# CSB5/lofreq

Measured on AMD Instinct MI355X. Metric: pileup columns/sec at depth 10000, higher is better.
Workload: dtype f64

## Files before the change

lofreq_amd/csrc/lfq_api.hip:

```cpp
#include "lfq_bound.h"
#include "lfq_ctx.h"

namespace {

struct LfqDeviceStreams {
    hipStream_t stream = nullptr, dps = nullptr, side[2] = {nullptr, nullptr};
    hipEvent_t ev_tail[3] = {nullptr, nullptr, nullptr};
    bool tail_recorded = false;
    hipEvent_t ev_end = nullptr;
    bool end_recorded = false;
    int refs = 0;
};
std::mutex g_streams_m;
LfqDeviceStreams g_streams[64];

bool acquire_streams(int device, lfq_ctx *c);
void release_streams(int device);

void *pin_acquire_impl(lfq_ctx *c, size_t bytes, int *slot)
{
    int best = -1, empty = -1, smallest = -1;
    for (int i = 0; i < LFQ_PIN_SLOTS; i++) {
        auto &b = c->pin_pool[i];
        if (b.used) {
            continue;
        }
        if (!b.p) {
            empty = (empty < 0) ? i : empty;
        } else if (b.cap >= bytes) {
            best = (best < 0 || b.cap < c->pin_pool[best].cap) ? i : best;
        } else {
            smallest = (smallest < 0 || b.cap < c->pin_pool[smallest].cap) ? i : smallest;
        }
    }
    if (best < 0) {
        best = (empty >= 0) ? empty : smallest;
        if (best < 0) {
            return nullptr;
        }
        auto &b = c->pin_pool[best];
        if (b.p) {
            (void)hipHostFree(b.p);
            b.p = nullptr;
            b.cap = 0;
        }
        const size_t cap = std::max<size_t>(bytes + bytes / 4, (size_t)1 << 16);
        if (hipHostMalloc(&b.p, cap, hipHostMallocDefault) != hipSuccess) {
            b.p = nullptr;
            return nullptr;
        }
        b.cap = cap;
    }
    c->pin_pool[best].used = 1;
    *slot = best;
    return c->pin_pool[best].p;
}

int phred_safe(double p) { return (p <= 0.0) ? INT32_MAX : (int)(-10.0 * log10l(p)); }

double jq_threshold(int m)
{
    if (m <= 0) {
        return INFINITY;
    }
    uint64_t lo = 1, hi;
    double one = 2.0;
    memcpy(&hi, &one, 8);
    if (phred_safe(4.9406564584124654e-324) < m) {
        return 0.0;
    }
    while (hi - lo > 1) {
        const uint64_t mid = lo + (hi - lo) / 2;
        double x;
        memcpy(&x, &mid, 8);
        if (phred_safe(x) >= m) {
            lo = mid;
        } else {
            hi = mid;
        }
    }
    double x;
    memcpy(&x, &lo, 8);
    return x;
}

}

int lfq_make_params(const lfq_conf *conf, const lfq_tracks *tr, LfqParams *P, bool indel_mode)
{
    if (conf->def_alt_jq == -1) {
        return LFQ_ERR_UNSUPPORTED;
    }
    memset(P, 0, sizeof(*P));
    P->min_bq4 = std::min(std::max(conf->min_bq, 0), 128);
    P->min_alt_bq4 = std::min(std::max(std::max(conf->min_bq, conf->min_alt_bq), 0), 128);
    P->def_alt_bq = conf->def_alt_bq;
    P->jq_reject_above = jq_threshold(conf->min_jq);
    P->alt_jq_reject_above = jq_threshold(conf->min_alt_jq);
    P->def_alt_jp = (conf->def_alt_jq != 0) ? pow(10.0, -1.0 * conf->def_alt_jq / 10.0) : -1.0;
    P->general = (conf->min_jq > 0) || (conf->min_alt_jq > 0) || (conf->def_alt_bq == -1);
    P->min_cov = conf->min_cov;
    P->use_baq = (conf->flag & LFQ_USE_BAQ) && tr->baq;
    P->use_mq = (conf->flag & LFQ_USE_MQ) != 0;
    P->use_sq = (conf->flag & LFQ_USE_SQ) && tr->sq;
    P->bonf_dynamic = conf->bonf_dynamic;
    P->bonf_base = conf->bonf_subst;
    P->sig = (double)conf->sig;
    P->prune_slack = 1e-6;
    P->bonf_step = 3;
    P->bonf_reset_first = 1;
    P->phase1_chunks = LFQ_PHASE1_CHUNKS;
    P->seg_budget_mid = P->seg_budget_big = LFQ_SEG_BUDGET;
    P->seg_max = lfq_knobs().seg_max >= 0 ? lfq_knobs().seg_max : LFQ_SEG_MAX;
    P->seg_max_mid = lfq_knobs().seg_max_mid >= 0 ? lfq_knobs().seg_max_mid : LFQ_SEG_MAX;
    if (indel_mode) {
        P->min_bq4 = P->min_alt_bq4 = 0;
        P->def_alt_bq = 0;
        P->jq_reject_above = P->alt_jq_reject_above = INFINITY;
        P->def_alt_jp = -1.0;
        P->general = 0;
        P->min_cov = 0;
        P->use_baq = tr->baq != nullptr;
        P->bonf_base = conf->bonf_indel;
        P->bonf_step = 1;
        P->bonf_reset_first = 0;
    }
    return LFQ_OK;
}


namespace {

bool acquire_streams(int device, lfq_ctx *c)
{
    std::lock_guard<std::mutex> lk(g_streams_m);
    if (device < 0 || device >= 64) {
        return false;
    }
    LfqDeviceStreams &d = g_streams[device];
    if (d.refs == 0) {
        int prio_lo = 0, prio_hi = 0;
        (void)hipDeviceGetStreamPriorityRange(&prio_lo, &prio_hi);
        bool ok = true;
        ok = hipStreamCreateWithFlags(&d.stream, hipStreamNonBlocking) == hipSuccess;
        ok = ok && hipStreamCreateWithPriority(&d.dps, hipStreamNonBlocking, prio_hi) == hipSuccess;
        for (int i = 0; ok && i < 2; i++) {
            ok = hipStreamCreateWithPriority(&d.side[i], hipStreamNonBlocking, prio_hi) == hipSuccess;
        }
        for (int i = 0; ok && i < 3; i++) {
            ok = hipEventCreateWithFlags(&d.ev_tail[i], hipEventDisableTiming) == hipSuccess;
        }
        ok = ok && hipEventCreateWithFlags(&d.ev_end, hipEventDisableTiming) == hipSuccess;
        d.tail_recorded = false;
        d.end_recorded = false;
        if (!ok) {
            return false;
        }
    }
    d.refs++;
    c->stream = d.stream;
    c->dps = d.dps;
    c->side[0] = d.side[0];
    c->side[1] = d.side[1];
    return true;
}

void release_streams(int device)
{
    std::lock_guard<std::mutex> lk(g_streams_m);
    LfqDeviceStreams &d = g_streams[device];
    if (d.refs > 0 && --d.refs == 0) {
        if (d.stream) (void)hipStreamDestroy(d.stream);
        if (d.dps) (void)hipStreamDestroy(d.dps);
        for (int i = 0; i < 2; i++) {
            if (d.side[i]) (void)hipStreamDestroy(d.side[i]);
        }
        for (int i = 0; i < 3; i++) {
            if (d.ev_tail[i]) (void)hipEventDestroy(d.ev_tail[i]);
        }
        if (d.ev_end) (void)hipEventDestroy(d.ev_end);
        d = LfqDeviceStreams();
    }
}

int tail_wait(lfq_ctx *c, hipStream_t st)
{
    std::lock_guard<std::mutex> lk(g_streams_m);
    LfqDeviceStreams &d = g_streams[c->device];
    if (c->stream != d.stream || c->batch_gate == LFQ_GATE_NONE) {
        return LFQ_OK;
    }
    if (c->batch_gate == LFQ_GATE_END) {
        if (d.end_recorded && hipStreamWaitEvent(st, d.ev_end, 0) != hipSuccess) {
            return LFQ_ERR_HIP;
        }
        return LFQ_OK;
    }
    if (!d.tail_recorded) {
        return LFQ_OK;
    }
    for (int i = 0; i < 3; i++) {
        if (hipStreamWaitEvent(st, d.ev_tail[i], 0) != hipSuccess) {
            return LFQ_ERR_HIP;
        }
    }
    return LFQ_OK;
}

int tail_record(lfq_ctx *c, int i, hipStream_t on)
{
    std::lock_guard<std::mutex> lk(g_streams_m);
    LfqDeviceStreams &d = g_streams[c->device];
    if (c->stream != d.stream) {
        return LFQ_OK;
    }
    if (hipEventRecord(d.ev_tail[i], on) != hipSuccess) {
        return LFQ_ERR_HIP;
    }
    d.tail_recorded = true;
    return LFQ_OK;
}

int end_record(lfq_ctx *c, hipStream_t on)
{
    std::lock_guard<std::mutex> lk(g_streams_m);
    LfqDeviceStreams &d = g_streams[c->device];
    if (c->stream != d.stream) {
        return LFQ_OK;
    }
    if (hipEventRecord(d.ev_end, on) != hipSuccess) {
        return LFQ_ERR_HIP;
    }
    d.end_recorded = true;
    return LFQ_OK;
}

void fill_luts(LfqLuts *L)
{
    for (int q = 0; q < 256; q++) {
        const double p = pow(10.0, -1.0 * q / 10.0);
        L->bq[q] = p;
        L->baq[q] = p;
        L->mq[q] = p;
        L->sq[q] = p;
    }
    L->baq[255] = 0.0;
    L->sq[255] = 0.0;
    L->sq[254] = 0.0;
    L->mq[255] = 0.0;
    L->mq[0] = 0.5;
}

void leader_main(lfq_ctx *c)
{
    (void)hipSetDevice(c->device);
    for (;;) {
        {
            std::unique_lock<std::mutex> lk(*c->lm);
            c->lcv->wait(lk, [&] { return c->leader_go > 0 || c->leader_stop; });
            if (c->leader_stop) {
                return;
            }
            c->leader_go--;
        }
        int64_t n = 0;
        if (hipEventSynchronize(c->ev_heavy) == hipSuccess) {
            n = std::min<int64_t>(std::max<int64_t>(*(volatile int32_t *)c->h_nheavy, 0), c->heavy_cap);
        }
        lfq_sb_precompute(c->h_tuples, 3 * n);
        {
            std::lock_guard<std::mutex> lk(*c->lm);
            c->sb_pending--;
        }
        c->lcv->notify_all();
    }
}

int ensure_workspace(lfq_ctx *c, int64_t ncols)
{
    if (ncols > c->ws_cols) {
        int64_t cap = 0;
        int64_t want = ncols + ncols / 8 + 1024;
        if (c->d_flags) (void)hipFree(c->d_flags);
        if (c->d_prefix) (void)hipFree(c->d_prefix);
        if (c->d_entries) (void)hipFree(c->d_entries);
        if (c->d_tiles) (void)hipFree(c->d_tiles);
        if (c->d_unsplit) (void)hipFree(c->d_unsplit);
        if (c->d_retry) (void)hipFree(c->d_retry);
        c->d_unsplit = nullptr;
        c->d_retry = nullptr;
        c->d_flags = nullptr;
        c->d_prefix = nullptr;
        c->d_entries = nullptr;
        c->d_tiles = nullptr;
        c->ws_cols = 0;
        LFQ_TRY(grow(&c->d_flags, &cap, want));
        cap = 0;
        LFQ_TRY(grow(&c->d_prefix, &cap, want));
        cap = 0;
        LFQ_TRY(grow(&c->d_entries, &cap, want));
        cap = 0;
        LFQ_TRY(grow(&c->d_tiles, &cap, 2 * (want / 1024 + 8 * (LFQ_MAX_SEGMENTS + 1))));
        cap = 0;
        LFQ_TRY(grow(&c->d_unsplit, &cap, want));
        cap = 0;
        LFQ_TRY(grow(&c->d_retry, &cap, want));
        c->ws_cols = want;
    }
    return LFQ_OK;
}


}

void *lfq_pin_acquire(lfq_ctx *c, size_t bytes, int *slot) { return pin_acquire_impl(c, bytes, slot); }

extern "C" {

void *lfq_host_alloc(size_t bytes)
{
    void *p = nullptr;
    if (hipHostMalloc(&p, bytes ? bytes : 1, hipHostMallocDefault) != hipSuccess) {
        (void)hipGetLastError();
        return nullptr;
    }
    return p;
}

void lfq_host_free(void *p)
{
    if (p) {
        (void)hipHostFree(p);
    }
}
int lfq_create(lfq_ctx **out, int device_ordinal)
{
    if (!out) {
        return LFQ_ERR_INVALID;
    }
    *out = nullptr;
    int ndev = 0;
    if (hipGetDeviceCount(&ndev) != hipSuccess || ndev <= 0 || device_ordinal < 0 || device_ordinal >= ndev) {
        return LFQ_ERR_NO_DEVICE;
    }
    if (hipSetDevice(device_ordinal) != hipSuccess) {
        return LFQ_ERR_NO_DEVICE;
    }
    lfq_ctx *c = (lfq_ctx *)calloc(1, sizeof(lfq_ctx));
    if (!c) {
        return LFQ_ERR_NOMEM;
    }
    c->device = device_ordinal;
    c->sub_ncols = -1;
    c->dense_strand = 1;
    c->dense_counts = 1;
    c->indel_host_arrays = 1;
    c->plp_max_depth = LFQ_NO_MAX_DEPTH;
    c->baq_par_d = 0.00001f;
    c->baq_par_e = 0.4f;
    hipDeviceProp_t prop;
    c->n_cu = 256;
    if (hipGetDeviceProperties(&prop, device_ordinal) == hipSuccess && prop.multiProcessorCount > 0) {
        c->n_cu = prop.multiProcessorCount;
    }
    bool ok = acquire_streams(device_ordinal, c);
    c->own_streams = ok ? 1 : 0;
    ok = ok && hipMalloc((void **)&c->d_luts, sizeof(LfqLuts)) == hipSuccess;
    ok = ok && hipMalloc((void **)&c->d_counters, (LFQ_MAX_SEGMENTS + 1) * LFQ_NCOUNTERS * sizeof(int32_t)) == hipSuccess;
    ok = ok && hipHostMalloc((void **)&c->h_counters, (LFQ_MAX_SEGMENTS + 1) * LFQ_NCOUNTERS * sizeof(int32_t) + 16,
                             hipHostMallocDefault) == hipSuccess;
    for (int i = 0; ok && i < 4; i++) {
        ok = hipEventCreate(&c->ev[i]) == hipSuccess;
    }
    for (int i = 0; ok && i < 3; i++) {
        ok = hipEventCreate(&c->ev_join[i]) == hipSuccess;
    }
    for (int s = 0; ok && s < LFQ_MAX_SEGMENTS; s++) {
        ok = hipEventCreate(&c->ev_cnt[s][0]) == hipSuccess && hipEventCreate(&c->ev_cnt[s][1]) == hipSuccess;
        ok = ok && hipEventCreate(&c->ev_scan[s]) == hipSuccess;
        ok = ok && hipEventCreate(&c->ev_light[s][0]) == hipSuccess && hipEventCreate(&c->ev_light[s][1]) == hipSuccess;
        for (int i = 0; ok && i < 2; i++) {
            ok = hipEventCreate(&c->ev_side[i][s][0]) == hipSuccess && hipEventCreate(&c->ev_side[i][s][1]) == hipSuccess;
        }
    }
    if (ok && !lfq_knobs().no_sb_precompute) {
        c->heavy_cap = 1 << 16;
        ok = hipHostMalloc((void **)&c->h_tuples, (size_t)c->heavy_cap * 3 * 4 * sizeof(int32_t), hipHostMallocMapped) == hipSuccess
             && hipHostMalloc((void **)&c->h_nheavy, 64, hipHostMallocMapped) == hipSuccess
             && hipHostGetDevicePointer((void **)&c->d_tuples_mapped, c->h_tuples, 0) == hipSuccess
             && hipHostGetDevicePointer((void **)&c->d_nheavy_mapped, c->h_nheavy, 0) == hipSuccess
             && hipEventCreateWithFlags(&c->ev_heavy, hipEventDisableTiming) == hipSuccess;
        if (ok) {
            *c->h_nheavy = 0;
            c->lm = new std::mutex();
            c->lcv = new std::condition_variable();
            c->leader = new std::thread(leader_main, c);
        }
    }
    if (ok) {
        LfqLuts h;
        fill_luts(&h);
        ok = hipMemcpy(c->d_luts, &h, sizeof(h), hipMemcpyHostToDevice) == hipSuccess;
    }
    if (ok && lfq_knobs().private_stream) {
        ok = lfq_set_private_stream(c, 1) == LFQ_OK;
    }
    if (!ok) {
        lfq_destroy(c);
        return LFQ_ERR_HIP;
    }
    *out = c;
    return LFQ_OK;
}

void lfq_destroy(lfq_ctx *c)
{
    if (c && c->leader) {
        {
            std::lock_guard<std::mutex> lk(*c->lm);
            c->leader_stop = 1;
        }
        c->lcv->notify_all();
        c->leader->join();
        delete c->leader;
        delete c->lm;
        delete c->lcv;
        c->leader = nullptr;
    }
    if (c) {
        if (c->d_plp_in) (void)hipFree(c->d_plp_in);
        if (c->d_plp_out) (void)hipFree(c->d_plp_out);
        delete c->plp_indel;
        if (c->d_plp_ne) (void)hipFree(c->d_plp_ne);
        for (int i = 0; i < 5; i++) {
            if (c->d_tmp[i]) (void)hipFree(c->d_tmp[i]);
        }
        for (int k = 0; k < 9; k++) {
            if (c->rs_cache[k].p) (void)(k == 4 || k == 7 ? hipHostFree(c->rs_cache[k].p) : hipFree(c->rs_cache[k].p));
        }
        if (c->up_stream) (void)hipStreamDestroy(c->up_stream);
        if (c->priv_stream) (void)hipStreamDestroy(c->priv_stream);
        if (c->ev_up) (void)hipEventDestroy(c->ev_up);
        if (c->ev_apply) (void)hipEventDestroy(c->ev_apply);
        free_pinned(&c->h_pin, &c->pin_bytes);
        free_pinned(&c->h_pin2, &c->pin2_bytes);
        free_pinned(&c->h_sum, &c->h_sum_bytes);
        free_pinned(&c->h_pq, &c->h_pq_bytes);
        for (int i = 0; i < LFQ_PIN_SLOTS; i++) {
            if (c->pin_pool[i].p) (void)hipHostFree(c->pin_pool[i].p);
        }
        for (LfqEvPair *t : {&c->baq_t, &c->fill_t, &c->idq_t, &c->sites_t[0], &c->sites_t[1], &c->sum_t, &c->pq_t}) {
            t->destroy();
        }
        if (c->d_detlim) (void)hipFree(c->d_detlim);
        if (c->d_sites_in) (void)hipFree(c->d_sites_in);
        if (c->d_sites_out) (void)hipFree(c->d_sites_out);
        if (c->d_sum) (void)hipFree(c->d_sum);
        delete c->plp_sum;
        if (c->d_pq) (void)hipFree(c->d_pq);
        if (c->d_baq_scr) (void)hipFree(c->d_baq_scr);
        if (c->d_baq_expect) (void)hipFree(c->d_baq_expect);
        if (c->d_baq_tmp8) (void)hipFree(c->d_baq_tmp8);
        if (c->d_baq_nflag) (void)hipFree(c->d_baq_nflag);
        if (c->d_baq_itab) (void)hipFree(c->d_baq_itab);
        if (c->d_baq_terms) (void)hipFree(c->d_baq_terms);
        lfq_viterbi_release(c);
        lfq_bam_release(c);
        lfq_bgzf_release(c);
        lfq_bgzf_deflate_release(c);
        lfq_bam_index_release(c);
        lfq_fasta_release(c);
        lfq_bed_dev_release(c->bed);
        if (c->h_tuples) (void)hipHostFree(c->h_tuples);
        if (c->h_nheavy) (void)hipHostFree(c->h_nheavy);
        if (c->ev_heavy) (void)hipEventDestroy(c->ev_heavy);
    }
    if (!c) {
        return;
    }
    (void)hipSetDevice(c->device);
    if (c->stream) (void)hipStreamSynchronize(c->stream);
    void *bufs[] = {c->d_luts, c->d_flags, c->d_prefix, c->d_entries, c->d_counters, c->d_tiles, c->d_longs, c->d_pool, c->d_unsplit, c->d_retry,
                    c->d_scratch, c->d_counts, c->d_pvals, c->d_stage, c->d_approx_mu};
    for (void *b : bufs) {
        if (b) (void)hipFree(b);
    }
    if (c->h_counters) (void)hipHostFree(c->h_counters);
    for (int i = 0; i < 4; i++) {
        if (c->ev[i]) (void)hipEventDestroy(c->ev[i]);
    }
    for (int i = 0; i < 3; i++) {
        if (c->ev_join[i]) (void)hipEventDestroy(c->ev_join[i]);
        if (i == 0 && c->ev_segw) (void)hipEventDestroy(c->ev_segw);
        if (i == 0 && c->ev_prep) (void)hipEventDestroy(c->ev_prep);
        if (i == 0 && c->ev_mid) (void)hipEventDestroy(c->ev_mid);
    }
    for (int s = 0; s < LFQ_MAX_SEGMENTS; s++) {
        hipEvent_t evs[] = {c->ev_cnt[s][0], c->ev_cnt[s][1], c->ev_scan[s], c->ev_light[s][0], c->ev_light[s][1],
                            c->ev_side[0][s][0], c->ev_side[0][s][1], c->ev_side[1][s][0], c->ev_side[1][s][1]};
        for (hipEvent_t e : evs) {
            if (e) (void)hipEventDestroy(e);
        }
    }
    if (c->own_streams) {
        release_streams(c->device);
    }
    free(c);
}

int lfq_synchronize(lfq_ctx *c)
{
    if (!c) {
        return LFQ_ERR_INVALID;
    }
    LFQ_TRY_HIP(hipStreamSynchronize(c->stream));
    LFQ_TRY_HIP(hipEventSynchronize(c->ev[3]));
    return LFQ_OK;
}

int lfq_order_after_batch(lfq_ctx *c, hipStream_t st)
{
    if (c->batch_recorded) {
        LFQ_TRY_HIP(hipStreamWaitEvent(st, c->ev[3], 0));
    }
    return LFQ_OK;
}

int lfq_batch_device_impl(lfq_ctx *c, const lfq_conf *conf, const lfq_tracks *tr, lfq_col_counts *d_counts,
                             lfq_col_pvals *d_pvals, int64_t pvals_capacity, void *stream_or_null,
                             bool indel_mode)
{
    if (!c || !conf || !tr || tr->ncols < 0 || tr->ncols > 0x7ffffff0LL) {
        return LFQ_ERR_INVALID;
    }
    if (tr->ncols > 0 && (!tr->nt || !tr->bq || !tr->mq || !tr->col_off || !tr->ref_base || !d_counts
                          || (!d_pvals && pvals_capacity > 0))) {
        return LFQ_ERR_INVALID;
    }
    if ((((uintptr_t)tr->nt) | ((uintptr_t)tr->bq)) & 15u) {
        return LFQ_ERR_INVALID;
    }
    LFQ_TRY_HIP(hipSetDevice(c->device));
    hipStream_t st = stream_or_null ? (hipStream_t)stream_or_null : c->stream;
    const LfqKnobs &kn = lfq_knobs();
    const bool single_stream = kn.single_stream != 0;
    hipStream_t dps = single_stream ? st : c->dps;
    hipStream_t side0 = single_stream ? st : c->side[0], side1 = single_stream ? st : c->side[1];
    hipStream_t side_i[2] = {side0, side1};
    LfqParams P;
    LFQ_TRY(lfq_make_params(conf, tr, &P, indel_mode));
    if (c->batch_gate == LFQ_GATE_NONE && !indel_mode) {
        if (kn.seg_max < 0) {
            P.seg_max = 2;
        }
        if (kn.seg_max_mid < 0) {
            P.seg_max_mid = 2;
        }
    }
    P.detlim_af = indel_mode ? nullptr : c->detlim_af;
    P.lazy_strand = (c->lazy_now && !indel_mode && !P.general && !P.detlim_af) ? 1 : 0;
    P.sparse_counts = (P.lazy_strand && ((d_counts == c->d_counts && c->lazy_forced) || !c->dense_counts)) ? 1 : 0;
    P.scan_gate_maxk = 0;
    P.approx_n = (!P.detlim_af && conf->approx_threshold_n > 0) ? conf->approx_threshold_n : 0;
    LFQ_TRY(ensure_workspace(c, tr->ncols));

    LfqTracksDev T;
    T.nt = tr->nt;
    T.nt_packed = (tr->flags & LFQ_TRACKS_NT_PACKED) ? 1 : 0;
    T.pad_ = 0;
    T.bq = tr->bq;
    T.baq = tr->baq;
    T.mq = tr->mq;
    T.sq = tr->sq;
    T.col_off = tr->col_off;
    T.ref_base = tr->ref_base;
    T.coverage_plp = tr->coverage_plp;
    T.num_bases = tr->num_bases;
    T.ncols = tr->ncols;

    const int64_t ncols = tr->ncols;
    int32_t *gcounters = c->d_counters + LFQ_MAX_SEGMENTS * LFQ_NCOUNTERS;
    c->cur_stream = st;
    c->cur_pvals_cap = pvals_capacity;
    c->cur_ncols = ncols;
    c->cur_segments = 0;
    c->cur_col_off = tr->col_off;
    c->cur_indel_mode = indel_mode ? 1 : 0;
    c->cur_obs_bytes_x2 = (T.nt_packed ? 1 : 2) + 2;
    if (P.general) {
        c->cur_obs_bytes_x2 += 2 * ((T.baq ? 1 : 0) + 1 + (T.sq ? 1 : 0));
        if (P.def_alt_bq == -1) {
            c->cur_obs_bytes_x2 += (T.nt_packed ? 1 : 2) + 2;
        }
    }
    c->cur_col_bytes = 8 + 1 + (T.coverage_plp ? 4 : 0) + (T.num_bases ? 4 : 0) + (P.detlim_af ? 4 : 0);
    LFQ_TRY(lfq_order_after_batch(c, st));
    LFQ_TRY(tail_wait(c, st));
    LFQ_TRY_HIP(hipMemsetAsync(c->d_counters, 0, (LFQ_MAX_SEGMENTS + 1) * LFQ_NCOUNTERS * sizeof(int32_t), st));
    if (ncols > 0) {
        LFQ_TRY_HIP(hipMemsetAsync(c->d_retry, 0, (size_t)ncols, st));
    }
    LFQ_TRY_HIP(hipEventRecord(c->ev[0], st));
    if (ncols == 0) {
        LFQ_TRY_HIP(hipMemcpyAsync(c->h_counters, c->d_counters,
                                   (LFQ_MAX_SEGMENTS + 1) * LFQ_NCOUNTERS * sizeof(int32_t), hipMemcpyDeviceToHost, st));
        LFQ_TRY_HIP(hipEventRecord(c->ev[3], st));
        c->batch_recorded = 1;
        return LFQ_OK;
    }

    int64_t max_depth = tr->max_col_obs;
    if (max_depth <= 0) {
        LFQ_TRY(lfq_launch_maxdepth(T, gcounters, st));
        LFQ_TRY_HIP(hipMemcpyAsync(c->h_counters, gcounters, LFQ_NCOUNTERS * sizeof(int32_t), hipMemcpyDeviceToHost, st));
        LFQ_TRY_HIP(hipStreamSynchronize(st));
        max_depth = c->h_counters[LFQ_GC_MAXDEPTH];
    }
    {
        static const LfqLuts h_luts = [] {
            LfqLuts h;
            fill_luts(&h);
            return h;
        }();
        const bool lb = !P.general && P.def_alt_bq == 0 && P.def_alt_jp < 0.0;
        P.bound_p_lo = (lb && !indel_mode && kn.bound_gate && lfq_count_is_lean(T, P, max_depth))
                           ? lfq_bound_p_lo(h_luts.bq, P.min_alt_bq4, LFQ_BOUND_QLO) : 0.0;
        const int kreg = lfq_screen_kreg(c->kreg_hint);
        const bool screen_runs = !kn.skip_light && kn.light_kernel != 2 && kreg > 0;
        P.scan_gate_maxk = (P.bound_p_lo > 0.0 && P.approx_n == 0 && kn.scan_gate && screen_runs) ? kreg - 1 : 0;
    }
    const int64_t per_block = 3 * max_depth + 72;
    int n_big_blocks = c->n_cu;
    const int64_t budget = (int64_t)1 << 29;
    if (per_block * n_big_blocks > budget) {
        n_big_blocks = (int)std::max<int64_t>(8, budget / per_block);
    }
    LFQ_TRY(grow(&c->d_scratch, &c->scratch_doubles, per_block * n_big_blocks));
    if (!c->d_longs) {
        c->long_cap = 1 << 16;
        c->pool_cells = kn.split_pool_cells;
        LFQ_TRY_HIP(hipMalloc((void **)&c->d_longs, (size_t)c->long_cap * (sizeof(LfqLong) + LFQ_SEG_MAX * sizeof(int32_t))));
        LFQ_TRY_HIP(hipMalloc((void **)&c->d_pool, (size_t)std::max(c->pool_cells, 1) * sizeof(LfqSegCell)));
        LFQ_TRY_HIP(hipEventCreateWithFlags(&c->ev_segw, hipEventDisableTiming));
        LFQ_TRY_HIP(hipEventCreateWithFlags(&c->ev_prep, hipEventDisableTiming));
        LFQ_TRY_HIP(hipEventCreateWithFlags(&c->ev_mid, hipEventDisableTiming));
    }

    const int n_seg = 1;
    c->cur_segments = n_seg;
    LFQ_TRY_HIP(hipEventRecord(c->ev_join[2], st));
    LFQ_TRY_HIP(hipStreamWaitEvent(dps, c->ev_join[2], 0));

    bool big_joined = false;
    for (int s = 0; s < n_seg; s++) {
        const int64_t c0 = ncols * s / n_seg, c1 = ncols * (s + 1) / n_seg;
        LfqWork W;
        W.tested_prefix = c->d_prefix;
        W.entries = c->d_entries + c0;
        W.counters = c->d_counters + s * LFQ_NCOUNTERS;
        W.gcounters = gcounters;
        W.block_sums = (int32_t *)(c->d_tiles + 2 * (c0 / 1024 + 8 * s));
        W.long_cap = c->long_cap / n_seg;
        W.pool_cells = c->pool_cells / n_seg;
        W.longs = c->d_longs + (int64_t)s * W.long_cap;
        W.pool = c->d_pool + (int64_t)s * W.pool_cells;
        W.unsplit = c->d_unsplit + c0;

        LFQ_TRY_HIP(hipEventRecord(c->ev_cnt[s][0], st));
        const bool ungated = c->batch_gate == LFQ_GATE_NONE && st == c->stream && !c->priv_stream_on && !single_stream;
        LFQ_TRY(lfq_launch_count(T, c0, c1, P, c->d_luts, d_counts, c->d_flags, max_depth, st, ungated));
        c->cur_sparse_counts = P.sparse_counts && lfq_count_is_shallow(T, P, max_depth);
        LFQ_TRY_HIP(hipEventRecord(c->ev_cnt[s][1], st));

        LFQ_TRY_HIP(hipStreamWaitEvent(dps, c->ev_cnt[s][1], 0));
        LFQ_TRY(lfq_launch_scan(T, c0, c1, P, c->d_flags, d_counts, W, dps));
        if (P.approx_n > 0) {
            LFQ_TRY(grow(&c->d_approx_mu, &c->approx_mu_bytes, (c1 - c0) * 8));
            LFQ_TRY(lfq_launch_approx_gate(T, P, c->d_luts, d_counts, W, c1 - c0, (double *)c->d_approx_mu, c->d_flags, dps));
            LFQ_TRY(lfq_launch_scan(T, c0, c1, P, c->d_flags, d_counts, W, dps, true));
        }
        LFQ_TRY_HIP(hipEventRecord(c->ev_scan[s], dps));
        const bool sb_heavy = n_seg == 1 && !indel_mode && c->leader && !kn.no_sb_precompute;
        auto launch_heavy = [&]() -> int {
            if (P.lazy_strand) {
                LFQ_TRY(lfq_launch_strand_heavy(T, W, d_counts, c->d_tuples_mapped, c->d_nheavy_mapped, c->heavy_cap, 16, dps));
            } else {
                LFQ_TRY(lfq_launch_gather_heavy(W, d_counts, c->d_tuples_mapped, c->d_nheavy_mapped, c->heavy_cap, 16, dps));
            }
            LFQ_TRY_HIP(hipEventRecord(c->ev_heavy, dps));
            {
                std::lock_guard<std::mutex> lk(*c->lm);
                c->leader_go++;
                c->sb_pending++;
            }
            c->lcv->notify_all();
            return LFQ_OK;
        };
        const bool screen = !kn.skip_light && kn.light_kernel != 2;
        if (sb_heavy && !screen) {
            LFQ_TRY(launch_heavy());
        }
        const int64_t seg_cols = c1 - c0;
        const int screen_auto = (c->batch_gate == LFQ_GATE_NONE && !indel_mode) ? (tr->max_col_obs >= 4096 ? 1 : 2) : 4;
        const int light_waves_per_cu = kn.light_kernel == 0 ? screen_auto : 10;
        const int n_light_waves = (int)std::min<int64_t>((int64_t)c->n_cu * light_waves_per_cu, std::max<int64_t>(seg_cols / 8, 4));
        const int n_mid_waves = (int)std::min<int64_t>((int64_t)c->n_cu * 4, std::max<int64_t>(seg_cols, 4));
        const int dp_wg = (c->batch_gate == LFQ_GATE_NONE && !indel_mode && kn.dp_wg_waves > 0) ? kn.dp_wg_waves : 4;
        const bool run_big = !kn.skip_big, run_mid = !kn.skip_mid;
        const bool dbg_sync = kn.debug_sync != 0;
#define LFQ_DBG_STAGE(name)                                                        \
    do {                                                                           \
        if (dbg_sync) {                                                            \
            fprintf(stderr, "[lfq] %s launched\n", name);                          \
            hipError_t e_ = hipDeviceSynchronize();                                \
            fprintf(stderr, "[lfq] %s done (%d)\n", name, (int)e_);                \
        }                                                                          \
    } while (0)
        LFQ_TRY_HIP(hipStreamWaitEvent(side1, c->ev_scan[s], 0));
        LFQ_TRY_HIP(hipEventRecord(c->ev_side[1][s][0], side1));
        LFQ_TRY_HIP(hipStreamWaitEvent(side0, c->ev_scan[s], 0));
        LFQ_TRY_HIP(hipEventRecord(c->ev_side[0][s][0], side0));
        if (run_big) {
            LFQ_TRY(lfq_launch_dp_big_prep(T, P, c->d_luts, d_counts, W, d_pvals, pvals_capacity, c->n_cu * 2, side0));
            LFQ_DBG_STAGE("prep");
        }
        LFQ_TRY_HIP(hipEventRecord(c->ev_prep, side0));
        if (run_mid) {
            LFQ_TRY(lfq_launch_dp_mid(T, P, c->d_luts, d_counts, W, d_pvals, pvals_capacity, n_mid_waves, dp_wg, side1));
            LFQ_DBG_STAGE("mid");
        }
        const bool big_on_st = run_big && !single_stream && !kn.big_on_side && c->batch_gate != LFQ_GATE_NONE;
        if (big_on_st) {
            LFQ_TRY_HIP(hipStreamWaitEvent(st, c->ev_prep, 0));
            LFQ_TRY(lfq_launch_dp_big(T, P, c->d_luts, d_counts, W, d_pvals, pvals_capacity, c->d_scratch, per_block,
                                      n_big_blocks, st));
            LFQ_DBG_STAGE("big");
            LFQ_TRY_HIP(hipEventRecord(c->ev_segw, st));
            big_joined = true;
        }
        if (run_big) {
            LFQ_TRY(lfq_launch_dp_seg(1, T, P, c->d_luts, W, c->n_cu * 8, dp_wg, side0));
            LFQ_DBG_STAGE("seg big");
            LFQ_TRY(tail_record(c, 0, side0));
            LFQ_TRY(lfq_launch_dp_combine(1, P, d_counts, W, d_pvals, pvals_capacity, c->n_cu, side0));
            LFQ_DBG_STAGE("combine big");
            if (!big_on_st) {
                LFQ_TRY(lfq_launch_dp_big(T, P, c->d_luts, d_counts, W, d_pvals, pvals_capacity, c->d_scratch, per_block,
                                          n_big_blocks, side0));
                LFQ_DBG_STAGE("big");
            }
        }
        if (!run_big) {
            LFQ_TRY(tail_record(c, 0, side0));
        }
        LFQ_TRY_HIP(hipStreamWaitEvent(side1, c->ev_prep, 0));
        if (run_mid || run_big) {
            LFQ_TRY(lfq_launch_dp_seg(0, T, P, c->d_luts, W, c->n_cu * 8, dp_wg, side1));
            LFQ_DBG_STAGE("seg mid");
            LFQ_TRY(tail_record(c, 1, side1));
            LFQ_TRY(lfq_launch_dp_combine(0, P, d_counts, W, d_pvals, pvals_capacity, c->n_cu, side1));
            LFQ_DBG_STAGE("combine mid");
        }
        if (!(run_mid || run_big)) {
            LFQ_TRY(tail_record(c, 1, side1));
        }
        LFQ_TRY_HIP(hipEventRecord(c->ev_light[s][0], dps));
        if (!kn.skip_light) {
            if (kn.light_kernel == 2) {
                LFQ_TRY(lfq_launch_dp_light(T, P, c->d_luts, d_counts, W, d_pvals, pvals_capacity, n_light_waves, dps));
            } else {
                const int kh = indel_mode ? c->kreg_hint_indel : c->kreg_hint;
                LFQ_TRY(lfq_launch_dp_quad(T, P, c->d_luts, d_counts, W, c->d_retry + c0, d_pvals, pvals_capacity,
                                           n_light_waves, kh, dps, 1));
                LFQ_TRY(tail_record(c, 2, dps));
                if (sb_heavy) {
                    LFQ_TRY(launch_heavy());
                }
                LFQ_TRY(lfq_launch_dp_quad(T, P, c->d_luts, d_counts, W, c->d_retry + c0, d_pvals, pvals_capacity,
                                           n_light_waves, kh, dps, 2));
            }
        }
        LFQ_TRY_HIP(hipEventRecord(c->ev_light[s][1], dps));
        if (!screen) {
            LFQ_TRY(tail_record(c, 2, dps));
        }
        for (int i = 0; i < 2; i++) {
            LFQ_TRY_HIP(hipEventRecord(c->ev_side[i][s][1], side_i[i]));
        }
    }
    hipStream_t jn = (st != c->stream || single_stream) ? st : side0;
    LFQ_TRY_HIP(hipEventRecord(c->ev[1], st));
    LFQ_TRY_HIP(hipEventRecord(c->ev_join[0], side0));
    LFQ_TRY_HIP(hipEventRecord(c->ev_join[1], side1));
    LFQ_TRY_HIP(hipEventRecord(c->ev_join[2], dps));
    for (int i = 0; i < 3; i++) {
        LFQ_TRY_HIP(hipStreamWaitEvent(jn, c->ev_join[i], 0));
    }
    if (big_joined && jn != st) {
        LFQ_TRY_HIP(hipStreamWaitEvent(jn, c->ev_segw, 0));
    }
    if (P.lazy_strand && d_pvals && pvals_capacity > 0) {
        LFQ_TRY(lfq_launch_strand_pvals(T, d_pvals, gcounters + LFQ_GC_PVALS, pvals_capacity, c->n_cu, jn));
    }
    LFQ_TRY(end_record(c, jn));
    LFQ_TRY_HIP(hipMemcpyAsync(c->h_counters, c->d_counters, (LFQ_MAX_SEGMENTS + 1) * LFQ_NCOUNTERS * sizeof(int32_t),
                               hipMemcpyDeviceToHost, jn));
    {
        uint64_t *h_ends = reinterpret_cast<uint64_t *>(c->h_counters + (LFQ_MAX_SEGMENTS + 1) * LFQ_NCOUNTERS);
        if (c->cur_col_off) {
            LFQ_TRY_HIP(hipMemcpyAsync(h_ends, c->cur_col_off, 8, hipMemcpyDeviceToHost, jn));
            LFQ_TRY_HIP(hipMemcpyAsync(h_ends + 1, c->cur_col_off + c->cur_ncols, 8, hipMemcpyDeviceToHost, jn));
        }
    }
    LFQ_TRY_HIP(hipEventRecord(c->ev[3], jn));
    c->batch_recorded = 1;
    return LFQ_OK;
}

int lfq_snv_batch_device(lfq_ctx *c, const lfq_conf *conf, const lfq_tracks *tr, lfq_col_counts *d_counts,
                         lfq_col_pvals *d_pvals, int64_t pvals_capacity, void *stream_or_null)
{
    if (!c) {
        return LFQ_ERR_INVALID;
    }
    if (!c->lazy_forced) {
        c->lazy_now = !c->dense_strand;
    }
    return lfq_batch_device_impl(c, conf, tr, d_counts, d_pvals, pvals_capacity, stream_or_null, false);
}

int lfq_set_indel_arrays_on_host(lfq_ctx *c, int on)
{
    if (!c) {
        return LFQ_ERR_INVALID;
    }
    c->indel_host_arrays = on ? 1 : 0;
    return LFQ_OK;
}

int lfq_set_indel_arrays_all_columns(lfq_ctx *c, int on)
{
    if (!c) {
        return LFQ_ERR_INVALID;
    }
    c->indel_all_columns = on ? 1 : 0;
    return LFQ_OK;
}

int lfq_set_pileup_nt_packed(lfq_ctx *c, int on)
{
    if (!c) {
        return LFQ_ERR_INVALID;
    }
    c->plp_nt_bytes = on ? 0 : 1;
    return LFQ_OK;
}

int lfq_set_pileup_unsorted(lfq_ctx *c, int on)
{
    if (!c) {
        return LFQ_ERR_INVALID;
    }
    c->plp_unsorted_ok = on ? 1 : 0;
    return LFQ_OK;
}

int lfq_set_max_depth(lfq_ctx *c, int64_t max_depth)
{
    if (!c || max_depth < LFQ_NO_MAX_DEPTH) {
        return LFQ_ERR_INVALID;
    }
    c->plp_max_depth = max_depth;
    return LFQ_OK;
}

int lfq_set_baq_hmm_params(lfq_ctx *c, float gap_open, float gap_ext)
{
    if (!c || !(gap_open > 0.f) || !(gap_open < 0.5f) || !(gap_ext > 0.f) || !(gap_ext < 1.f)) {
        return LFQ_ERR_INVALID;
    }
    c->baq_par_d = gap_open;
    c->baq_par_e = gap_ext;
    return LFQ_OK;
}

int lfq_pack_nt_track(const uint8_t *nt_bytes, int64_t n_obs, uint8_t *packed_out)
{
    if (n_obs < 0 || (n_obs > 0 && (!nt_bytes || !packed_out))) {
        return LFQ_ERR_INVALID;
    }
    const int64_t full = n_obs / 8;
    for (int64_t g = 0; g < full; g++) {
        for (int k = 0; k < 4; k++) {
            packed_out[4 * g + k] = (uint8_t)((nt_bytes[8 * g + k] & 15) | ((nt_bytes[8 * g + 4 + k] & 15) << 4));
        }
    }
    if (n_obs & 7) {
        uint8_t last[8] = {0, 0, 0, 0, 0, 0, 0, 0};
        memcpy(last, nt_bytes + 8 * full, (size_t)(n_obs & 7));
        for (int k = 0; k < 4; k++) {
            packed_out[4 * full + k] = (uint8_t)((last[k] & 15) | ((last[4 + k] & 15) << 4));
        }
    }
    return LFQ_OK;
}

int lfq_set_batch_gate(lfq_ctx *c, int gate)
{
    if (!c || (gate != LFQ_GATE_TAIL && gate != LFQ_GATE_END && gate != LFQ_GATE_NONE)) {
        return LFQ_ERR_INVALID;
    }
    c->batch_gate = gate;
    return LFQ_OK;
}

int lfq_set_private_stream(lfq_ctx *c, int on)
{
    if (!c || !c->own_streams) {
        return LFQ_ERR_INVALID;
    }
    LFQ_TRY_HIP(hipSetDevice(c->device));
    LFQ_TRY(lfq_synchronize(c));
    LFQ_TRY_HIP(hipStreamSynchronize(c->stream));
    if (on) {
        if (!c->priv_stream) {
            LFQ_TRY_HIP(hipStreamCreateWithFlags(&c->priv_stream, hipStreamNonBlocking));
        }
        c->stream = c->priv_stream;
        c->priv_stream_on = 1;
    } else {
        std::lock_guard<std::mutex> lk(g_streams_m);
        c->stream = g_streams[c->device].stream;
        c->priv_stream_on = 0;
    }
    return LFQ_OK;
}

int lfq_set_dense_counts(lfq_ctx *c, int on)
{
    if (!c) {
        return LFQ_ERR_INVALID;
    }
    c->dense_counts = on ? 1 : 0;
    return LFQ_OK;
}

int lfq_set_dense_strand_counts(lfq_ctx *c, int on)
{
    if (!c) {
        return LFQ_ERR_INVALID;
    }
    c->dense_strand = on ? 1 : 0;
    return LFQ_OK;
}

int lfq_indel_batch_device(lfq_ctx *c, const lfq_conf *conf, const lfq_tracks *tr, lfq_col_counts *d_counts,
                           lfq_col_pvals *d_pvals, int64_t pvals_capacity, void *stream_or_null)
{
    return lfq_batch_device_impl(c, conf, tr, d_counts, d_pvals, pvals_capacity, stream_or_null, true);
}

int lfq_batch_finish(lfq_ctx *c, lfq_batch_stats *stats)
{
    if (!c) {
        return LFQ_ERR_INVALID;
    }
    LFQ_TRY_HIP(hipEventSynchronize(c->ev[3]));
    const uint64_t *h_ends = reinterpret_cast<const uint64_t *>(c->h_counters + (LFQ_MAX_SEGMENTS + 1) * LFQ_NCOUNTERS);
    const int64_t batch_obs = (c->cur_col_off && c->cur_ncols > 0) ? (int64_t)(h_ends[1] - h_ends[0]) : 0;
    c->cur_count_read = batch_obs * c->cur_obs_bytes_x2 / 2 + c->cur_ncols * c->cur_col_bytes;
    c->cur_count_written = c->cur_ncols * (int64_t)(sizeof(lfq_col_counts) + 1);
    if (c->cur_sparse_counts) {
        c->cur_count_written = c->cur_ncols + (int64_t)c->h_counters[LFQ_MAX_SEGMENTS * LFQ_NCOUNTERS + LFQ_GC_TESTED] * (int64_t)sizeof(lfq_col_counts);
    }
    const int32_t *g = c->h_counters + LFQ_MAX_SEGMENTS * LFQ_NCOUNTERS;
    memset(&c->times, 0, sizeof(c->times));
    float ms = 0.f;
    if (hipEventElapsedTime(&ms, c->ev[0], c->ev[3]) == hipSuccess) c->times.ms_total = ms;
    float dp_end = 0.f;
    for (int s = 0; s < c->cur_segments; s++) {
        if (hipEventElapsedTime(&ms, c->ev_cnt[s][0], c->ev_cnt[s][1]) == hipSuccess) c->times.ms_count += ms;
        if (hipEventElapsedTime(&ms, c->ev_cnt[s][1], c->ev_scan[s]) == hipSuccess) c->times.ms_scan += ms;
        if (hipEventElapsedTime(&ms, c->ev_light[s][0], c->ev_light[s][1]) == hipSuccess) c->times.ms_dp_light += ms;
        if (hipEventElapsedTime(&ms, c->ev_side[0][s][0], c->ev_side[0][s][1]) == hipSuccess) c->times.ms_dp_big += ms;
        if (hipEventElapsedTime(&ms, c->ev_side[1][s][0], c->ev_side[1][s][1]) == hipSuccess) c->times.ms_dp_mid += ms;
    }
    if (c->cur_segments > 0 && hipEventElapsedTime(&dp_end, c->ev_cnt[c->cur_segments - 1][1], c->ev[3]) == hipSuccess) {
        c->times.ms_dp = dp_end;
    }
    c->times.n_segments = c->cur_segments;
    memset(&c->work, 0, sizeof(c->work));
    memcpy(&c->work.cells, g + LFQ_GC_CELLS, 8);
    memcpy(&c->work.rows, g + LFQ_GC_ROWS, 8);
    c->work.n_light_retry = g[LFQ_GC_SCREEN_RETRY];
    c->work.n_approx_pruned = g[LFQ_GC_APPROX_PRUNED];
    for (int s = 0; s < c->cur_segments; s++) {
        const int32_t *sc = c->h_counters + s * LFQ_NCOUNTERS;
        c->work.n_light += sc[LFQ_CNT_LIGHT];
        c->work.n_mid += sc[LFQ_CNT_MID];
        c->work.n_big += sc[LFQ_CNT_BIG];
    }
    {
        const int32_t *sc = c->h_counters;
        const int64_t n_light = sc[LFQ_CNT_LIGHT];
        int hint = 64;
        for (int f = LFQ_NKHIST - 1; f >= 0; f--) {
            if ((int64_t)sc[LFQ_CNT_KHIST + f] >= n_light - n_light / 2000) {
                hint = lfq_khist_thr(f) + 1;
            }
        }
        if (n_light > 0) {
            (c->cur_indel_mode ? c->kreg_hint_indel : c->kreg_hint) = hint;
        }
    }
    c->work.bytes_read_count = c->cur_count_read;
    c->work.bytes_written_count = c->cur_count_written;
    if (stats) {
        stats->n_tested = g[LFQ_GC_TESTED];
        stats->n_pvals = std::min<int64_t>(g[LFQ_GC_PVALS], c->cur_pvals_cap);
        stats->n_obs = batch_obs;
    }
    if (g[LFQ_GC_OVERFLOW]) {
        return LFQ_ERR_CAPACITY;
    }
    return LFQ_OK;
}

int lfq_debug_counters(lfq_ctx *c, int32_t *out16)
{
    if (!c || !out16) {
        return LFQ_ERR_INVALID;
    }
    memcpy(out16, c->h_counters, 64 * sizeof(int32_t));
    return LFQ_OK;
}

int lfq_last_dp_work(lfq_ctx *c, lfq_dp_work *w)
{
    if (!c || !w) {
        return LFQ_ERR_INVALID;
    }
    *w = c->work;
    return LFQ_OK;
}

int lfq_last_kernel_times(lfq_ctx *c, lfq_kernel_times *t)
{
    if (!c || !t) {
        return LFQ_ERR_INVALID;
    }
    *t = c->times;
    return LFQ_OK;
}

int lfq_stage_tracks(lfq_ctx *c, const lfq_tracks *tr, int tracks_on_device, lfq_tracks *dev_out)
{
    const int64_t ncols = tr->ncols;
    lfq_tracks dev = *tr;
    if (ncols > 0 && (!tr->nt || !tr->bq || !tr->mq || !tr->col_off || !tr->ref_base)) {
        return LFQ_ERR_INVALID;
    }
    if (!tracks_on_device) {
        const uint64_t n_obs = tr->col_off[ncols];
        const int64_t trk = (int64_t)((n_obs + 15) / 16 * 16) + 16;
        int64_t need = 5 * trk + (ncols + 1) * 8 + (ncols + 16) + 2 * (ncols * 4 + 16) + 64;
        if (!c->up_stream && hipStreamCreateWithFlags(&c->up_stream, hipStreamNonBlocking) != hipSuccess) {
            c->up_stream = nullptr;
            return LFQ_ERR_HIP;
        }
        if (!c->ev_up && hipEventCreateWithFlags(&c->ev_up, hipEventDisableTiming) != hipSuccess) {
            return LFQ_ERR_HIP;
        }
        hipStream_t ups = c->up_stream;
        LFQ_TRY(lfq_order_after_batch(c, ups));
        LFQ_TRY(grow(&c->d_stage, &c->stage_bytes, need));
        uint8_t *p = c->d_stage;
        auto put = [&](const void *src, int64_t bytes, int64_t reserve) -> uint8_t * {
            uint8_t *dst = p;
            p += (reserve + 15) / 16 * 16;
            if (!src) {
                return nullptr;
            }
            if (bytes > 0 && hipMemcpyAsync(dst, src, (size_t)bytes, hipMemcpyHostToDevice, ups) != hipSuccess) {
                return nullptr;
            }
            return dst;
        };
        dev.nt = put(tr->nt, (tr->flags & LFQ_TRACKS_NT_PACKED) ? (int64_t)((n_obs + 7) / 8 * 4) : (int64_t)n_obs, trk);
        dev.bq = put(tr->bq, (int64_t)n_obs, trk);
        dev.baq = put(tr->baq, (int64_t)n_obs, trk);
        dev.mq = put(tr->mq, (int64_t)n_obs, trk);
        dev.sq = put(tr->sq, (int64_t)n_obs, trk);
        dev.col_off = (const uint64_t *)put(tr->col_off, (ncols + 1) * 8, (ncols + 1) * 8);
        dev.ref_base = put(tr->ref_base, ncols, ncols + 16);
        dev.coverage_plp = (const int32_t *)put(tr->coverage_plp, ncols * 4, ncols * 4 + 16);
        dev.num_bases = (const int32_t *)put(tr->num_bases, ncols * 4, ncols * 4 + 16);
        if (!dev.nt || !dev.bq || !dev.mq || !dev.col_off || !dev.ref_base) {
            return LFQ_ERR_HIP;
        }
        if (dev.max_col_obs <= 0) {
            uint64_t md = 0;
            for (int64_t i = 0; i < ncols; i++) {
                md = std::max(md, tr->col_off[i + 1] - tr->col_off[i]);
            }
            dev.max_col_obs = (int64_t)md;
        }
        LFQ_TRY_HIP(hipEventRecord(c->ev_up, ups));
        LFQ_TRY_HIP(hipStreamWaitEvent(c->stream, c->ev_up, 0));
    }

    *dev_out = dev;
    return LFQ_OK;
}

int lfq_call_snvs_submit(lfq_ctx *c, const lfq_conf *conf, const lfq_tracks *tr, int tracks_on_device)
{
    if (!c || !conf || !tr || tr->ncols < 0) {
        return LFQ_ERR_INVALID;
    }
    if (c->sub_ncols >= 0) {
        return LFQ_ERR_INVALID;
    }
    c->sub_t0 = lfq_now_ms();
    if (tr->ncols == 0) {
        c->sub_ncols = 0;
        return LFQ_OK;
    }
    LFQ_TRY_HIP(hipSetDevice(c->device));
    const int64_t ncols = tr->ncols;
    lfq_tracks dev;
    LFQ_TRY(lfq_stage_tracks(c, tr, tracks_on_device, &dev));
    LFQ_TRY(grow(&c->d_counts, &c->counts_cap, ncols));
    LFQ_TRY(grow(&c->d_pvals, &c->pvals_cap, ncols));
    LFQ_TRY(lfq_snv_batch_device(c, conf, &dev, c->d_counts, c->d_pvals, c->pvals_cap, c->stream));
    c->sub_ncols = ncols;
    c->sub_ref_host = tracks_on_device ? nullptr : tr->ref_base;
    c->sub_t1 = lfq_now_ms();
    return LFQ_OK;
}

int lfq_call_snvs_wait(lfq_ctx *c)
{
    if (!c || c->sub_ncols < 0) {
        return LFQ_ERR_INVALID;
    }
    if (c->sub_ncols == 0) {
        return LFQ_OK;
    }
    LFQ_TRY_HIP(hipSetDevice(c->device));
    LFQ_TRY_HIP(hipEventSynchronize(c->ev[3]));
    return LFQ_OK;
}

int lfq_call_snvs_collect(lfq_ctx *c, lfq_conf *conf, lfq_snv_record *records, int64_t records_capacity,
                          int64_t *n_records, lfq_col_counts *h_counts_or_null, lfq_batch_stats *stats_out)
{
    if (!c || !conf || !n_records || c->sub_ncols < 0) {
        return LFQ_ERR_INVALID;
    }
    *n_records = 0;
    const int64_t ncols = c->sub_ncols;
    if (ncols > 0 && h_counts_or_null && c->cur_sparse_counts) {
        return LFQ_ERR_INVALID;
    }
    c->sub_ncols = -1;
    if (ncols == 0) {
        if (stats_out) memset(stats_out, 0, sizeof(*stats_out));
        return LFQ_OK;
    }
    LFQ_TRY_HIP(hipSetDevice(c->device));
    double tp[4];
    tp[0] = lfq_now_ms();
    lfq_batch_stats st;
    LFQ_TRY(lfq_batch_finish(c, &st));
    tp[1] = lfq_now_ms();
    LfqPin<lfq_col_pvals> h_pv(c, (size_t)st.n_pvals);
    LFQ_PIN_OK(h_pv);
    if (st.n_pvals > 0) {
        LFQ_TRY_HIP(hipMemcpy(h_pv.data(), c->d_pvals, (size_t)st.n_pvals * sizeof(lfq_col_pvals),
                              hipMemcpyDeviceToHost));
    }
    if (h_counts_or_null) {
        LFQ_TRY_HIP(hipMemcpy(h_counts_or_null, c->d_counts, (size_t)ncols * sizeof(lfq_col_counts),
                              hipMemcpyDeviceToHost));
    }
    tp[2] = lfq_now_ms();
    if (c->leader) {
        std::unique_lock<std::mutex> lk(*c->lm);
        c->lcv->wait(lk, [&] { return c->sb_pending == 0 || c->leader_stop; });
    }
    int rc = lfq_finalize_pvals(conf, h_pv.data(), st.n_pvals, nullptr, c->sub_ref_host, records, records_capacity,
                                n_records);
    tp[3] = lfq_now_ms();
    if (lfq_timing_on) {
        fprintf(stderr, "[lfq timing] launch %.3f  wait %.3f  d2h %.3f  finalize %.3f ms (kernels %.3f ms, %ld records)\n",
                c->sub_t1 - c->sub_t0, tp[1] - tp[0], tp[2] - tp[1], tp[3] - tp[2], (double)c->times.ms_total, (long)st.n_pvals);
    }
    if (st.n_tested > 0) {
        if (conf->bonf_dynamic) {
            conf->bonf_subst = ((conf->bonf_subst == 1) ? 0 : conf->bonf_subst) + 3 * st.n_tested;
        }
        conf->num_snv_tests += 3 * st.n_tested;
    }
    if (stats_out) {
        *stats_out = st;
    }
    return rc;
}

int lfq_call_snvs_collect_pvals(lfq_ctx *c, lfq_col_pvals *pvals, int64_t pvals_capacity, int64_t *n_pvals,
                                lfq_batch_stats *stats_out)
{
    if (!c || !n_pvals || c->sub_ncols < 0 || pvals_capacity < 0 || (pvals_capacity > 0 && !pvals)) {
        return LFQ_ERR_INVALID;
    }
    *n_pvals = 0;
    const int64_t ncols = c->sub_ncols;
    c->sub_ncols = -1;
    if (ncols == 0) {
        if (stats_out) memset(stats_out, 0, sizeof(*stats_out));
        return LFQ_OK;
    }
    LFQ_TRY_HIP(hipSetDevice(c->device));
    lfq_batch_stats st;
    LFQ_TRY(lfq_batch_finish(c, &st));
    if (c->leader) {
        std::unique_lock<std::mutex> lk(*c->lm);
        c->lcv->wait(lk, [&] { return c->sb_pending == 0 || c->leader_stop; });
    }
    if (stats_out) {
        *stats_out = st;
    }
    *n_pvals = st.n_pvals;
    if (st.n_pvals > pvals_capacity) {
        return LFQ_ERR_CAPACITY;
    }
    if (st.n_pvals > 0) {
        LfqPin<lfq_col_pvals> h_pv(c, (size_t)st.n_pvals);
        LFQ_PIN_OK(h_pv);
        LFQ_TRY_HIP(hipMemcpy(h_pv.data(), c->d_pvals, (size_t)st.n_pvals * sizeof(lfq_col_pvals), hipMemcpyDeviceToHost));
        memcpy(pvals, h_pv.data(), (size_t)st.n_pvals * sizeof(lfq_col_pvals));
    }
    return LFQ_OK;
}

int lfq_call_snvs_batch(lfq_ctx *c, lfq_conf *conf, const lfq_tracks *tr, int tracks_on_device,
                        lfq_snv_record *records, int64_t records_capacity, int64_t *n_records,
                        lfq_col_counts *h_counts_or_null, lfq_batch_stats *stats_out)
{
    if (!c || !conf || !tr || !n_records || tr->ncols < 0) {
        return LFQ_ERR_INVALID;
    }
    *n_records = 0;
    c->lazy_forced = 1;
    c->lazy_now = h_counts_or_null == nullptr;
    const int rc = lfq_call_snvs_submit(c, conf, tr, tracks_on_device);
    c->lazy_forced = 0;
    LFQ_TRY(rc);
    return lfq_call_snvs_collect(c, conf, records, records_capacity, n_records, h_counts_or_null, stats_out);
}
static inline float lfq_uniq_reset_af(float af)
{
    if (af < 0.0 || af > 1.0) {
        return af < 0.0 ? 0.01f : 1.0f;
    }
    return af;
}

int lfq_uniq_detlim_batch(lfq_ctx *c, const lfq_tracks *tr, int tracks_on_device, const float *af,
                          uint8_t *detectable, long double *pvalue_or_null)
{
    if (!c || !tr || !af || !detectable || tr->ncols < 0) {
        return LFQ_ERR_INVALID;
    }
    const int64_t ncols = tr->ncols;
    if (ncols == 0) {
        return LFQ_OK;
    }
    LFQ_TRY_HIP(hipSetDevice(c->device));
    LfqPin<float> h_af(c, (size_t)ncols);
    LFQ_PIN_OK(h_af);
    for (int64_t i = 0; i < ncols; i++) {
        if (af[i] != af[i]) {
            return LFQ_ERR_INVALID;
        }
        h_af[(size_t)i] = lfq_uniq_reset_af(af[i]);
    }
    lfq_conf conf;
    lfq_conf_init(&conf);
    conf.bonf_dynamic = 0;
    conf.bonf_subst = 1;
    conf.sig = 0.01f;
    lfq_tracks dev;
    LFQ_TRY(lfq_stage_tracks(c, tr, tracks_on_device, &dev));
    LFQ_TRY(grow(&c->d_counts, &c->counts_cap, ncols));
    LFQ_TRY(grow(&c->d_pvals, &c->pvals_cap, ncols));
    LFQ_TRY(grow(&c->d_detlim, &c->detlim_cap, ncols));
    LFQ_TRY_HIP(hipMemcpyAsync(c->d_detlim, h_af.data(), (size_t)ncols * 4, hipMemcpyHostToDevice, c->stream));
    c->detlim_af = c->d_detlim;
    int rc = lfq_snv_batch_device(c, &conf, &dev, c->d_counts, c->d_pvals, c->pvals_cap, c->stream);
    c->detlim_af = nullptr;
    LFQ_TRY(rc);
    lfq_batch_stats st;
    LFQ_TRY(lfq_batch_finish(c, &st));
    LfqPin<lfq_col_pvals> h_pv(c, (size_t)st.n_pvals);
    LFQ_PIN_OK(h_pv);
    if (st.n_pvals > 0) {
        LFQ_TRY_HIP(hipMemcpy(h_pv.data(), c->d_pvals, (size_t)st.n_pvals * sizeof(lfq_col_pvals), hipMemcpyDeviceToHost));
    }
    memset(detectable, 0, (size_t)ncols);
    if (pvalue_or_null) {
        for (int64_t i = 0; i < ncols; i++) {
            pvalue_or_null[i] = LDBL_MAX;
        }
    }
    const int bonf = 1;
    const float alpha = 0.01f;
    for (size_t pi = 0; pi < h_pv.size(); pi++) {
        const lfq_col_pvals &p = h_pv[pi];
        if (p.col < 0 || p.col >= ncols || p.status[0] == LFQ_PV_NONE) {
            continue;
        }
        const long double pv = lfq_pvalue_from_log(p.logp[0], p.status[0]);
        if (pvalue_or_null) {
            pvalue_or_null[p.col] = pv;
        }
        detectable[p.col] = (pv * (float)bonf < alpha) ? 1 : 0;
    }
    return LFQ_OK;
}

int lfq_uniq_binom_batch(lfq_ctx *c, const lfq_tracks *tr, int tracks_on_device, const float *af, const char *alt_base,
                         int32_t *uq_out, double *pvalue_or_null)
{
    if (!c || !tr || !af || !alt_base || !uq_out || tr->ncols < 0) {
        return LFQ_ERR_INVALID;
    }
    const int64_t ncols = tr->ncols;
    if (ncols == 0) {
        return LFQ_OK;
    }
    LFQ_TRY_HIP(hipSetDevice(c->device));
    lfq_tracks dev;
    LFQ_TRY(lfq_stage_tracks(c, tr, tracks_on_device, &dev));
    LfqTracksDev T;
    memset(&T, 0, sizeof(T));
    T.nt = dev.nt;
    T.bq = dev.bq;
    T.col_off = dev.col_off;
    T.ncols = ncols;
    T.nt_packed = (dev.flags & LFQ_TRACKS_NT_PACKED) ? 1 : 0;
    LFQ_TRY(grow(&c->d_counts, &c->counts_cap, ncols));
    int32_t *d_nt = reinterpret_cast<int32_t *>(c->d_counts);
    LFQ_TRY(lfq_launch_ntcount(T, d_nt, c->stream));
    LfqPin<int32_t> h_nt(c, (size_t)ncols * 4), h_cov(c, dev.coverage_plp ? (size_t)ncols : 0);
    LfqPin<uint64_t> h_off(c, (size_t)ncols + 1);
    LFQ_PIN_OK(h_nt);
    LFQ_PIN_OK(h_cov);
    LFQ_PIN_OK(h_off);
    LFQ_TRY_HIP(hipMemcpyAsync(h_nt.data(), d_nt, (size_t)ncols * 16, hipMemcpyDeviceToHost, c->stream));
    LFQ_TRY_HIP(hipMemcpyAsync(h_off.data(), dev.col_off, ((size_t)ncols + 1) * 8, hipMemcpyDeviceToHost, c->stream));
    if (dev.coverage_plp) {
        LFQ_TRY_HIP(hipMemcpyAsync(h_cov.data(), dev.coverage_plp, (size_t)ncols * 4, hipMemcpyDeviceToHost, c->stream));
    }
    LFQ_TRY_HIP(hipStreamSynchronize(c->stream));
    for (int64_t i = 0; i < ncols; i++) {
        uq_out[i] = -1;
        if (pvalue_or_null) {
            pvalue_or_null[i] = -1.0;
        }
        const int coverage = dev.coverage_plp ? h_cov[(size_t)i] : (int)(h_off[(size_t)i + 1] - h_off[(size_t)i]);
        if (coverage < 1) {
            continue;
        }
        const char ab = alt_base[i];
        const int code = (ab == 'A' || ab == 'a') ? 0 : (ab == 'C' || ab == 'c') ? 1 : (ab == 'G' || ab == 'g') ? 2
                         : (ab == 'T' || ab == 't') ? 3 : 4;
        const int n_col = (int)(h_off[(size_t)i + 1] - h_off[(size_t)i]);
        const int32_t *cn = &h_nt[(size_t)i * 4];
        const int alt_count = code < 4 ? cn[code] : n_col - cn[0] - cn[1] - cn[2] - cn[3];
        int st = 0;
        const double pv = lfq_binom_cdf(coverage, alt_count, (double)lfq_uniq_reset_af(af[i]), &st);
        if (st != 0) {
            continue;
        }
        uq_out[i] = phred_safe(pv);
        if (pvalue_or_null) {
            pvalue_or_null[i] = pv;
        }
    }
    return LFQ_OK;
}

int lfq_readset_uniq(lfq_ctx *c, lfq_readset *rs, const lfq_uniq_variants *v, int use_det_lim, int min_plp_bq,
                     lfq_uniq_result *out)
{
    if (!c || !rs || !v || !out || v->n < 0
        || (v->n > 0 && (!v->pos || !v->ref_off || !v->alt_off || !v->ref || !v->alt || !v->af))) {
        return LFQ_ERR_INVALID;
    }
    const int64_t n = v->n;
    if (n == 0) {
        lfq_tracks none;
        return lfq_readset_sites_impl(c, rs, nullptr, 0, min_plp_bq, nullptr, nullptr, nullptr, &none, nullptr, nullptr, nullptr, nullptr);
    }
    for (int64_t i = 0; i < n; i++) {
        if (v->ref_off[i + 1] < v->ref_off[i] || v->alt_off[i + 1] < v->alt_off[i] || v->af[i] != v->af[i]) {
            return LFQ_ERR_INVALID;
        }
    }
    std::vector<uint8_t> is_indel((size_t)n), key_del((size_t)n);
    std::vector<int64_t> key_off((size_t)n + 1, 0);
    std::vector<char> key_chars;
    bool any_indel = false, any_snv = false;
    for (int64_t i = 0; i < n; i++) {
        const int64_t rl = v->ref_off[i + 1] - v->ref_off[i], al = v->alt_off[i + 1] - v->alt_off[i];
        is_indel[(size_t)i] = (rl > 1 || al > 1 || (v->indel_key_or_null && v->indel_key_or_null[i])) ? 1 : 0;
        key_del[(size_t)i] = 0;
        if (is_indel[(size_t)i]) {
            any_indel = true;
            const bool del = rl > al;
            key_del[(size_t)i] = del ? 1 : 0;
            const char *s = del ? v->ref + v->ref_off[i] : v->alt + v->alt_off[i];
            const int64_t l = del ? rl : al;
            if (l > 1) {
                key_chars.insert(key_chars.end(), s + 1, s + l);
            }
        } else {
            any_snv = true;
        }
        key_off[(size_t)i + 1] = (int64_t)key_chars.size();
    }
    const bool keys = any_indel && !use_det_lim;
    key_chars.push_back('\0');
    lfq_tracks T;
    std::vector<int32_t> cov((size_t)n), nb((size_t)n), tails((size_t)n), ev((size_t)n, 0);
    LFQ_TRY(lfq_readset_sites_impl(c, rs, v->pos, n, min_plp_bq, keys ? key_off.data() : nullptr, key_chars.data(),
                                   key_del.data(), &T, cov.data(), nb.data(), tails.data(), keys ? ev.data() : nullptr));
    for (int64_t i = 0; i < n; i++) {
        cov[(size_t)i] -= is_indel[(size_t)i] ? tails[(size_t)i] : 0;
        if (out->coverage) out->coverage[i] = cov[(size_t)i];
        if (out->alt_count) out->alt_count[i] = 0;
        if (out->uq) out->uq[i] = -1;
        if (out->pvalue) out->pvalue[i] = -1.0;
        if (out->detectable) out->detectable[i] = 0;
    }
    if (use_det_lim) {
        std::vector<uint8_t> det((size_t)n);
        LFQ_TRY(lfq_uniq_detlim_batch(c, &T, 1, v->af, det.data(), nullptr));
        for (int64_t i = 0; i < n && out->detectable; i++) {
            out->detectable[i] = (cov[(size_t)i] >= 1 && det[(size_t)i]) ? 1 : 0;
        }
        return LFQ_OK;
    }
    LfqPin<int32_t> h_nt(c, any_snv ? (size_t)n * 4 : 0);
    LFQ_PIN_OK(h_nt);
    if (any_snv) {
        LfqTracksDev D;
        memset(&D, 0, sizeof(D));
        D.nt = T.nt;
        D.bq = T.bq;
        D.col_off = T.col_off;
        D.ncols = n;
        D.nt_packed = 0;
        LFQ_TRY(grow(&c->d_counts, &c->counts_cap, n));
        int32_t *d_nt = reinterpret_cast<int32_t *>(c->d_counts);
        LFQ_TRY(lfq_launch_ntcount(D, d_nt, c->stream));
        LFQ_TRY_HIP(hipMemcpyAsync(h_nt.data(), d_nt, (size_t)n * 16, hipMemcpyDeviceToHost, c->stream));
        LFQ_TRY_HIP(hipStreamSynchronize(c->stream));
    }
    for (int64_t i = 0; i < n; i++) {
        if (cov[(size_t)i] < 1) {
            continue;
        }
        int alt_count;
        if (is_indel[(size_t)i]) {
            alt_count = ev[(size_t)i];
        } else {
            const char ab = v->alt_off[i + 1] > v->alt_off[i] ? v->alt[v->alt_off[i]] : '\0';
            const int code = (ab == 'A' || ab == 'a') ? 0 : (ab == 'C' || ab == 'c') ? 1 : (ab == 'G' || ab == 'g') ? 2
                             : (ab == 'T' || ab == 't') ? 3 : 4;
            const int32_t *cn = &h_nt[(size_t)i * 4];
            const int64_t n_col = nb[(size_t)i];
            alt_count = code < 4 ? cn[code] : (int)(n_col - cn[0] - cn[1] - cn[2] - cn[3]);
        }
        if (out->alt_count) out->alt_count[i] = alt_count;
        int st = 0;
        const double pv = lfq_binom_cdf(cov[(size_t)i], alt_count, (double)lfq_uniq_reset_af(v->af[i]), &st);
        if (st != 0) {
            continue;
        }
        if (out->uq) out->uq[i] = phred_safe(pv);
        if (out->pvalue) out->pvalue[i] = pv;
    }
    return LFQ_OK;
}

int lfq_pileup_skip_snv_columns(lfq_ctx *c, const uint8_t *skip, int64_t ncols)
{
    if (!c || !skip || ncols < 0 || !c->d_plp_out || ncols != c->plp_ncols) {
        return LFQ_ERR_INVALID;
    }
    if (ncols == 0) {
        return LFQ_OK;
    }
    LFQ_TRY_HIP(hipSetDevice(c->device));
    LfqPin<uint8_t> h(c, (size_t)ncols);
    LFQ_PIN_OK(h);
    memcpy(h.data(), skip, (size_t)ncols);
    LFQ_TRY(lfq_order_after_batch(c, c->stream));
    LFQ_TRY(grow(&c->d_tmp[2], &c->tmp_bytes[2], ncols));
    LFQ_TRY_HIP(hipMemcpyAsync(c->d_tmp[2], h.data(), (size_t)ncols, hipMemcpyHostToDevice, c->stream));
    LFQ_TRY(lfq_launch_skip_columns(c->d_plp_nb, c->d_tmp[2], ncols, c->stream));
    LFQ_TRY_HIP(hipStreamSynchronize(c->stream));
    return LFQ_OK;
}

int lfq_synth_fill_device(lfq_ctx *c, uint64_t seed, uint32_t depth, uint32_t plant_period, int64_t col_begin,
                          int64_t ncols, uint8_t *d_nt, uint8_t *d_bq, uint8_t *d_baq, uint8_t *d_mq,
                          uint64_t *d_col_off, uint8_t *d_ref_base, void *stream_or_null)
{
    return lfq_synth_fill_device_layout(c, seed, depth, plant_period, col_begin, ncols, d_nt, d_bq, d_baq, d_mq, d_col_off,
                                        d_ref_base, 0, stream_or_null);
}

int lfq_synth_fill_device_layout(lfq_ctx *c, uint64_t seed, uint32_t depth, uint32_t plant_period, int64_t col_begin,
                                 int64_t ncols, uint8_t *d_nt, uint8_t *d_bq, uint8_t *d_baq, uint8_t *d_mq,
                                 uint64_t *d_col_off, uint8_t *d_ref_base, int nt_packed, void *stream_or_null)
{
    if (!c || !d_nt || !d_bq || !d_baq || !d_mq || !d_col_off || !d_ref_base || ncols < 0 || depth == 0) {
        return LFQ_ERR_INVALID;
    }
    LFQ_TRY_HIP(hipSetDevice(c->device));
    lfq_synth_spec s;
    memset(&s, 0, sizeof(s));
    s.seed = seed;
    s.depth = depth;
    s.plant_period = plant_period;
    for (int q = 0; q < 64; q++) {
        const long double p = powl(10.0L, -(long double)q / 10.0L);
        const long double t = floorl(p * 18446744073709551616.0L);
        s.err_thresh[q] = (t >= 18446744073709551615.0L) ? UINT64_MAX : (uint64_t)t;
    }
    hipStream_t st = stream_or_null ? (hipStream_t)stream_or_null : c->stream;
    LFQ_TRY(lfq_order_after_batch(c, st));
    return lfq_launch_synth(&s, col_begin, ncols, d_nt, d_bq, d_baq, d_mq, d_col_off, d_ref_base, nt_packed ? 1 : 0, st);
}

}
```

lofreq_amd/csrc/lfq_ctx.h:

```cpp
#ifndef LFQ_CTX_H
#define LFQ_CTX_H

#include <hip/hip_runtime.h>

#include <ctype.h>
#include <float.h>
#include <math.h>
#include <stdio.h>
#include <stdlib.h>
#include <string.h>

#include <algorithm>
#include <chrono>
#include <condition_variable>
#include <mutex>
#include <string>
#include <atomic>
#include <functional>
#include <unistd.h>
#include <fcntl.h>
#include <sys/file.h>
#include <thread>
#include <vector>

#include "lfq_internal.h"
#include "lfq_plp_indel_host.h"
#include "lfq_bed.h"
#include "lofreq_synth.h"

#define LFQ_TRY_HIP(expr)           \
    do {                            \
        hipError_t e_ = (expr);     \
        if (e_ != hipSuccess) {     \
            return LFQ_ERR_HIP;     \
        }                           \
    } while (0)

#define LFQ_TRY(expr)               \
    do {                            \
        int rc_ = (expr);           \
        if (rc_ != LFQ_OK) {        \
            return rc_;             \
        }                           \
    } while (0)

static inline double lfq_now_ms()
{
    return std::chrono::duration<double, std::milli>(std::chrono::steady_clock::now().time_since_epoch()).count();
}
#define lfq_timing_on (lfq_knobs().timing != 0)

#if defined(__x86_64__) || defined(__i386__)
#define LFQ_CPU_PAUSE() __builtin_ia32_pause()
#elif defined(__aarch64__)
#define LFQ_CPU_PAUSE() __asm__ __volatile__("yield")
#else
#define LFQ_CPU_PAUSE() std::this_thread::yield()
#endif

#define LFQ_HOST_PARTS 16

class LfqLoopPool {
public:
    static LfqLoopPool &instance()
    {
        static LfqLoopPool p;
        return p;
    }
    bool try_run(int parts, const std::function<void(int)> &task)
    {
        if (parts - 1 > (int)th_.size() || getpid() != pid_ || !call_m_.try_lock()) {
            return false;
        }
        job_ = &task;
        want_ = parts - 1;
        pending_.store((int)th_.size(), std::memory_order_relaxed);
        gen_.fetch_add(1, std::memory_order_seq_cst);
        if (sleepers_.load(std::memory_order_seq_cst) > 0) {
            { std::lock_guard<std::mutex> lk(m_); }
            cv_.notify_all();
        }
        return true;
    }
    void finish()
    {
        while (pending_.load(std::memory_order_acquire) > 0) {
            LFQ_CPU_PAUSE();
        }
        job_ = nullptr;
        call_m_.unlock();
    }

private:
    LfqLoopPool() : pid_(getpid())
    {
        spin_us_ = lfq_knobs().host_spin_us;
        const unsigned hw = std::max(1u, lfq_cpu_budget() / (unsigned)std::max(lfq_knobs().local_world_size, 1));
        const unsigned want = (unsigned)std::min<long>(std::max<long>(lfq_knobs().host_loop_threads, 1), LFQ_HOST_PARTS);
        const int n = spin_us_ < 0 ? 0 : (int)std::min(want - 1u, hw - 1u);
        for (int i = 0; i < n; i++) {
            th_.emplace_back([this, i] { loop(i); });
        }
    }
    ~LfqLoopPool()
    {
        if (getpid() != pid_) {
            for (auto &t : th_) {
                t.detach();
            }
            return;
        }
        stop_.store(true);
        gen_.fetch_add(1, std::memory_order_seq_cst);
        { std::lock_guard<std::mutex> lk(m_); }
        cv_.notify_all();
        for (auto &t : th_) {
            t.join();
        }
    }
    void loop(int idx)
    {
        uint64_t seen = 0;
        for (;;) {
            const double t0 = lfq_now_ms();
            int polls = 0;
            while (gen_.load(std::memory_order_acquire) == seen) {
                LFQ_CPU_PAUSE();
                if ((++polls & 255) == 0 && (lfq_now_ms() - t0) * 1e3 > (double)spin_us_) {
                    std::unique_lock<std::mutex> lk(m_);
                    sleepers_.fetch_add(1, std::memory_order_seq_cst);
                    cv_.wait(lk, [&] { return gen_.load(std::memory_order_seq_cst) != seen; });
                    sleepers_.fetch_sub(1, std::memory_order_seq_cst);
                }
            }
            if (stop_.load()) {
                return;
            }
            seen = gen_.load(std::memory_order_acquire);
            if (idx < want_ && job_) {
                (*job_)(idx + 1);
            }
            pending_.fetch_sub(1, std::memory_order_release);
        }
    }
    std::vector<std::thread> th_;
    std::mutex call_m_, m_;
    std::condition_variable cv_;
    std::atomic<uint64_t> gen_{0};
    std::atomic<int> pending_{0}, sleepers_{0};
    std::atomic<bool> stop_{false};
    const std::function<void(int)> *job_ = nullptr;
    int want_ = 0;
    long spin_us_ = 2000;
    pid_t pid_;
};

template <typename F>
static void lfq_run_parts(int n_parts, F f)
{
    const std::function<void(int)> task = [&](int p) { f(p); };
    if (n_parts > 1 && LfqLoopPool::instance().try_run(n_parts, task)) {
        f(0);
        LfqLoopPool::instance().finish();
        return;
    }
    std::vector<std::thread> th;
    for (int p = 1; p < n_parts; p++) {
        th.emplace_back([&f, p] { f(p); });
    }
    f(0);
    for (auto &t : th) {
        t.join();
    }
}

template <typename F>
static void lfq_for_reads(int64_t n, F f, int *parts_out = nullptr)
{
    int parts = 1;
    const int64_t par_min = lfq_knobs().host_par_min;
    if (n >= par_min) {
        unsigned hw = lfq_cpu_budget();
        hw = std::max(1u, hw / (unsigned)lfq_knobs().local_world_size);
        const unsigned want = (unsigned)std::min<long>(std::max<long>(lfq_knobs().host_loop_threads, 1), LFQ_HOST_PARTS);
        parts = (int)std::min<int64_t>(std::min<unsigned>(hw ? hw : 1u, want), n / std::max<int64_t>(par_min / 2, 1));
        parts = std::max(parts, 1);
    }
    if (parts_out) {
        *parts_out = parts;
    }
    lfq_run_parts(parts, [&](int p) { f(n * p / parts, n * (p + 1) / parts, p); });
}

struct LfqSummaryOwned {
    lfq_plp_summary sum;
    std::vector<int64_t> col_pos, key_off;
    std::vector<uint8_t> ref_base, cons_kind;
    std::vector<int32_t> n_ins, n_dels, hrun, cov;
    std::vector<char> key_chars;
};

#define LFQ_PIN_SLOTS 40

struct LfqEvPair {
    hipEvent_t ev[2];
    int begin(hipStream_t st)
    {
        for (hipEvent_t &e : ev) {
            if (!e && hipEventCreate(&e) != hipSuccess) {
                return LFQ_ERR_HIP;
            }
        }
        return hipEventRecord(ev[0], st) == hipSuccess ? (int)LFQ_OK : (int)LFQ_ERR_HIP;
    }
    int end(hipStream_t st) { return !ev[1] || hipEventRecord(ev[1], st) == hipSuccess ? (int)LFQ_OK : (int)LFQ_ERR_HIP; }
    template <typename T> int ms(T *out) const
    {
        float t = 0.f;
        if (ev[1] && hipEventSynchronize(ev[1]) != hipSuccess) {
            return LFQ_ERR_HIP;
        }
        if (ev[1] && hipEventElapsedTime(&t, ev[0], ev[1]) == hipSuccess) {
            *out = (T)t;
        }
        return LFQ_OK;
    }
    void destroy()
    {
        for (hipEvent_t &e : ev) {
            if (e) (void)hipEventDestroy(e);
            e = nullptr;
        }
    }
};

struct LfqBedDev {
    std::atomic<int> refs;
    LfqBedName host;
    int32_t *d;
    LfqBedTab tab;
};
static inline LfqBedDev *lfq_bed_dev_retain(LfqBedDev *b)
{
    if (b) b->refs.fetch_add(1);
    return b;
}
void lfq_bed_dev_release(LfqBedDev *b);

struct lfq_ctx {
    int device;
    hipStream_t stream;
    LfqLuts *d_luts;
    int64_t ws_cols;
    uint8_t *d_flags;
    uint8_t *d_approx_mu;
    int64_t approx_mu_bytes;
    int32_t *d_prefix, *d_counters;
    LfqEntry *d_entries;
    hipStream_t dps;
    hipStream_t side[2];
    hipEvent_t ev_mid;
    hipEvent_t ev_cnt[LFQ_MAX_SEGMENTS][2];
    hipEvent_t ev_scan[LFQ_MAX_SEGMENTS];
    hipEvent_t ev_light[LFQ_MAX_SEGMENTS][2];
    hipEvent_t ev_side[2][LFQ_MAX_SEGMENTS][2];
    hipEvent_t ev_join[3];
    int cur_segments;
    uint64_t *d_tiles;
    double *d_scratch;
    int64_t scratch_doubles;
    LfqLong *d_longs;
    LfqSegCell *d_pool;
    int32_t long_cap, pool_cells;
    hipEvent_t ev_segw, ev_prep;
    int32_t *d_unsplit;
    uint8_t *d_retry;
    int32_t *h_counters;
    lfq_col_counts *d_counts;
    int64_t counts_cap;
    lfq_col_pvals *d_pvals;
    int64_t pvals_cap;
    uint8_t *d_stage;
    int64_t stage_bytes;
    hipStream_t cur_stream;
    int64_t cur_pvals_cap;
    int64_t cur_ncols;
    hipEvent_t ev[4];
    lfq_kernel_times times;
    lfq_dp_work work;
    int64_t cur_count_read, cur_count_written;
    const uint64_t *cur_col_off;
    int cur_obs_bytes_x2, cur_col_bytes;
    int cur_sparse_counts;
    int n_cu;
    int32_t *h_tuples, *d_tuples_mapped;
    int32_t *h_nheavy, *d_nheavy_mapped;
    int heavy_cap;
    hipEvent_t ev_heavy;
    uint8_t *d_plp_in, *d_plp_out;
    int64_t plp_in_bytes, plp_out_bytes;
    uint8_t *d_tmp[5];
    struct { void *p; size_t cap; } rs_cache[9];
    int priv_stream_on;
    hipStream_t priv_stream;
    hipStream_t up_stream;
    hipEvent_t ev_up;
    hipEvent_t ev_apply;
    uint8_t *h_pin;
    int64_t pin_bytes;
    uint8_t *h_pin2;
    int64_t pin2_bytes;
    int64_t tmp_bytes[5];
    int64_t plp_ne_cap;
    LfqIndelColsOwned *plp_indel;
    int indel_host_arrays;
    int16_t *d_plp_ne;
    int64_t plp_ne_total[2];
    int dense_counts;
    int dense_strand;
    int lazy_forced;
    LfqEvPair baq_t;
    int32_t baq_launches;
    int64_t baq_reads, baq_bases;
    LfqEvPair fill_t;
    lfq_baq_fill_stats fill_stats;
    int fill_hmm, fill_merge;
    LfqEvPair idq_t;
    lfq_indelqual_times idq_times;
    int batch_gate;
    int lazy_now;
    int64_t sub_ncols;
    int batch_recorded;
    float baq_par_d, baq_par_e;
    int plp_nt_bytes;
    int plp_unsorted_ok;
    int64_t plp_max_depth;
    const uint8_t *sub_ref_host;
    double sub_t0, sub_t1;
    const float *detlim_af;
    float *d_detlim;
    int64_t detlim_cap;
    int32_t *d_plp_nb;
    uint8_t *d_sites_in, *d_sites_out;
    int64_t sites_in_bytes, sites_out_bytes;
    LfqEvPair sites_t[2];
    lfq_sites_times sites_times;
    int64_t plp_ncols;
    uint8_t *d_sum;
    int64_t sum_bytes;
    uint8_t *h_sum;
    int64_t h_sum_bytes;
    struct LfqSummaryOwned *plp_sum;
    LfqEvPair sum_t;
    lfq_summary_times sum_times;
    uint8_t *d_pq;
    int64_t pq_bytes;
    uint8_t *h_pq;
    int64_t h_pq_bytes;
    lfq_plp_quals plp_quals;
    LfqEvPair pq_t;
    lfq_plp_quals_times pq_times;
    int indel_all_columns;
    double *d_baq_scr;
    int32_t *d_baq_expect;
    uint8_t *d_baq_tmp8;
    uint8_t *d_baq_nflag;
    int64_t baq_nflag_bytes;
    int32_t *d_baq_itab;
    double *d_baq_terms;
    int64_t baq_scr_bytes, baq_expect_bytes, baq_tmp8_bytes, baq_itab_bytes, baq_terms_bytes;
    std::thread *leader;
    std::mutex *lm;
    std::condition_variable *lcv;
    int leader_go, leader_stop;
    int own_streams;
    int kreg_hint, kreg_hint_indel;
    int cur_indel_mode;
    int sb_pending;
    struct { void *p; size_t cap; int used; } pin_pool[LFQ_PIN_SLOTS];
    struct LfqViterbiState *vit;
    struct LfqBamState *bam;
    struct LfqBgzfState *bgzf;
    struct LfqBgzfDefState *bgzf_def;
    struct LfqBamIdxState *bamidx;
    LfqBedDev *bed;
    struct LfqFastaState *fasta;
};

template <typename T>
int grow(T **ptr, int64_t *cap, int64_t need)
{
    if (need <= *cap && *ptr) {
        return LFQ_OK;
    }
    if (*ptr) {
        (void)hipFree(*ptr);
        *ptr = nullptr;
    }
    int64_t n = std::max<int64_t>(need, 16);
    if (hipMalloc((void **)ptr, (size_t)n * sizeof(T)) != hipSuccess) {
        *cap = 0;
        return LFQ_ERR_NOMEM;
    }
    *cap = n;
    return LFQ_OK;
}

static inline int grow_pinned(uint8_t **ptr, int64_t *cap, int64_t need)
{
    if (need <= *cap && *ptr) {
        return LFQ_OK;
    }
    if (*ptr) {
        (void)hipHostFree(*ptr);
        *ptr = nullptr;
    }
    if (hipHostMalloc((void **)ptr, (size_t)std::max<int64_t>(need, 16), hipHostMallocDefault) != hipSuccess) {
        *cap = 0;
        return LFQ_ERR_NOMEM;
    }
    *cap = std::max<int64_t>(need, 16);
    return LFQ_OK;
}
static inline void free_pinned(uint8_t **ptr, int64_t *cap)
{
    if (*ptr) (void)hipHostFree(*ptr);
    *ptr = nullptr;
    *cap = 0;
}

static inline bool lfq_is_pinned(const void *p)
{
    if (!p) {
        return true;
    }
    hipPointerAttribute_t at;
    memset(&at, 0, sizeof(at));
    if (hipPointerGetAttributes(&at, p) != hipSuccess) {
        (void)hipGetLastError();
        return false;
    }
    return at.type == hipMemoryTypeHost;
}

void *lfq_pin_acquire(lfq_ctx *c, size_t bytes, int *slot);

template <typename T>
struct LfqPin {
    lfq_ctx *c;
    T *p = nullptr;
    size_t n = 0;
    int slot = -1;
    LfqPin(lfq_ctx *ctx, size_t count) : c(ctx), n(count)
    {
        p = (T *)lfq_pin_acquire(c, std::max<size_t>(count, 1) * sizeof(T), &slot);
    }
    LfqPin(lfq_ctx *ctx, size_t count, T v) : LfqPin(ctx, count)
    {
        if (p) {
            std::fill(p, p + n, v);
        }
    }
    LfqPin(const LfqPin &) = delete;
    LfqPin &operator=(const LfqPin &) = delete;
    ~LfqPin()
    {
        if (slot >= 0) {
            c->pin_pool[slot].used = 0;
        }
    }
    bool ok() const { return p != nullptr; }
    T *data() { return p; }
    const T *data() const { return p; }
    size_t size() const { return n; }
    T &operator[](size_t i) { return p[i]; }
    const T &operator[](size_t i) const { return p[i]; }
    T &back() { return p[n - 1]; }
};
#define LFQ_PIN_OK(v)                                                                                                  \
    do {                                                                                                               \
        if (!(v).ok()) {                                                                                               \
            return LFQ_ERR_NOMEM;                                                                                      \
        }                                                                                                              \
    } while (0)

int lfq_make_params(const lfq_conf *conf, const lfq_tracks *tr, LfqParams *P, bool indel_mode);
void lfq_viterbi_release(lfq_ctx *c);
int lfq_viterbi_run(lfq_ctx *c, const lfq_baq_reads *reads, int def_qual, const LfqReadsDev *res,
                    const lfq_viterbi_result **out);
int lfq_viterbi_permute(lfq_ctx *c, int64_t n_reads, int64_t n_bases, const int64_t *d_new_off, const int64_t *old_start,
                        int n_arrays, const uint8_t *const *src, uint8_t *const *dst);
struct LfqBamIn {
    const uint8_t *data;
    int64_t data_bytes;
    int first_shift;
    bool pinned;
};
void lfq_bam_release(lfq_ctx *c);
void lfq_bam_times_reset(lfq_ctx *c, int64_t n_reads, int64_t n_bases, int64_t n_data_bytes);
int lfq_bam_aux(lfq_ctx *c, const LfqBamIn &in, const int64_t *desc, int64_t n, int64_t nb, uint8_t *flags_out, int *any_bi,
                int *any_bd, unsigned read_tags, uint8_t *stored_out);
int lfq_bam_bases(lfq_ctx *c, uint8_t *d_seq, uint8_t *d_qual, uint8_t *d_bi, uint8_t *d_bd, uint8_t *h_seq, uint8_t *h_qual,
                  uint8_t *h_bi, uint8_t *h_bd);
int lfq_bam_stored(lfq_ctx *c, uint8_t *const d_dst[3]);
int lfq_bam_merge(const int64_t *d_seq_off, const uint8_t *d_take, const uint8_t *const d_src[3], uint8_t *const d_dst[3],
                  uint8_t *d_tagfl, int64_t n, int64_t nb, hipStream_t st);
struct LfqBamRead {
    int64_t rec, end;
    int32_t l_qseq;
    uint32_t n_cigar;
    uint16_t l_qname, flag;
    uint32_t pad_;
};
struct LfqBamEncIn {
    LfqBamIn recs;
    const LfqBamRead *reads;
    int64_t n;
    unsigned what;
    bool uniform;
    LfqReadsDev rd;
    const uint8_t *d_fl, *d_lb, *d_ai, *d_ad, *d_bi, *d_bd;
    const int64_t *src;
    const int32_t *pos;
    const uint32_t *n_cigar;
};
int lfq_bam_encode(lfq_ctx *c, const LfqBamEncIn *in, const lfq_bam_encoded **out);
int lfq_bam_encode_empty(lfq_ctx *c, const lfq_bam_encoded **out);
void lfq_bgzf_release(lfq_ctx *c);
const uint8_t *lfq_bgzf_resident(lfq_ctx *c, const uint8_t *p, int64_t bytes);
const uint8_t *lfq_bgzf_resident_bytes(lfq_ctx *c, const uint8_t *p, int64_t bytes);
const uint8_t *lfq_bam_framed_resident(lfq_ctx *c, const uint8_t *p, int64_t bytes);
void lfq_bgzf_deflate_release(lfq_ctx *c);
void lfq_bam_index_release(lfq_ctx *c);
void lfq_fasta_release(lfq_ctx *c);
const uint8_t *lfq_fasta_resident(lfq_ctx *c, const uint8_t *p, int64_t bytes);
int lfq_launch_bed_keep(const LfqBedTab &tab, const int32_t *pos, const int64_t *cigar_off, const uint32_t *cigar, int64_t n,
                        uint8_t *keep_out, void *stream);
int lfq_launch_bed_mask_columns(const LfqBedTab &tab, int64_t begin, int64_t width, int32_t *cov, int32_t *nb_or_null, void *stream);
extern "C" {
int lfq_order_after_batch(lfq_ctx *c, hipStream_t st);
int lfq_batch_device_impl(lfq_ctx *c, const lfq_conf *conf, const lfq_tracks *tr, lfq_col_counts *d_counts,
                          lfq_col_pvals *d_pvals, int64_t pvals_capacity, void *stream_or_null, bool indel_mode);
int lfq_stage_tracks(lfq_ctx *c, const lfq_tracks *tr, int tracks_on_device, lfq_tracks *dev_out);
int lfq_readset_sites_impl(lfq_ctx *c, lfq_readset *rs, const int64_t *site_pos, int64_t n_sites, int min_plp_bq,
                           const int64_t *key_off, const char *key_chars, const uint8_t *key_del, lfq_tracks *out,
                           int32_t *cov_out, int32_t *nb_out, int32_t *tails_out, int32_t *ev_out);
int lfq_readset_from_bam_ends(lfq_ctx *c, const lfq_bam_records *recs, const int64_t *data_end, unsigned read_tags, lfq_readset **out);
}

#endif
```

lofreq_amd/csrc/lfq_host.cpp:

```cpp
#include <errno.h>
#include <fenv.h>
#include <float.h>
#include <limits.h>
#include <math.h>
#include <stdio.h>
#include <stdlib.h>
#include <string.h>

#include <algorithm>
#include <atomic>
#include <chrono>
#include <condition_variable>
#include <functional>
#include <mutex>
#include <sched.h>
#include <string>
#include <thread>
#include <unordered_map>
#include <vector>

#include "lofreq_amd.h"
#include "lfq_internal.h"

#ifdef LFQ_TUNE
#define LFQ_TUNE_I(name, dflt) geti(name, dflt)
#define LFQ_TUNE_HAS(name) has(name)
#else
#define LFQ_TUNE_I(name, dflt) ((long)(dflt))
#define LFQ_TUNE_HAS(name) false
#endif
const LfqKnobs &lfq_knobs(void)
{
    static const LfqKnobs k = [] {
        LfqKnobs x;
        memset(&x, 0, sizeof(x));
        auto geti = [](const char *name, long dflt) -> long {
            const char *e = getenv(name);
            return (e && *e) ? atol(e) : dflt;
        };
        auto has = [](const char *name) { return getenv(name) != nullptr; };
        x.timing = has("LFQ_TIMING");
        x.single_stream = has("LFQ_SINGLE_STREAM");
        x.debug_sync = has("LFQ_DEBUG_SYNC");
        x.private_stream = (int)geti("LFQ_PRIVATE_STREAM", 0);
        x.sync_upload = (int)geti("LFQ_SYNC_UPLOAD", 0);
        x.baq_scratch_mb = geti("LFQ_BAQ_SCRATCH_MB", -1);
        x.host_threads = (int)geti("LFQ_HOST_THREADS", -1);
        x.host_loop_threads = geti("LFQ_HOST_LOOP_THREADS", 8);
        x.host_spin_us = geti("LFQ_HOST_SPIN_US", 2000);
        x.local_world_size = (int)std::max(1L, geti("LOCAL_WORLD_SIZE", 1));
        x.no_sb_precompute = LFQ_TUNE_HAS("LFQ_NO_SB_PRECOMPUTE");
#ifdef LFQ_TUNE
        if (const char *sk = getenv("LFQ_DEBUG_SKIP")) {
            x.skip_light = strstr(sk, "light") != nullptr;
            x.skip_mid = strstr(sk, "mid") != nullptr;
            x.skip_big = strstr(sk, "big") != nullptr;
        }
        if (const char *lk = getenv("LFQ_LIGHT_KERNEL")) {
            x.light_kernel = !strcmp(lk, "wave") ? 2 : 0;
        }
#endif
        x.screen_rounds = (int)std::max(1L, LFQ_TUNE_I("LFQ_SCREEN_ROUNDS", 24));
        {
            const long both = LFQ_TUNE_I("LFQ_SEG_MAX", -1);
            const long big = LFQ_TUNE_I("LFQ_SEG_MAX_BIG", both), mid = LFQ_TUNE_I("LFQ_SEG_MAX_MID", both);
            x.seg_max = big < 0 ? -1 : (int)std::min((long)LFQ_SEG_MAX, std::max(2L, big));
            x.seg_max_mid = mid < 0 ? -1 : (int)std::min((long)LFQ_SEG_MAX, std::max(2L, mid));
        }
        x.split_pool_cells = (int)std::max(0L, LFQ_TUNE_I("LFQ_SPLIT_POOL_CELLS", 8L << 20));
        x.count_multi_below = LFQ_TUNE_I("LFQ_COUNT_MULTI_BELOW", 4096);
        x.big_on_side = LFQ_TUNE_HAS("LFQ_BIG_ON_SIDE");
        x.pileup_tiles = (int)LFQ_TUNE_I("LFQ_PILEUP_TILES", 1);
        x.baq_one_variant = LFQ_TUNE_HAS("LFQ_BAQ_ONE_VARIANT") ? 1 : 0;
        x.count_lpg4_below = LFQ_TUNE_I("LFQ_COUNT_LPG4_BELOW", 320);
        x.count_lpg8_below = LFQ_TUNE_I("LFQ_COUNT_LPG8_BELOW", 900);
        x.host_par_min = std::max(1L, LFQ_TUNE_I("LFQ_HOST_PAR_MIN", 200000));
        x.indel_host_pack = LFQ_TUNE_HAS("LFQ_INDEL_HOST_PACK");
        x.pileup_atomic = LFQ_TUNE_HAS("LFQ_PILEUP_ATOMIC");
        x.baq_lds = LFQ_TUNE_I("LFQ_BAQ_LDS", 1) != 0;
        x.bound_gate = LFQ_TUNE_I("LFQ_BOUND_GATE", 1) != 0;
        x.scan_gate = LFQ_TUNE_I("LFQ_SCAN_GATE", 1) != 0;
        {
            const long w = LFQ_TUNE_I("LFQ_DP_WG_WAVES", 0);
            x.dp_wg_waves = w <= 0 ? 0 : (w >= 16 ? 16 : (w >= 8 ? 8 : 4));
        }
        (void)geti;
        (void)has;
        return x;
    }();
    return k;
}

namespace {

inline double phred_to_prob(int q)
{
    return (q == INT_MAX) ? DBL_MIN : pow(10.0, -1.0 * q / 10.0);
}

inline int prob_to_phred(long double p) { return (int)(-10.0 * log10l(p)); }

inline int prob_to_phred_safe(double p) { return (p <= 0.0) ? INT_MAX : (int)(-10.0 * log10l(p)); }

inline int eps_cmp(double a, double b)
{
    if (fabs(a - b) < DBL_EPSILON) {
        return 0;
    }
    return a < b ? -1 : (a > b ? 1 : 0);
}

struct IndexedP {
    double p;
    int64_t i;
};

void sort_indexed(std::vector<IndexedP> &v)
{
    std::stable_sort(v.begin(), v.end(), [](const IndexedP &a, const IndexedP &b) { return eps_cmp(a.p, b.p) < 0; });
}


double log_choose(int n, int k)
{
    if (k == 0 || n == k) {
        return 0;
    }
    int sg;
    return lgamma_r(n + 1, &sg) - lgamma_r(k + 1, &sg) - lgamma_r(n - k + 1, &sg);
}

double hypergeom(int n11, int n1_, int n_1, int n)
{
    return exp(log_choose(n1_, n11) + log_choose(n - n1_, n_1 - n11) - log_choose(n, n_1));
}

struct HyperAcc {
    int n11, n1_, n_1, n;
    double p;
};

double hypergeom_next(int n11, int n1_, int n_1, int n, HyperAcc &s)
{
    if (n1_ || n_1 || n) {
        s.n11 = n11;
        s.n1_ = n1_;
        s.n_1 = n_1;
        s.n = n;
    } else {
        if (n11 % 11 && n11 + s.n - s.n1_ - s.n_1) {
            if (n11 == s.n11 + 1) {
                s.p *= (double)(s.n1_ - s.n11) / n11 * (s.n_1 - s.n11) / (n11 + s.n - s.n1_ - s.n_1);
                s.n11 = n11;
                return s.p;
            }
            if (n11 == s.n11 - 1) {
                s.p *= (double)s.n11 / (s.n1_ - n11) * (s.n11 + s.n - s.n1_ - s.n_1) / (s.n_1 - n11);
                s.n11 = n11;
                return s.p;
            }
        }
        s.n11 = n11;
    }
    s.p = hypergeom(s.n11, s.n1_, s.n_1, s.n);
    return s.p;
}

}

unsigned lfq_cpu_budget(void)
{
    static const unsigned budget = [] {
        unsigned n = std::thread::hardware_concurrency();
        n = n ? n : 1u;
        cpu_set_t set;
        CPU_ZERO(&set);
        if (sched_getaffinity(0, sizeof(set), &set) == 0) {
            const int a = CPU_COUNT(&set);
            if (a > 0) {
                n = std::min<unsigned>(n, (unsigned)a);
            }
        }
        long long quota = -1, period = -1;
        if (FILE *f = fopen("/sys/fs/cgroup/cpu.max", "r")) {
            char q[32];
            if (fscanf(f, "%31s %lld", q, &period) == 2 && strcmp(q, "max") != 0) {
                quota = atoll(q);
            }
            fclose(f);
        } else {
            if (FILE *g = fopen("/sys/fs/cgroup/cpu/cpu.cfs_quota_us", "r")) {
                if (fscanf(g, "%lld", &quota) != 1) quota = -1;
                fclose(g);
            }
            if (FILE *g = fopen("/sys/fs/cgroup/cpu/cpu.cfs_period_us", "r")) {
                if (fscanf(g, "%lld", &period) != 1) period = -1;
                fclose(g);
            }
        }
        if (quota > 0 && period > 0) {
            n = std::min<unsigned>(n, (unsigned)std::max<long long>(1, (quota + period - 1) / period));
        }
        return std::max(1u, n);
    }();
    return budget;
}

namespace {

class LfqPool {
public:
    static LfqPool &instance()
    {
        static LfqPool p;
        return p;
    }
    int size() const { return (int)threads_.size(); }
    void run(const std::function<void()> &f, int helpers)
    {
        helpers = std::max(0, std::min(helpers, size()));
        if (helpers == 0) {
            f();
            return;
        }
        std::unique_lock<std::mutex> call_lock(call_m_, std::try_to_lock);
        if (!call_lock.owns_lock()) {
            f();
            return;
        }
        {
            std::lock_guard<std::mutex> lk(m_);
            job_ = &f;
            want_ = helpers;
            pending_ = helpers;
            generation_++;
        }
        cv_start_.notify_all();
        f();
        std::unique_lock<std::mutex> lk(m_);
        cv_done_.wait(lk, [&] { return pending_ == 0; });
        job_ = nullptr;
    }

private:
    LfqPool()
    {
        unsigned hw = lfq_cpu_budget();
        const LfqKnobs &kn = lfq_knobs();
        hw = std::max(1u, hw / (unsigned)kn.local_world_size);
        int n = (int)std::min<unsigned>(hw > 1 ? hw - 1 : 0, 63u);
        if (kn.host_threads >= 0) {
            n = std::max(0, std::min(kn.host_threads - 1, 255));
        }
        for (int i = 0; i < n; i++) {
            threads_.emplace_back([this, i] { loop(i); });
        }
    }
    ~LfqPool()
    {
        {
            std::lock_guard<std::mutex> lk(m_);
            stop_ = true;
            generation_++;
        }
        cv_start_.notify_all();
        for (auto &t : threads_) {
            t.join();
        }
    }
    void loop(int idx)
    {
        int seen = 0;
        for (;;) {
            const std::function<void()> *job = nullptr;
            {
                std::unique_lock<std::mutex> lk(m_);
                cv_start_.wait(lk, [&] { return generation_ != seen; });
                seen = generation_;
                if (stop_) {
                    return;
                }
                if (idx >= want_) {
                    continue;
                }
                job = job_;
            }
            (*job)();
            {
                std::lock_guard<std::mutex> lk(m_);
                pending_--;
            }
            cv_done_.notify_one();
        }
    }
    std::vector<std::thread> threads_;
    std::mutex m_, call_m_;
    std::condition_variable cv_start_, cv_done_;
    const std::function<void()> *job_ = nullptr;
    int generation_ = 0, want_ = 0, pending_ = 0;
    bool stop_ = false;
};

}

namespace {

struct SbKey {
    int32_t a, b, c, d;
    bool operator==(const SbKey &o) const { return a == o.a && b == o.b && c == o.c && d == o.d; }
};
struct SbKeyHash {
    size_t operator()(const SbKey &k) const
    {
        uint64_t h = (uint64_t)(uint32_t)k.a * 0x9E3779B97F4A7C15ull;
        h ^= ((uint64_t)(uint32_t)k.b + 0x7F4A7C15ull) * 0xC2B2AE3D27D4EB4Full;
        h ^= ((uint64_t)(uint32_t)k.c + 0x165667B1ull) * 0x9E3779B97F4A7C15ull + (h << 6);
        h ^= ((uint64_t)(uint32_t)k.d + 0x27D4EB2Full) * 0xC2B2AE3D27D4EB4Full + (h >> 3);
        return (size_t)h;
    }
};

class LfqSbCache {
public:
    static LfqSbCache &instance()
    {
        static LfqSbCache c;
        return c;
    }
    void publish(std::vector<std::pair<SbKey, int>> &items)
    {
        std::lock_guard<std::mutex> lk(m_);
        if (map_.size() + items.size() > ((size_t)1 << 18)) {
            map_.clear();
        }
        map_.reserve(map_.size() + items.size());
        for (auto &it : items) {
            map_.emplace(it.first, it.second);
        }
    }
    bool lookup(const SbKey &k, int *sb)
    {
        std::lock_guard<std::mutex> lk(m_);
        return lookup_locked(k, sb);
    }
    template <typename F>
    void with_lock(F f)
    {
        std::lock_guard<std::mutex> lk(m_);
        f();
    }
    bool lookup_locked(const SbKey &k, int *sb)
    {
        auto it = map_.find(k);
        if (it == map_.end()) {
            return false;
        }
        *sb = it->second;
        return true;
    }

private:
    std::mutex m_;
    std::unordered_map<SbKey, int, SbKeyHash> map_;
};

}

void lfq_sb_precompute(const int32_t *tuples, int64_t n)
{
    std::vector<std::pair<SbKey, int>> items;
    items.reserve((size_t)std::max<int64_t>(n, 0));
    for (int64_t i = 0; i < n; i++) {
        const int32_t *t = tuples + 4 * i;
        if (t[0] | t[1] | t[2] | t[3]) {
            items.push_back({SbKey{t[0], t[1], t[2], t[3]}, 0});
        }
    }
    std::sort(items.begin(), items.end(), [](const std::pair<SbKey, int> &x, const std::pair<SbKey, int> &y) {
        return (int64_t)x.first.c + x.first.d > (int64_t)y.first.c + y.first.d;
    });
    std::atomic<int64_t> next(0);
    const int64_t m = (int64_t)items.size();
    auto work = [&]() {
        for (;;) {
            const int64_t i = next.fetch_add(1);
            if (i >= m) {
                break;
            }
            const SbKey &k = items[(size_t)i].first;
            items[(size_t)i].second = lfq_sb_phred(k.a, k.b, k.c, k.d);
        }
    };
    LfqPool::instance().run(work, (int)std::min<int64_t>(LfqPool::instance().size(), m / 2));
    LfqSbCache::instance().publish(items);
}

extern "C" {

int lfq_abi_version(void) { return LFQ_ABI_VERSION; }

const char *lfq_strerror(int status)
{
    switch (status) {
    case LFQ_OK: return "ok";
    case LFQ_ERR_INVALID: return "invalid argument";
    case LFQ_ERR_NO_DEVICE: return "no usable HIP device";
    case LFQ_ERR_NOMEM: return "out of memory";
    case LFQ_ERR_CAPACITY: return "output capacity too small";
    case LFQ_ERR_UNSUPPORTED: return "unsupported option (the reference rejects it too)";
    case LFQ_ERR_HIP: return "HIP runtime error";
    default: return "unknown error";
    }
}

void lfq_conf_init(lfq_conf *c)
{
    memset(c, 0, sizeof(*c));
    c->min_bq = 6;
    c->min_alt_bq = 6;
    c->def_alt_bq = 0;
    c->min_jq = 0;
    c->min_alt_jq = 0;
    c->def_alt_jq = 0;
    c->bonf_dynamic = 1;
    c->min_cov = 1;
    c->bonf_subst = 1;
    c->sig = 0.01;
    c->flag = LFQ_USE_MQ | LFQ_USE_BAQ;
    c->num_snv_tests = 0;
    c->bonf_indel = 1;
    c->num_indel_tests = 0;
    c->flag |= LFQ_USE_IDAQ;
    c->approx_threshold_n = -1;
}

long double lfq_pvalue_from_log(double logp, int status)
{
    if (status == LFQ_PV_NONE) {
        return LDBL_MAX;
    }
    if (status == LFQ_PV_UNDERFLOW) {
        return LDBL_MIN;
    }
    errno = 0;
    feclearexcept(FE_ALL_EXCEPT);
    long double pv = expl(logp);
    const int errsv = errno;
    const bool bad = errsv || fetestexcept(FE_INVALID | FE_DIVBYZERO | FE_OVERFLOW | FE_UNDERFLOW)
                     || status == LFQ_PV_LOG_FECLAMP;
    if (bad) {
        pv = (pv < DBL_EPSILON) ? LDBL_MIN : LDBL_MAX;
    }
    return pv;
}

double lfq_fisher_exact(int n11, int n12, int n21, int n22, double *left_out, double *right_out,
                        double *two_out)
{
    HyperAcc acc;
    const int row1 = n11 + n12, col1 = n11 + n21, tot = n11 + n12 + n21 + n22;
    const int hi = (col1 < row1) ? col1 : row1;
    int lo = row1 + col1 - tot;
    if (lo < 0) {
        lo = 0;
    }
    *two_out = *left_out = *right_out = 1.;
    if (lo == hi) {
        return 1.;
    }
    const double q = hypergeom_next(n11, row1, col1, tot, acc);
    int i, j;
    double left, right;
    double p = hypergeom_next(lo, 0, 0, 0, acc);
    for (left = 0., i = lo + 1; p < 0.99999999 * q; ++i) {
        left += p;
        p = hypergeom_next(i, 0, 0, 0, acc);
    }
    --i;
    if (p < 1.00000001 * q) {
        left += p;
    } else {
        --i;
    }
    p = hypergeom_next(hi, 0, 0, 0, acc);
    for (right = 0., j = hi - 1; p < 0.99999999 * q; --j) {
        right += p;
        p = hypergeom_next(j, 0, 0, 0, acc);
    }
    ++j;
    if (p < 1.00000001 * q) {
        right += p;
    } else {
        ++j;
    }
    *two_out = left + right;
    if (*two_out > 1.) {
        *two_out = 1.;
    }
    if (abs(i - n11) < abs(j - n11)) {
        right = 1. - left + q;
    } else {
        left = 1.0 - right + q;
    }
    *left_out = left;
    *right_out = right;
    return q;
}

int lfq_sb_phred(int ref_fw, int ref_rv, int alt_fw, int alt_rv)
{
    if ((ref_fw + ref_rv) == 0 && (alt_fw == 0 || alt_rv == 0)) {
        return INT_MAX;
    }
    double l, r, two;
    (void)lfq_fisher_exact(ref_fw, ref_rv, alt_fw, alt_rv, &l, &r, &two);
    return prob_to_phred_safe(two);
}

int lfq_snvqual_thresh(float sig, int64_t bonf_subst)
{
    int t = INT_MAX;
    if (bonf_subst) {
        t = prob_to_phred(sig / (long long)bonf_subst);
        if (t < 0) {
            t = 0;
        }
    }
    return t;
}

int lfq_finalize_pvals(const lfq_conf *conf, const lfq_col_pvals *pvals, int64_t n_pvals,
                       const int32_t *coverage_plp_or_null, const uint8_t *ref_base,
                       lfq_snv_record *records, int64_t records_capacity, int64_t *n_records)
{
    if (!conf || (!pvals && n_pvals > 0) || !n_records || n_pvals < 0) {
        return LFQ_ERR_INVALID;
    }
    const bool timing = lfq_knobs().timing != 0;
    auto now = [] { return std::chrono::duration<double, std::milli>(std::chrono::steady_clock::now().time_since_epoch()).count(); };
    double tf[6] = {now(), 0, 0, 0, 0, 0};
    std::vector<int64_t> order((size_t)n_pvals);
    for (int64_t i = 0; i < n_pvals; i++) {
        order[(size_t)i] = i;
    }
    std::sort(order.begin(), order.end(), [&](int64_t a, int64_t b) { return pvals[a].col < pvals[b].col; });

    struct PvQ {
        long double pv[3];
        int qual[3];
    };
    std::vector<PvQ> pvq((size_t)n_pvals);
    {
        std::atomic<int64_t> nextp(0);
        auto workp = [&]() {
            for (;;) {
                const int64_t i0 = nextp.fetch_add(64);
                if (i0 >= n_pvals) {
                    break;
                }
                for (int64_t i = i0; i < std::min(n_pvals, i0 + 64); i++) {
                    const lfq_col_pvals &r = pvals[i];
                    for (int a = 0; a < 3; a++) {
                        pvq[(size_t)i].pv[a] = lfq_pvalue_from_log(r.logp[a], r.status[a]);
                        pvq[(size_t)i].qual[a] = (r.status[a] != LFQ_PV_NONE) ? prob_to_phred(pvq[(size_t)i].pv[a]) : 0;
                    }
                }
            }
        };
        LfqPool::instance().run(workp, n_pvals >= 256 ? std::min(LfqPool::instance().size(), 8) : 0);
    }

    tf[1] = now();
    static const char acgt[4] = {'A', 'C', 'G', 'T'};
    int64_t n_out = 0;
    for (int64_t oi = 0; oi < n_pvals; oi++) {
        const lfq_col_pvals &r = pvals[order[(size_t)oi]];
        const lfq_col_counts &cn = r.counts;
        const double bonf = (double)r.bonf;
        const long double *pv = pvq[(size_t)order[(size_t)oi]].pv;
        const int *quals = pvq[(size_t)order[(size_t)oi]].qual;
        int kmax = 0;
        for (int a = 0; a < 3; a++) {
            kmax = std::max(kmax, cn.alt_counts[a]);
        }
        bool main_ok = false;
        for (int a = 0; a < 3; a++) {
            if (cn.alt_counts[a] == kmax && kmax > 0 && r.status[a] != LFQ_PV_NONE) {
                main_ok = !(pv[a] * bonf > (double)conf->sig);
                break;
            }
        }
        if (!main_ok) {
            continue;
        }
        char refc = ref_base ? (char)ref_base[r.col] : (char)r.ref_base;
        int ref_code = -1;
        for (int x = 0; x < 4; x++) {
            if (acgt[x] == refc) {
                ref_code = x;
            }
        }
        if (ref_code < 0) {
            continue;
        }
        const int cov = coverage_plp_or_null ? coverage_plp_or_null[r.col] : cn.coverage;
        int ai = 0;
        for (int x = 0; x < 4; x++) {
            if (x == ref_code) {
                continue;
            }
            const int a = ai++;
            if (pv[a] * bonf < conf->sig) {
                if (n_out >= records_capacity) {
                    *n_records = n_out;
                    return LFQ_ERR_CAPACITY;
                }
                lfq_snv_record &o = records[n_out++];
                memset(&o, 0, sizeof(o));
                o.col = r.col;
                o.pvalue = pv[a];
                o.qual = quals[a];
                o.dp = cov;
                o.alt_raw_count = cn.alt_raw_counts[a];
                o.ref_fw = cn.ref_fw;
                o.ref_rv = cn.ref_rv;
                o.alt_fw = cn.alt_fw[a];
                o.alt_rv = cn.alt_raw_counts[a] - cn.alt_fw[a];
                o.hqa = cn.alt_counts[a];
                o.sb = 0;
                o.ref = refc;
                o.alt = acgt[x];
            }
        }
    }
    {
        const int64_t n = n_out;
        std::atomic<int64_t> next(0);
        tf[2] = now();
        LfqSbCache &cache = LfqSbCache::instance();
        tf[3] = now();
        std::vector<int64_t> miss;
        cache.with_lock([&] {
            for (int64_t i = 0; i < n; i++) {
                lfq_snv_record &o = records[i];
                if (!cache.lookup_locked(SbKey{o.ref_fw, o.ref_rv, o.alt_fw, o.alt_rv}, &o.sb)) {
                    miss.push_back(i);
                }
            }
        });
        const int64_t nm = (int64_t)miss.size();
        auto work = [&]() {
            for (;;) {
                const int64_t j = next.fetch_add(1);
                if (j >= nm) {
                    break;
                }
                lfq_snv_record &o = records[miss[(size_t)j]];
                o.sb = lfq_sb_phred(o.ref_fw, o.ref_rv, o.alt_fw, o.alt_rv);
            }
        };
        int64_t cost = 0;
        for (int64_t j = 0; j < nm; j++) {
            cost += records[miss[(size_t)j]].alt_fw + records[miss[(size_t)j]].alt_rv;
        }
        const int helpers = cost < 4000 ? 0 : (int)std::min<int64_t>(LfqPool::instance().size(), nm / 4);
        LfqPool::instance().run(work, helpers);
        tf[4] = now();
        if (timing) {
            fprintf(stderr, "[lfq timing] finalize: p-values+QUAL %.3f  records %.3f  wait for SB precompute %.3f  SB lookups %.3f ms (%ld misses of %ld)\n",
                    tf[1] - tf[0], tf[2] - tf[1], tf[3] - tf[2], tf[4] - tf[3], (long)nm, (long)n);
        }
    }
    *n_records = n_out;
    return LFQ_OK;
}

int lfq_format_snv_record(char *buf, int buflen, const char *chrom, int64_t pos0, const lfq_snv_record *rec,
                          const char *filter_or_null)
{
    const float af = rec->alt_raw_count / (float)rec->dp;
    return snprintf(buf, (size_t)buflen, "%s\t%ld\t.\t%c\t%c\t%d\t%s\tDP=%d;AF=%f;SB=%d;DP4=%d,%d,%d,%d;HQA=%d\n",
                    chrom, (long)(pos0 + 1), rec->ref, rec->alt, rec->qual,
                    filter_or_null ? filter_or_null : ".", rec->dp, af, rec->sb, rec->ref_fw, rec->ref_rv,
                    rec->alt_fw, rec->alt_rv, rec->hqa);
}

int lfq_filter_indel_records(const lfq_indel_record *recs, int64_t n, int indelqual_thresh, int apply_defaults,
                             int32_t *keep)
{
    if (n < 0 || (n > 0 && (!recs || !keep))) {
        return LFQ_ERR_INVALID;
    }
    for (int64_t i = 0; i < n; i++) {
        bool ok = true;
        if (indelqual_thresh > 0 && recs[i].qual > -1 && recs[i].qual < indelqual_thresh) {
            ok = false;
        }
        if (apply_defaults && recs[i].dp < 10) {
            ok = false;
        }
        keep[i] = ok ? 1 : 0;
    }
    return LFQ_OK;
}

int lfq_format_indel_record(char *buf, int buflen, const char *chrom, int64_t pos0, const char *ref,
                            const char *alt, int qual, int dp, float af, int sb, int ref_fw, int ref_rv,
                            int alt_fw, int alt_rv, int hrun, const char *filter_or_null)
{
    return snprintf(buf, (size_t)buflen, "%s\t%ld\t.\t%s\t%s\t%d\t%s\tDP=%d;AF=%f;SB=%d;DP4=%d,%d,%d,%d;INDEL;HRUN=%d\n",
                    chrom, (long)(pos0 + 1), ref, alt, qual, filter_or_null ? filter_or_null : ".", dp, af, sb,
                    ref_fw, ref_rv, alt_fw, alt_rv, hrun);
}

int lfq_format_plp_summary(char *buf, int buflen, const char *chrom, const lfq_plp_summary *s, int64_t col)
{
    if (!buf || buflen < 0 || !chrom || !s || col < 0 || col >= s->ncols) {
        return LFQ_ERR_INVALID;
    }
    char cons[1024];
    const int64_t k0 = s->cons_key_off[col], k1 = s->cons_key_off[col + 1];
    if (s->cons_kind[col] == 0) {
        cons[0] = (char)s->cons_nt[col];
        cons[1] = '\0';
    } else {
        if (k1 - k0 > (int64_t)sizeof(cons) - 2) {
            return LFQ_ERR_CAPACITY;
        }
        cons[0] = s->cons_kind[col] == 1 ? '+' : '-';
        memcpy(cons + 1, s->cons_key_chars + k0, (size_t)(k1 - k0));
        cons[1 + (k1 - k0)] = '\0';
    }
    const int32_t *fw = s->fw + col * 5, *rv = s->rv + col * 5;
    const int n = snprintf(buf, (size_t)buflen,
                           "%s\t%d\t%c\t%s\tA:%lu/%lu\tC:%lu/%lu\tG:%lu/%lu\tT:%lu/%lu\tN:%lu/%lu\theads:%d\ttails:%d\tins:%d\tdels:%d\thrun:%d\n",
                           chrom, (int)(s->col_pos[col] + 1), (char)s->ref_base[col], cons,
                           (unsigned long)fw[0], (unsigned long)rv[0], (unsigned long)fw[1], (unsigned long)rv[1],
                           (unsigned long)fw[2], (unsigned long)rv[2], (unsigned long)fw[3], (unsigned long)rv[3],
                           (unsigned long)fw[4], (unsigned long)rv[4], s->num_heads[col], s->num_tails[col], s->num_ins[col],
                           s->num_dels[col], s->hrun[col]);
    if (n < 0) {
        return LFQ_ERR_INVALID;
    }
    return n < buflen ? n : LFQ_ERR_CAPACITY;
}

namespace {
struct PlpText {
    char *buf;
    int64_t cap, len;
    void put(const char *s, size_t n)
    {
        if (buf && len + (int64_t)n <= cap) {
            memcpy(buf + len, s, n);
        }
        len += (int64_t)n;
    }
    void str(const char *s) { put(s, strlen(s)); }
    void num(int v)
    {
        char t[16];
        const int n = snprintf(t, sizeof(t), " %d", v);
        put(t, (size_t)n);
    }
    int finish()
    {
        if (len > INT_MAX) {
            return LFQ_ERR_CAPACITY;
        }
        if (!buf) {
            return (int)len;
        }
        if (len > cap) {
            return LFQ_ERR_CAPACITY;
        }
        buf[len] = '\0';
        return (int)len;
    }
};
}

int lfq_format_plp_quals(char *buf, int64_t buflen, const lfq_plp_quals *q, int64_t col, int flag)
{
    if (!q || col < q->col_begin || col >= q->col_begin + q->ncols || !q->nt_off || buflen < 0 || (!buf && buflen != 0)) {
        return LFQ_ERR_INVALID;
    }
    const bool use_baq = (flag & LFQ_USE_BAQ) != 0, use_sq = (flag & LFQ_USE_SQ) != 0;
    if (!q->bq || !q->mq || (use_baq && !q->baq) || (use_sq && !q->sq)) {
        return LFQ_ERR_INVALID;
    }
    PlpText T = {buf, buf ? buflen - 1 : 0, 0};
    if (buf && buflen == 0) {
        return LFQ_ERR_CAPACITY;
    }
    static const char *title[] = {"BQ", "BAQ", "MQ", "SQ"};
    const int64_t *off = q->nt_off + 5 * (col - q->col_begin);
    for (int i = 0; i < 5; i++) {
        if (off[i + 1] == off[i]) {
            continue;
        }
        for (int x = 0; x < (use_sq ? 4 : 3); x++) {
            char head[16];
            const int n = snprintf(head, sizeof(head), "  %c\t%s =\t", "ACGTN"[i], title[x]);
            T.put(head, (size_t)n);
            for (int64_t j = off[i]; j < off[i + 1]; j++) {
                int v = -1;
                if (x == 0) {
                    v = q->bq[j];
                } else if (x == 1 && use_baq) {
                    v = q->baq[j] == LFQ_Q_MISSING ? -1 : q->baq[j];
                } else if (x == 2) {
                    v = q->mq[j];
                } else if (x == 3) {
                    v = q->sq[j] == LFQ_Q_MISSING ? -1 : (q->sq[j] == 254 ? 49314 : q->sq[j]);
                }
                T.num(v);
            }
            T.str("\n");
        }
    }
    return T.finish();
}

int lfq_format_plp_indel_quals(char *buf, int64_t buflen, const lfq_indel_columns *b, int64_t col)
{
    if (!b || col < 0 || col >= b->ncols || buflen < 0 || (!buf && buflen != 0)) {
        return LFQ_ERR_INVALID;
    }
    for (int sd = 0; sd < 2; sd++) {
        const lfq_indel_side &S = b->side[sd];
        if (!S.ne_off || !S.ne_q || !S.ne_mq || !S.ev_off || !S.key_off || !S.key_chars || !S.rd_off || !S.rd_q || !S.rd_mq
            || !S.rd_aq || !S.rd_sq || !S.non_fw || !S.non_rv) {
            return LFQ_ERR_INVALID;
        }
        if (S.ne_off[col + 1] == S.ne_off[col] && S.non_fw[col] + S.non_rv[col] > 0) {
            return LFQ_ERR_INVALID;
        }
    }
    if (buf && buflen == 0) {
        return LFQ_ERR_CAPACITY;
    }
    PlpText T = {buf, buf ? buflen - 1 : 0, 0};
    for (int sd = 0; sd < 2; sd++) {
        const lfq_indel_side &S = b->side[sd];
        const char t = sd == 0 ? '+' : '-';
        char head[8];
        snprintf(head, sizeof(head), "  %c", t);
        T.str(head);
        T.str("0\tIDQ =\t");
        for (int64_t i = S.ne_off[col]; i < S.ne_off[col + 1]; i++) {
            T.num(S.ne_q[i]);
        }
        T.str("\n");
        T.str(head);
        T.str("0\tMQ =\t");
        for (int64_t i = S.ne_off[col]; i < S.ne_off[col + 1]; i++) {
            T.num(S.ne_mq[i]);
        }
        T.str("\n");
        static const char *title[2][4] = {{"IQ", "MQ", "AQ", "SQ"}, {"IDQ", "MQ", "AQ", "SQ"}};
        for (int64_t e = S.ev_off[col]; e < S.ev_off[col + 1]; e++) {
            const int16_t *arr[4] = {S.rd_q, S.rd_mq, S.rd_aq, S.rd_sq};
            for (int x = 0; x < 4; x++) {
                T.str(head);
                T.put(S.key_chars + S.key_off[e], (size_t)(S.key_off[e + 1] - S.key_off[e]));
                T.str("\t");
                T.str(title[sd][x]);
                T.str(" =\t");
                for (int64_t i = S.rd_off[e]; i < S.rd_off[e + 1]; i++) {
                    const int v = arr[x][i];
                    T.num(x == 3 && v == 32767 ? 49314 : v);
                }
                T.str("\n");
            }
        }
    }
    T.str("\n");
    return T.finish();
}

int64_t lfq_format_vcf(char *buf, int64_t buflen, const char *chrom, const int64_t *pos0_or_null,
                       const lfq_snv_record *recs, int64_t n, const uint8_t *keep_or_null,
                       const char *filter_or_null)
{
    if (n >= 256) {
        constexpr int SLOT = 320;
        std::vector<char> slots((size_t)n * SLOT);
        std::vector<int32_t> lens((size_t)n, 0);
        std::atomic<int64_t> next(0);
        std::atomic<int> bad(0);
        auto work = [&]() {
            for (;;) {
                const int64_t i0 = next.fetch_add(32);
                if (i0 >= n) {
                    break;
                }
                for (int64_t i = i0; i < std::min(n, i0 + 32); i++) {
                    if (keep_or_null && !keep_or_null[i]) {
                        continue;
                    }
                    const int64_t pos0 = pos0_or_null ? pos0_or_null[i] : recs[i].col;
                    const int len = lfq_format_snv_record(&slots[(size_t)i * SLOT], SLOT, chrom, pos0, &recs[i], filter_or_null);
                    if (len < 0 || len >= SLOT) {
                        bad.store(1);
                    }
                    lens[(size_t)i] = len;
                }
            }
        };
        LfqPool::instance().run(work, std::min(LfqPool::instance().size(), 8));
        if (!bad.load()) {
            int64_t used = 0;
            for (int64_t i = 0; i < n; i++) {
                const int len = lens[(size_t)i];
                if (buf && len > 0 && used + len <= buflen) {
                    memcpy(buf + used, &slots[(size_t)i * SLOT], (size_t)len);
                }
                used += len;
            }
            return used;
        }
    }
    int64_t used = 0;
    char line[512];
    for (int64_t i = 0; i < n; i++) {
        if (keep_or_null && !keep_or_null[i]) {
            continue;
        }
        const int64_t pos0 = pos0_or_null ? pos0_or_null[i] : recs[i].col;
        const int len = lfq_format_snv_record(line, (int)sizeof(line), chrom, pos0, &recs[i], filter_or_null);
        if (len < 0) {
            return LFQ_ERR_INVALID;
        }
        if (buf && used + len <= buflen) {
            memcpy(buf + used, line, (size_t)len);
        }
        used += len;
    }
    return used;
}

void lfq_bonf_corr(double *pvals, int64_t n, int64_t num_tests)
{
    const int64_t fac = (num_tests < 1) ? n : num_tests;
    for (int64_t i = 0; i < n; i++) {
        pvals[i] *= fac;
    }
}

void lfq_holm_bonf_corr(double *pvals, int64_t n, double alpha, int64_t num_tests)
{
    std::vector<IndexedP> ix((size_t)n);
    for (int64_t i = 0; i < n; i++) {
        ix[(size_t)i] = {pvals[i], i};
    }
    sort_indexed(ix);
    int64_t lp = (num_tests < 1) ? n : num_tests;
    double seen = n ? ix[0].p : 0.0;
    for (int64_t i = 0; i < n; i++) {
        if (eps_cmp(ix[(size_t)i].p, seen) != 0) {
            lp = (num_tests < 1) ? n - i : num_tests - i;
            seen = ix[(size_t)i].p;
        }
        const double tp = ix[(size_t)i].p * 1. / lp;
        if (eps_cmp(tp, alpha) < 0) {
            pvals[ix[(size_t)i].i] = ix[(size_t)i].p * lp;
        }
    }
}

int64_t lfq_fdr(const double *pvals, int64_t n, double alpha, int64_t num_tests, int64_t *rejected_idx)
{
    std::vector<IndexedP> ix((size_t)n);
    for (int64_t i = 0; i < n; i++) {
        ix[(size_t)i] = {pvals[i], i};
    }
    sort_indexed(ix);
    const int64_t m = (num_tests < 1) ? n : num_tests;
    int64_t nrej = 0;
    for (int64_t i = n; i > 0; i--) {
        if (ix[(size_t)(i - 1)].p < (alpha * i / (float)m)) {
            nrej = i;
            break;
        }
    }
    if (rejected_idx) {
        for (int64_t i = 0; i < nrej; i++) {
            rejected_idx[i] = ix[(size_t)i].i;
        }
    }
    return nrej;
}

double lfq_binom_cdf(int n, int k, double pr, int *status_or_null)
{
    int st = 0;
    double out = 0.0;
    if (n <= 0) {
        st = -5;
    } else if (k < 0 || k > n) {
        st = -4;
    } else if (!(pr >= 0.0 && pr <= 1.0)) {
        st = -6;
    } else if (k >= n || pr <= 0.0) {
        out = 1.0;
    } else if (pr >= 1.0) {
        out = 0.0;
    } else {
        const long double N = n, P = pr, Q = 1.0L - P, odds = P / Q;
        auto log_term = [&](int i) {
            const long double I = i;
            return lgammal(N + 1.0L) - lgammal(I + 1.0L) - lgammal(N - I + 1.0L) + I * logl(P) + (N - I) * log1pl(-P);
        };
        const int mode = (int)floorl((N + 1.0L) * P);
        if (k < mode) {
            long double t = expl(log_term(k)), sum = t;
            for (int i = k; i > 0 && t > sum * 1e-25L; i--) {
                t *= (long double)i / (N - (long double)i + 1.0L) / odds;
                sum += t;
            }
            out = (double)sum;
        } else {
            long double t = expl(log_term(k + 1)), sum = t;
            for (int i = k + 1; i < n && t > sum * 1e-25L; i++) {
                t *= (N - (long double)i) / ((long double)i + 1.0L) * odds;
                sum += t;
            }
            const long double r = 1.0L - sum;
            out = (double)(r < 0.0L ? 0.0L : r);
        }
    }
    if (status_or_null) {
        *status_or_null = st;
    }
    return st ? 0.0 : out;
}

int lfq_uniq_mtc(const int32_t *uq, int64_t n, int mtc_type, double alpha, int64_t ntests, uint8_t *pass)
{
    if ((!uq || !pass) && n > 0) {
        return LFQ_ERR_INVALID;
    }
    if (mtc_type < 1 || mtc_type > 3 || n < 0) {
        return LFQ_ERR_INVALID;
    }
    if (!ntests) {
        ntests = n;
    }
    std::vector<double> pr((size_t)n);
    for (int64_t i = 0; i < n; i++) {
        pr[(size_t)i] = phred_to_prob(uq[i] < 0 ? 0 : uq[i]);
    }
    if (mtc_type == 1) {
        lfq_bonf_corr(pr.data(), n, ntests);
    } else if (mtc_type == 2) {
        lfq_holm_bonf_corr(pr.data(), n, alpha, ntests);
    } else {
        std::vector<int64_t> idx((size_t)std::max<int64_t>(n, 1));
        const int64_t nrej = lfq_fdr(pr.data(), n, alpha, ntests, idx.data());
        for (int64_t i = 0; i < nrej; i++) {
            pr[(size_t)idx[(size_t)i]] = -1;
        }
    }
    for (int64_t i = 0; i < n; i++) {
        pass[i] = pr[(size_t)i] > alpha ? 0 : 1;
    }
    return LFQ_OK;
}

int lfq_filter_records(const lfq_snv_record *records, int64_t n, int snvqual_thresh, int apply_defaults,
                       uint8_t *keep)
{
    if ((!records && n > 0) || !keep || n < 0) {
        return LFQ_ERR_INVALID;
    }
    for (int64_t i = 0; i < n; i++) {
        keep[i] = 1;
    }
    if (apply_defaults && n > 0) {
        const double alpha = 0.001;
        std::vector<double> sbp((size_t)n);
        std::vector<int64_t> rej((size_t)n);
        for (int64_t i = 0; i < n; i++) {
            sbp[(size_t)i] = phred_to_prob(records[i].sb);
        }
        const int64_t nrej = lfq_fdr(sbp.data(), n, alpha, n, rej.data());
        for (int64_t i = 0; i < nrej; i++) {
            const lfq_snv_record &r = records[rej[(size_t)i]];
            const float ratio = std::max(r.alt_fw, r.alt_rv) / (float)(r.alt_fw + r.alt_rv);
            if (ratio > 0.85) {
                keep[rej[(size_t)i]] = 0;
            }
        }
        for (int64_t i = 0; i < n; i++) {
            if (records[i].dp < 10) {
                keep[i] = 0;
            }
        }
    }
    if (snvqual_thresh) {
        for (int64_t i = 0; i < n; i++) {
            if (records[i].qual > -1 && records[i].qual < snvqual_thresh) {
                keep[i] = 0;
            }
        }
    }
    return LFQ_OK;
}

#define LFQ_HOST_TRY(expr) do { const int rc_ = (expr); if (rc_ != LFQ_OK) return rc_; } while (0)
void lfq_filter_conf_init(lfq_filter_conf *c)
{
    if (!c) {
        return;
    }
    memset(c, 0, sizeof(*c));
    c->dp_min = c->dp_max = -1;
    c->af_min = c->af_max = -1;
    c->sb_alpha = c->snvqual_alpha = c->indelqual_alpha = 0.01;
}

void lfq_filter_conf_defaults(lfq_filter_conf *c)
{
    if (!c) {
        return;
    }
    if (c->sb_mtc_type == LFQ_MTC_NONE && !c->sb_thresh) {
        c->sb_mtc_type = LFQ_MTC_FDR;
        c->sb_alpha = 0.001;
    }
    if (c->dp_min < 0) {
        c->dp_min = 10;
    }
}

namespace {

int filter_mtc(std::vector<double> &p, int mtc_type, double alpha, int64_t *ntests, std::vector<uint8_t> &signif)
{
    const int64_t n = (int64_t)p.size();
    signif.assign((size_t)n, 0);
    if (n <= 0) {
        return LFQ_OK;
    }
    if (!*ntests) {
        *ntests = n;
    }
    if (mtc_type == LFQ_MTC_BONF) {
        lfq_bonf_corr(p.data(), n, *ntests);
    } else if (mtc_type == LFQ_MTC_HOLMBONF) {
        lfq_holm_bonf_corr(p.data(), n, alpha, *ntests);
    } else if (mtc_type == LFQ_MTC_FDR) {
        std::vector<int64_t> rej((size_t)n);
        const int64_t nrej = lfq_fdr(p.data(), n, alpha, *ntests, rej.data());
        std::fill(p.begin(), p.end(), DBL_MAX);
        for (int64_t i = 0; i < nrej; i++) {
            p[(size_t)rej[(size_t)i]] = -1;
        }
    } else {
        return LFQ_ERR_INVALID;
    }
    for (int64_t i = 0; i < n; i++) {
        signif[(size_t)i] = p[(size_t)i] < alpha ? 1 : 0;
    }
    return LFQ_OK;
}

bool alt_mostly_on_one_strand(const lfq_filter_var &v)
{
    const float ratio = std::max(v.alt_fw, v.alt_rv) / (float)(v.alt_fw + v.alt_rv);
    return ratio > 0.85;
}

const char *mtc_name(int t)
{
    return t == LFQ_MTC_BONF ? "bonf" : (t == LFQ_MTC_HOLMBONF ? "holmbonf" : (t == LFQ_MTC_FDR ? "fdr" : "none"));
}

}

int lfq_filter_vars(lfq_filter_conf *c, const lfq_filter_var *vars, int64_t n, uint32_t *fail)
{
    if (!c || n < 0 || (n > 0 && (!vars || !fail))) {
        return LFQ_ERR_INVALID;
    }
    if ((c->only_indels && c->only_snvs) || (c->dp_max > 0 && c->dp_max < c->dp_min)
        || (c->af_max > 0 && c->af_max < c->af_min) || c->af_max > 1.0
        || (c->sb_thresh && c->sb_mtc_type != LFQ_MTC_NONE) || (c->snvqual_thresh && c->snvqual_mtc_type != LFQ_MTC_NONE)
        || (c->indelqual_thresh && c->indelqual_mtc_type != LFQ_MTC_NONE)) {
        return LFQ_ERR_INVALID;
    }
    std::vector<uint8_t> sb_sig, iq_sig, sq_sig;
    std::vector<int64_t> sb_ix, iq_ix, sq_ix;
    errno = 0;
    auto qual_of = [](const lfq_filter_var &v) { return v.qual == -1 ? INT_MAX : v.qual; };
    if (c->sb_mtc_type != LFQ_MTC_NONE) {
        std::vector<double> p;
        for (int64_t i = 0; i < n; i++) {
            if (!c->sb_incl_indels && vars[i].is_indel) {
                continue;
            }
            p.push_back(phred_to_prob(vars[i].sb));
            sb_ix.push_back(i);
        }
        LFQ_HOST_TRY(filter_mtc(p, c->sb_mtc_type, c->sb_alpha, &c->sb_ntests, sb_sig));
    }
    if (c->indelqual_mtc_type != LFQ_MTC_NONE) {
        std::vector<double> p;
        for (int64_t i = 0; i < n; i++) {
            if (vars[i].is_indel) {
                p.push_back(phred_to_prob(qual_of(vars[i])));
                iq_ix.push_back(i);
            }
        }
        LFQ_HOST_TRY(filter_mtc(p, c->indelqual_mtc_type, c->indelqual_alpha, &c->indelqual_ntests, iq_sig));
    }
    if (c->snvqual_mtc_type != LFQ_MTC_NONE) {
        std::vector<double> p;
        for (int64_t i = 0; i < n; i++) {
            if (!vars[i].is_indel) {
                p.push_back(phred_to_prob(qual_of(vars[i])));
                sq_ix.push_back(i);
            }
        }
        LFQ_HOST_TRY(filter_mtc(p, c->snvqual_mtc_type, c->snvqual_alpha, &c->snvqual_ntests, sq_sig));
    }
    const bool af_off = errno == ERANGE;
    for (int64_t i = 0; i < n; i++) {
        const lfq_filter_var &v = vars[i];
        uint32_t f = 0;
        if ((c->only_snvs && v.is_indel) || (c->only_indels && !v.is_indel)) {
            fail[i] = LFQ_FILT_DROPPED;
            continue;
        }
        if (!af_off && c->af_min > 0.0 && v.af < c->af_min) f |= LFQ_FILT_AF_MIN;
        if (!af_off && c->af_max > 0.0 && v.af > c->af_max) f |= LFQ_FILT_AF_MAX;
        if (c->dp_min > 0 && v.dp < c->dp_min) f |= LFQ_FILT_DP_MIN;
        if (c->dp_max > 0 && v.dp > c->dp_max) f |= LFQ_FILT_DP_MAX;
        if (!v.is_indel && c->snvqual_thresh && v.qual > -1 && v.qual < c->snvqual_thresh) f |= LFQ_FILT_SNVQUAL;
        if (v.is_indel && c->indelqual_thresh && v.qual > -1 && v.qual < c->indelqual_thresh) f |= LFQ_FILT_INDELQUAL;
        if (c->sb_thresh && (!v.is_indel || c->sb_incl_indels) && v.sb > c->sb_thresh
            && (c->sb_no_compound || alt_mostly_on_one_strand(v))) {
            f |= LFQ_FILT_SB;
        }
        fail[i] = f;
    }
    for (size_t k = 0; k < sq_ix.size(); k++) {
        if (!sq_sig[k] && fail[sq_ix[k]] != LFQ_FILT_DROPPED) fail[sq_ix[k]] |= LFQ_FILT_SNVQUAL;
    }
    for (size_t k = 0; k < iq_ix.size(); k++) {
        if (!iq_sig[k] && fail[iq_ix[k]] != LFQ_FILT_DROPPED) fail[iq_ix[k]] |= LFQ_FILT_INDELQUAL;
    }
    for (size_t k = 0; k < sb_ix.size(); k++) {
        const int64_t i = sb_ix[k];
        if (sb_sig[k] && fail[i] != LFQ_FILT_DROPPED && (c->sb_no_compound || alt_mostly_on_one_strand(vars[i]))) {
            fail[i] |= LFQ_FILT_SB;
        }
    }
    return LFQ_OK;
}

int lfq_filter_id(const lfq_filter_conf *c, uint32_t bit, char *buf, int buflen)
{
    if (!c || !buf || buflen < 1) {
        return 0;
    }
    int k = 0;
    buf[0] = 0;
    switch (bit) {
    case LFQ_FILT_AF_MIN: if (c->af_min > 0) k = snprintf(buf, (size_t)buflen, "min_af_%f", c->af_min); break;
    case LFQ_FILT_AF_MAX: if (c->af_max > 0) k = snprintf(buf, (size_t)buflen, "max_af_%f", c->af_max); break;
    case LFQ_FILT_DP_MIN: if (c->dp_min > 0) k = snprintf(buf, (size_t)buflen, "min_dp_%d", c->dp_min); break;
    case LFQ_FILT_DP_MAX: if (c->dp_max > 0) k = snprintf(buf, (size_t)buflen, "max_dp_%d", c->dp_max); break;
    case LFQ_FILT_SB:
        if (c->sb_thresh > 0) k = snprintf(buf, (size_t)buflen, "max_sb_%d", c->sb_thresh);
        else if (c->sb_mtc_type != LFQ_MTC_NONE) k = snprintf(buf, (size_t)buflen, "sb_%s", mtc_name(c->sb_mtc_type));
        break;
    case LFQ_FILT_SNVQUAL:
        if (c->snvqual_thresh > 0) k = snprintf(buf, (size_t)buflen, "min_snvqual_%d", c->snvqual_thresh);
        else if (c->snvqual_mtc_type != LFQ_MTC_NONE) k = snprintf(buf, (size_t)buflen, "snvqual_%s", mtc_name(c->snvqual_mtc_type));
        break;
    case LFQ_FILT_INDELQUAL:
        if (c->indelqual_thresh > 0) k = snprintf(buf, (size_t)buflen, "min_indelqual_%d", c->indelqual_thresh);
        else if (c->indelqual_mtc_type != LFQ_MTC_NONE) k = snprintf(buf, (size_t)buflen, "indelqual_%s", mtc_name(c->indelqual_mtc_type));
        break;
    default: break;
    }
    return k < 0 ? 0 : (k >= buflen ? buflen - 1 : k);
}

int lfq_filter_string(const lfq_filter_conf *c, uint32_t f, char *buf, int buflen)
{
    if (!c || !buf || buflen < 5) {
        return 0;
    }
    static const uint32_t order[] = {LFQ_FILT_AF_MIN, LFQ_FILT_AF_MAX, LFQ_FILT_DP_MIN, LFQ_FILT_DP_MAX, LFQ_FILT_SNVQUAL,
                                     LFQ_FILT_INDELQUAL, LFQ_FILT_SB};
    int used = 0;
    buf[0] = 0;
    for (uint32_t b : order) {
        if (!(f & b)) {
            continue;
        }
        char id[96];
        const int k = lfq_filter_id(c, b, id, (int)sizeof(id));
        if (k <= 0 || used + k + 2 > buflen) {
            continue;
        }
        if (used) {
            buf[used++] = ';';
        }
        memcpy(buf + used, id, (size_t)k + 1);
        used += k;
    }
    if (!used) {
        used = snprintf(buf, (size_t)buflen, "PASS");
    }
    return used;
}

int lfq_filter_header_lines(const lfq_filter_conf *c, char *buf, int buflen)
{
    if (!c || !buf || buflen < 1) {
        return 0;
    }
    std::string s;
    char id[96], line[512];
    auto add = [&](const char *fmt, auto... a) {
        snprintf(line, sizeof(line), fmt, a...);
        s += line;
    };
    if (lfq_filter_id(c, LFQ_FILT_AF_MIN, id, sizeof(id))) add("##FILTER=<ID=%s,Description=\"Minimum allele frequency %f\">\n", id, c->af_min);
    if (lfq_filter_id(c, LFQ_FILT_AF_MAX, id, sizeof(id))) add("##FILTER=<ID=%s,Description=\"Maximum allele frequency %f\">\n", id, c->af_max);
    if (lfq_filter_id(c, LFQ_FILT_DP_MIN, id, sizeof(id))) add("##FILTER=<ID=%s,Description=\"Minimum Coverage %d\">\n", id, c->dp_min);
    if (lfq_filter_id(c, LFQ_FILT_DP_MAX, id, sizeof(id))) add("##FILTER=<ID=%s,Description=\"Maximum Coverage %d\">\n", id, c->dp_max);
    if (lfq_filter_id(c, LFQ_FILT_SB, id, sizeof(id))) {
        if (c->sb_thresh > 0) add("##FILTER=<ID=%s,Description=\"Maximum Strand-Bias Phred %d\">\n", id, c->sb_thresh);
        else add("##FILTER=<ID=%s,Description=\"Strand-Bias Multiple Testing Correction: %s corr. pvalue > %f\">\n", id, mtc_name(c->sb_mtc_type), c->sb_alpha);
    }
    if (lfq_filter_id(c, LFQ_FILT_SNVQUAL, id, sizeof(id))) {
        if (c->snvqual_thresh > 0) add("##FILTER=<ID=%s,Description=\"Minimum SNV Quality (Phred) %d\">\n", id, c->snvqual_thresh);
        else add("##FILTER=<ID=%s,Description=\"SNV Quality Multiple Testing Correction: %s corr. pvalue < %f\">\n", id, mtc_name(c->snvqual_mtc_type), c->snvqual_alpha);
    }
    if (lfq_filter_id(c, LFQ_FILT_INDELQUAL, id, sizeof(id))) {
        if (c->indelqual_thresh > 0) add("##FILTER=<ID=%s,Description=\"Minimum Indel Quality (Phred) %d\">\n", id, c->indelqual_thresh);
        else add("##FILTER=<ID=%s,Description=\"Indel Quality Multiple Testing Correction: %s corr. pvalue < %f\">\n", id, mtc_name(c->indelqual_mtc_type), c->indelqual_alpha);
    }
    const int k = (int)std::min<size_t>(s.size(), (size_t)buflen - 1);
    memcpy(buf, s.data(), (size_t)k);
    buf[k] = 0;
    return (int)s.size();
}

static float af_through_text(float af)
{
    char t[64];
    snprintf(t, sizeof(t), "%f", af);
    return strtof(t, nullptr);
}

void lfq_filter_var_from_snv(const lfq_snv_record *r, lfq_filter_var *o)
{
    memset(o, 0, sizeof(*o));
    o->is_indel = 0;
    o->qual = r->qual;
    o->dp = r->dp;
    o->sb = r->sb;
    o->alt_fw = r->alt_fw;
    o->alt_rv = r->alt_rv;
    o->af = af_through_text(r->alt_raw_count / (float)r->dp);
}

void lfq_filter_var_from_indel(const lfq_indel_record *r, lfq_filter_var *o)
{
    memset(o, 0, sizeof(*o));
    o->is_indel = 1;
    o->qual = r->qual;
    o->dp = r->dp;
    o->sb = r->sb;
    o->alt_fw = r->alt_fw;
    o->alt_rv = r->alt_rv;
    o->af = af_through_text(r->af);
}

}
```

lofreq_amd/csrc/lfq_internal.h:

```cpp
#ifndef LFQ_INTERNAL_H
#define LFQ_INTERNAL_H

#include <stdint.h>

#include "lofreq_amd.h"

struct LfqLuts {
    double bq[256];
    double baq[256];
    double mq[256];
    double sq[256];
};

struct LfqParams {
    int32_t min_bq4;
    int32_t min_alt_bq4;
    int32_t def_alt_bq;
    int32_t general;
    double jq_reject_above;
    double alt_jq_reject_above;
    double def_alt_jp;
    int32_t min_cov;
    int32_t use_baq, use_mq, use_sq;
    int32_t bonf_dynamic;
    int64_t bonf_base;
    int32_t bonf_step;
    int32_t bonf_reset_first;
    double sig;
    double prune_slack;
    int32_t seg_max;
    int32_t seg_max_mid;
    int32_t seg_budget_mid, seg_budget_big;
    int32_t phase1_chunks;
    const float *detlim_af;
    int32_t lazy_strand;
    int32_t approx_n;
    int32_t sparse_counts;
    int32_t scan_gate_maxk;
    double bound_p_lo;
};

struct LfqTracksDev {
    const uint8_t *nt, *bq, *baq, *mq, *sq;
    const uint64_t *col_off;
    const uint8_t *ref_base;
    const int32_t *coverage_plp, *num_bases;
    int64_t ncols;
    int32_t nt_packed;
    int32_t pad_;
};

struct LfqEntry {
    uint64_t off0;
    int32_t n_obs;
    int32_t col;
    int32_t prefix;
    int32_t kmax;
    int16_t median_ref_bq;
    uint8_t ref_code;
    uint8_t pad_;
    int32_t pad2_;
};

#define LFQ_FLAG_NLO_SHIFT 3
#define LFQ_FLAG_DROPPED (1u << LFQ_FLAG_NLO_SHIFT)

#if defined(__HIPCC__)
__host__ __device__
#endif
static inline int64_t lfq_bonf_of_prefix(const LfqParams &P, int prefix)
{
    int64_t bonf = P.bonf_base;
    if (P.bonf_dynamic) {
        bonf = ((P.bonf_reset_first && P.bonf_base == 1) ? 0 : P.bonf_base) + (int64_t)P.bonf_step * prefix;
    }
    return bonf;
}

struct LfqSegCell {
    double v;
    int32_t e;
    int32_t pad_;
};

struct LfqLong {
    uint64_t off0;
    int64_t bonf;
    int64_t cell0;
    int32_t n_obs, col;
    int32_t K;
    int32_t n_seg;
    int32_t ch_begin;
    int32_t phase1;
    uint32_t uf_mask;
    int32_t force_fe;
    int32_t pruned;
    int32_t rows;
    int16_t median_ref_bq;
    uint8_t ref_code;
    uint8_t pad0_;
    int32_t pad1_;
    double uf_bound[3];
    int64_t pad_[4];
};

#define LFQ_SEG_MAX 8
#include "lfq_seg_items.h"
#define LFQ_SEG_CLASSES 5
#define LFQ_SEG_MIN_CHUNKS 16
#ifndef LFQ_SEG_MIN_CHUNKS_SHORT
#define LFQ_SEG_MIN_CHUNKS_SHORT 4
#endif
#define LFQ_SEG_SHORT_BELOW 48
#define LFQ_PHASE1_CHUNKS 8
#define LFQ_SEG_BUDGET 4096
#define LFQ_SPLIT_MAX_K 2016

#if defined(__HIPCC__)
__host__ __device__
#endif
static inline int lfq_khist_thr(int f)
{
    return f == 0 ? 5 : f == 1 ? 7 : f == 2 ? 9 : f == 3 ? 11 : f == 4 ? 15 : f == 5 ? 23 : 31;
}
static inline int lfq_screen_kreg(int kreg_hint)
{
    const int want = kreg_hint > 0 ? kreg_hint : 8;
    return want <= 6 ? 6 : want <= 8 ? 8 : want <= 10 ? 10 : want <= 12 ? 12 : want <= 16 ? 16 : want <= 24 ? 24 : want <= 32 ? 32 : 0;
}

struct LfqWork {
    int32_t *tested_prefix;
    LfqEntry *entries;
    int32_t *gcounters;
    int32_t *counters;
    int32_t *block_sums;
    LfqLong *longs;
    int32_t *unsplit;
    LfqSegCell *pool;
    int32_t long_cap;
    int32_t pool_cells;
};

#define LFQ_MID_K 64
#define LFQ_BIG_K 250
#define LFQ_NCOUNTERS 320
#define LFQ_MAX_SEGMENTS 1
#define LFQ_GC_PVALS 0
#define LFQ_GC_OVERFLOW 1
#define LFQ_GC_TESTED 2
#define LFQ_GC_MAXDEPTH 3
#define LFQ_GC_CELLS 8
#define LFQ_GC_ROWS 10
#define LFQ_GC_APPROX_PRUNED 13
#define LFQ_GC_SCREEN_RETRY 12
#define LFQ_CNT_TESTED 0
#define LFQ_CNT_BIG 1
#define LFQ_CNT_MID 2
#define LFQ_CNT_LIGHT 3
#define LFQ_CNT_LIST_LIGHT 31
#define LFQ_CNT_HEAD 4
#define LFQ_CNT_CARRY_IN 15
#define LFQ_CNT_HEAD_LIGHT 12
#define LFQ_CNT_HEAD_MID 13
#define LFQ_CNT_UNSPLIT 5
#define LFQ_CNT_HEAD_PREP 6
#define LFQ_CNT_POOL 7
#define LFQ_CNT_HEAD_COMB 24
#define LFQ_CNT_HEAD_FOLD 48
#define LFQ_CNT_KLE7 26
#define LFQ_CNT_KLE15 27
#define LFQ_CNT_KLE31 28
#define LFQ_CNT_XHEAD 64
#define LFQ_CNT_KHIST 40
#define LFQ_NKHIST 7
#define LFQ_CNT_LONG0 16
#define LFQ_CNT_SEG_ITEMS 22

#define LFQ_SEQ_LETTERS "ACGTN=MRSVWYHKDB"
#if defined(__HIPCC__)
__host__ __device__
#endif
static inline char lfq_seq_letter(unsigned code)
{
    return code > 15u ? 'N' : LFQ_SEQ_LETTERS[code];
}

#if defined(__HIPCC__)
__host__ __device__ inline __attribute__((always_inline))
#else
static inline
#endif
int lfq_cigar_peek_indel(const uint32_t *cg, int nc, int k)
{
    int indel = 0;
    if (k + 1 < nc) {
        const int op2 = cg[k + 1] & 0xf, l2 = cg[k + 1] >> 4;
        if (op2 == 2) {
            indel = -l2;
        } else if (op2 == 1) {
            indel = l2;
        } else if (op2 == 6 && k + 2 < nc) {
            int l3 = 0;
            for (int kk = k + 2; kk < nc; ++kk) {
                const int o3 = cg[kk] & 0xf;
                if (o3 == 1) {
                    l3 += cg[kk] >> 4;
                } else if (o3 == 2 || o3 == 0 || o3 == 3 || o3 == 7 || o3 == 8) {
                    break;
                }
            }
            indel = l3 > 0 ? l3 : 0;
        }
    }
    return indel;
}

struct LfqKnobs {
    int timing;
    int single_stream;
    int no_sb_precompute;
    int debug_sync;
    int skip_light, skip_mid, skip_big;
    int light_kernel;
    int screen_rounds;
    int seg_max;
    int seg_max_mid;
    int split_pool_cells;
    long count_multi_below;
    int big_on_side;
    int baq_one_variant;
    int pileup_tiles;
    long host_loop_threads;
    long count_lpg4_below, count_lpg8_below;
    long host_spin_us;
    int sync_upload;
    int host_threads;
    long host_par_min;
    int local_world_size;
    int indel_host_pack;
    int pileup_atomic;
    int baq_lds;
    long baq_scratch_mb;
    int private_stream;
    int bound_gate;
    int scan_gate;
    int dp_wg_waves;
};
const LfqKnobs &lfq_knobs(void);
unsigned lfq_cpu_budget(void);

void lfq_sb_precompute(const int32_t *tuples, int64_t n);

static inline int64_t lfq_al(int64_t b)
{
    return (b + 255) / 256 * 256;
}

struct LfqReadsDev {
    int64_t n_reads;
    const int32_t *pos;
    const int64_t *cigar_off, *seq_off;
    const uint32_t *cigar;
    const uint8_t *seq, *qual;
    const uint8_t *baq;
    const uint8_t *mapq, *reverse;
    const uint8_t *ref;
    int64_t ref_len;
    const uint8_t *sq;
    const uint8_t *bi, *bd;
    const uint8_t *tag_flags;
    const int32_t *pmax_end;
    const int32_t *read_idx;
};

struct LfqBaqGeom {
    int32_t xb, l_ref;
    int32_t bw;
};
struct LfqBaqRead {
    int32_t pos;
    int32_t l_qseq;
    int32_t xb, l_ref;
    int32_t bw;
    int32_t n_cigar;
    int64_t cigar_off;
};

struct LfqBaqArgs : LfqReadsDev {
    const LfqBaqGeom *geom;
    uint8_t *lb_out;
    double *scratch;
    int32_t *expect;
    uint8_t *tmp8;
    const float *qual2prob;
    int32_t rows, W;
    int32_t baq_extended;
    float par_d, par_e;
    int32_t first_read;
    const int32_t *order;
    int32_t max_lref;
    int32_t lds_rows;
    uint8_t *ai_out, *ad_out;
    uint8_t *tagfl_out;
    int32_t *itab;
    double *terms;
    uint8_t *nflag;
};
#define LFQ_BAQ_MAX_INDELS 64
#define LFQ_BAQ_MAX_TERMS 1024
#define LFQ_BAQ_LDS_CELLS 51
#define LFQ_BAQ_BAND8_CELLS 57
#define LFQ_BAQ_LDS_BAND 15
#define LFQ_BAQ_LDS_MAX_LREF 300
int lfq_launch_baq(const LfqBaqArgs &a, int64_t n_launch, int lds, void *stream, int nmode = 0);

struct LfqPileupArgs : LfqReadsDev {
    int64_t begin, width;
    int32_t min_plp_bq;
    int32_t *cov, *nb, *cursor;
    const int32_t *col_index;
    const uint64_t *col_off;
    uint8_t *t_nt, *t_bq, *t_baq, *t_mq;
    uint8_t *t_sq;
};
int lfq_launch_pileup_count(const LfqPileupArgs &a, void *stream);
int lfq_launch_pileup_columns(const LfqPileupArgs &a, int scatter, void *stream);

struct LfqPlpIndelArgs : LfqReadsDev {
    int64_t begin, width;
    int32_t min_plp_idq;
    int32_t *cov, *tails, *non_indels, *n_ins, *n_dels, *non_ins_fw, *non_del_fw;
    int32_t *ne_qsum[2];
    const int64_t *ne_off[2];
    int32_t *cursor[2];
    int16_t *ne_q[2], *ne_mq[2];
};
int lfq_launch_plp_indel(const LfqPlpIndelArgs &a, int scatter, void *stream);
int lfq_launch_plp_indel_columns(const LfqPlpIndelArgs &a, int scatter, void *stream);
struct LfqSitesArgs : LfqReadsDev {
    int64_t n_sites;
    const int64_t *site_pos;
    int32_t min_plp_bq;
    const int64_t *key_off;
    const uint8_t *key_chars, *key_del;
    int32_t *counts;
    int64_t *win;
    const uint64_t *col_off;
    uint8_t *t_nt, *t_bq, *t_baq, *t_mq, *t_sq;
};
int lfq_launch_pileup_sites(const LfqSitesArgs &a, int scatter, void *stream);
struct LfqSummaryArgs : LfqReadsDev {
    int64_t n_cols;
    const int64_t *col_pos;
    int32_t min_plp_bq;
    const double *incr;
    int32_t *fw, *rv;
    int32_t *heads, *tails;
    uint8_t *cons_nt;
    uint8_t *ordered;
};
int lfq_launch_plp_summary(const LfqSummaryArgs &a, void *stream);
struct LfqPlpGroupArgs {
    const uint8_t *nt, *bq, *baq, *mq, *sq;
    const uint64_t *col_off;
    int64_t n_cols;
    uint64_t in_shift;
    uint8_t *o_bq, *o_baq, *o_mq, *o_sq;
    int64_t *nt_off;
};
int lfq_launch_plp_group(const LfqPlpGroupArgs &a, void *stream);
int64_t lfq_keep_compact_scratch(int64_t n);
int lfq_launch_keep_compact(const uint8_t *keep, const int32_t *pos, int64_t n, void *scratch, int32_t *kept_idx,
                            int32_t *kept_pos, int32_t *kept_pmax, void *stream);
struct LfqIdqArgs : LfqReadsDev {
    int64_t n_bases;
    const uint8_t *tab;
    int64_t tab_begin, tab_end;
    uint32_t ins_byte, del_byte;
    uint8_t *bi_out, *bd_out;
};
int lfq_launch_idq_table(const uint8_t *ref, int64_t ref_len, int64_t tab_begin, int64_t tab_end, uint8_t *tab, void *stream);
int lfq_launch_idq_fill(const LfqIdqArgs &a, void *stream);
uint8_t lfq_idq_ref_byte(const char *ref, int64_t ref_len, int64_t x);
uint8_t lfq_idq_host_byte(const char *ref, int64_t ref_len, int64_t pos, const uint32_t *cigar, int n_cigar, int64_t qpos);
int lfq_launch_flag_merge(uint8_t *fl, const uint8_t *tag, int64_t n, void *stream);
int lfq_launch_skip_columns(int32_t *nb, const uint8_t *skip, int64_t n, void *stream);
int lfq_launch_pack_nt(const uint8_t *nt_bytes, uint8_t *nt_packed, int64_t n_obs, void *stream);
#define LFQ_PLP_COMPACT_TILE 4096
int lfq_launch_plp_compact_sums(const int32_t *cov, const int32_t *nb, int64_t width, int64_t *tile_cols, uint64_t *tile_obs,
                                int32_t *tile_max, int64_t *totals, void *stream);
int lfq_launch_plp_compact_apply(const int32_t *cov, const int32_t *nb, int64_t width, int64_t begin, const uint8_t *ref,
                                 int64_t ref_len, const int64_t *tile_cols, const uint64_t *tile_obs, const int64_t *totals,
                                 int32_t *col_index, uint64_t *col_off, uint8_t *ref_base, int32_t *cov_c, int32_t *nb_c,
                                 int64_t *col_pos, void *stream);
int lfq_launch_gather2(const uint8_t *a, const uint8_t *b, const int64_t *idx, int64_t n, uint8_t *oa, uint8_t *ob, void *stream);

struct LfqIndelTestDesc {
    int64_t out_off;
    int64_t ne_off;
    int64_t rd_begin;
    int32_t ne_len, rd_len;
    int32_t me_begin, me_len;
    int32_t side, pad_;
};
struct LfqIndelPackArgs {
    const LfqIndelTestDesc *tests;
    int64_t n_tests;
    const int16_t *ne_q[2], *ne_mq[2];
    const int16_t *rd_q[2], *rd_aq[2], *rd_mq[2], *rd_sq[2];
    int32_t use_mq, use_sq, use_aq, pad_;
    uint8_t *nt, *bq, *baq, *mq, *sq;
};
int lfq_launch_indel_pack(const LfqIndelPackArgs &a, void *stream);

#define LFQ_DBL_EPSILON 2.220446049250313e-16
#define LFQ_SRCQ_LDS_CELLS 768
#define LFQ_SRCQ_NA 0
#define LFQ_SRCQ_PERFECT 1
#define LFQ_SRCQ_VALUE 2
struct LfqSrcqArgs : LfqReadsDev {
    const uint8_t *ign;
    int32_t nonmatch_qual, min_bq;
    double *scratch;
    int64_t scratch_cells;
    double *prob;
    uint8_t *status;
};
int lfq_launch_srcq(const LfqSrcqArgs &a, const LfqLuts *d_luts, int n_blocks, void *stream);
int lfq_launch_pileup_scatter(const LfqPileupArgs &a, void *stream);

int lfq_launch_strand_heavy(const LfqTracksDev &t, const LfqWork &w, lfq_col_counts *d_counts, int32_t *tuples_mapped,
                            int32_t *n_mapped, int cap_entries, int min_alt, void *stream);
int lfq_launch_strand_pvals(const LfqTracksDev &t, lfq_col_pvals *d_pvals, const int32_t *d_n_pvals, int64_t cap, int n_blocks,
                            void *stream);
int lfq_launch_gather_heavy(const LfqWork &w, const lfq_col_counts *d_counts, int32_t *tuples_mapped,
                            int32_t *n_mapped, int cap_entries, int min_alt, void *stream);
int lfq_launch_maxdepth(const LfqTracksDev &t, int32_t *d_gcounters, void *stream);
int lfq_launch_ntcount(const LfqTracksDev &t, int32_t *d_out, void *stream);
bool lfq_count_is_shallow(const LfqTracksDev &t, const LfqParams &p, int64_t max_col_obs);
int lfq_launch_count(const LfqTracksDev &t, int64_t c0, int64_t c1, const LfqParams &p, const LfqLuts *d_luts,
                     lfq_col_counts *d_counts, uint8_t *d_flags, int64_t max_col_obs, void *stream, bool shallow_half_cu = false);
bool lfq_count_is_lean(const LfqTracksDev &t, const LfqParams &p, int64_t max_col_obs);
int lfq_launch_scan(const LfqTracksDev &t, int64_t c0, int64_t c1, const LfqParams &p, uint8_t *d_flags,
                    const lfq_col_counts *d_counts, const LfqWork &w, void *stream, bool relist = false);
int lfq_launch_approx_gate(const LfqTracksDev &t, const LfqParams &p, const LfqLuts *d_luts, const lfq_col_counts *d_counts,
                           const LfqWork &w, int64_t ncols_seg, double *d_mu, uint8_t *d_flags, void *stream);
int lfq_launch_dp_light(const LfqTracksDev &t, const LfqParams &p, const LfqLuts *d_luts,
                        const lfq_col_counts *d_counts, const LfqWork &w, lfq_col_pvals *d_pvals,
                        int64_t pvals_capacity, int n_waves, void *stream);
int lfq_launch_dp_quad(const LfqTracksDev &t, const LfqParams &p, const LfqLuts *d_luts,
                       const lfq_col_counts *d_counts, const LfqWork &w, uint8_t *d_retry, lfq_col_pvals *d_pvals,
                       int64_t pvals_capacity, int n_waves, int kreg_hint, void *stream, int phase = 0);
int lfq_launch_dp_mid(const LfqTracksDev &t, const LfqParams &p, const LfqLuts *d_luts,
                      const lfq_col_counts *d_counts, const LfqWork &w, lfq_col_pvals *d_pvals,
                      int64_t pvals_capacity, int n_waves, int wg_waves, void *stream);
int lfq_launch_dp_big(const LfqTracksDev &t, const LfqParams &p, const LfqLuts *d_luts,
                      const lfq_col_counts *d_counts, const LfqWork &w, lfq_col_pvals *d_pvals,
                      int64_t pvals_capacity, double *d_scratch, int64_t scratch_doubles_per_block,
                      int n_blocks, void *stream);
int lfq_launch_dp_big_prep(const LfqTracksDev &t, const LfqParams &p, const LfqLuts *d_luts,
                           const lfq_col_counts *d_counts, const LfqWork &w, lfq_col_pvals *d_pvals,
                           int64_t pvals_capacity, int n_blocks, void *stream);
int lfq_launch_dp_seg(int mode, const LfqTracksDev &t, const LfqParams &p, const LfqLuts *d_luts,
                      const LfqWork &w, int n_waves, int wg_waves, void *stream);
int lfq_launch_dp_combine(int mode, const LfqParams &p, const lfq_col_counts *d_counts, const LfqWork &w,
                          lfq_col_pvals *d_pvals, int64_t pvals_capacity, int n_blocks, void *stream);
int lfq_launch_synth(const struct lfq_synth_spec *d_spec_host, int64_t col_begin, int64_t ncols,
                     uint8_t *d_nt, uint8_t *d_bq, uint8_t *d_baq, uint8_t *d_mq, uint64_t *d_col_off,
                     uint8_t *d_ref_base, int nt_packed, void *stream);

#endif
```

Measured before the change: 388.5 million.

## Share host pool across concurrent jobs and let collector take over SB precompute

Replaces the single-job host thread pool, where a second caller ran alone when the pool was busy, with a queue-based pool that lets concurrent jobs share the worker threads. Adds an LfqSbJob state machine so the strand-bias precompute can be started by the leader thread or taken over by the finishing thread when it collects, instead of the finisher blocking on a pending counter. The aim is to stop the SB precompute from running single-threaded while finalize work holds the pool, and to cut finisher wait time. It adds locking complexity and possible races between arm, lead and collect.

```diff
diff --git a/lofreq_amd/csrc/lfq_api.hip b/lofreq_amd/csrc/lfq_api.hip
--- a/lofreq_amd/csrc/lfq_api.hip
+++ b/lofreq_amd/csrc/lfq_api.hip
@@ -1,5 +1,6 @@
 #include "lfq_bound.h"
 #include "lfq_ctx.h"
+#include "lfq_pool.h"
 
 namespace {
 
@@ -251,10 +252,16 @@
     L->mq[0] = 0.5;
 }
 
+int64_t sb_tuples_ready(const lfq_ctx *c)
+{
+    return 3 * std::min<int64_t>(std::max<int64_t>(*(volatile int32_t *)c->h_nheavy, 0), c->heavy_cap);
+}
+
 void leader_main(lfq_ctx *c)
 {
     (void)hipSetDevice(c->device);
     for (;;) {
+        uint64_t seq;
         {
             std::unique_lock<std::mutex> lk(*c->lm);
             c->lcv->wait(lk, [&] { return c->leader_go > 0 || c->leader_stop; });
@@ -262,17 +269,27 @@
                 return;
             }
             c->leader_go--;
-        }
-        int64_t n = 0;
-        if (hipEventSynchronize(c->ev_heavy) == hipSuccess) {
-            n = std::min<int64_t>(std::max<int64_t>(*(volatile int32_t *)c->h_nheavy, 0), c->heavy_cap);
-        }
-        lfq_sb_precompute(c->h_tuples, 3 * n);
-        {
-            std::lock_guard<std::mutex> lk(*c->lm);
-            c->sb_pending--;
-        }
-        c->lcv->notify_all();
+            seq = c->sb_job->seq_locked();
+        }
+        const int64_t n = hipEventSynchronize(c->ev_heavy) == hipSuccess ? sb_tuples_ready(c) : 0;
+        const double t_ev = lfq_now_ms();
+        const bool led = c->sb_job->lead(seq, c->h_tuples, n);
+        if (lfq_timing_on) {
+            int64_t items;
+            {
+                std::lock_guard<std::mutex> lk(*c->lm);
+                items = c->sb_job->n_items_locked();
+            }
+            fprintf(stderr, "[lfq timing] leader %p: ev_heavy at %.3f  precompute %.3f ms  %ld items  %s\n", (void *)c, t_ev,
+                    lfq_now_ms() - t_ev, (long)items, led ? "started here, shared pool" : "taken by the collect");
+        }
+    }
+}
+
+void lfq_sb_collect(lfq_ctx *c)
+{
+    if (c->sb_job) {
+        c->sb_job->collect(c->h_tuples, sb_tuples_ready(c));
     }
 }
 
@@ -394,6 +411,7 @@
             *c->h_nheavy = 0;
             c->lm = new std::mutex();
             c->lcv = new std::condition_variable();
+            c->sb_job = new LfqSbJob(c->lm, c->lcv, &lfq_host_pool(), &lfq_sb_cache());
             c->leader = new std::thread(leader_main, c);
         }
     }
@@ -423,9 +441,11 @@
         c->lcv->notify_all();
         c->leader->join();
         delete c->leader;
+        delete c->sb_job;
         delete c->lm;
         delete c->lcv;
         c->leader = nullptr;
+        c->sb_job = nullptr;
     }
     if (c) {
         if (c->d_plp_in) (void)hipFree(c->d_plp_in);
@@ -691,7 +711,7 @@
             {
                 std::lock_guard<std::mutex> lk(*c->lm);
                 c->leader_go++;
-                c->sb_pending++;
+                c->sb_job->arm_locked();
             }
             c->lcv->notify_all();
             return LFQ_OK;
@@ -1185,10 +1205,7 @@
                               hipMemcpyDeviceToHost));
     }
     tp[2] = lfq_now_ms();
-    if (c->leader) {
-        std::unique_lock<std::mutex> lk(*c->lm);
-        c->lcv->wait(lk, [&] { return c->sb_pending == 0 || c->leader_stop; });
-    }
+    lfq_sb_collect(c);
     int rc = lfq_finalize_pvals(conf, h_pv.data(), st.n_pvals, nullptr, c->sub_ref_host, records, records_capacity,
                                 n_records);
     tp[3] = lfq_now_ms();
@@ -1224,10 +1241,7 @@
     LFQ_TRY_HIP(hipSetDevice(c->device));
     lfq_batch_stats st;
     LFQ_TRY(lfq_batch_finish(c, &st));
-    if (c->leader) {
-        std::unique_lock<std::mutex> lk(*c->lm);
-        c->lcv->wait(lk, [&] { return c->sb_pending == 0 || c->leader_stop; });
-    }
+    lfq_sb_collect(c);
     if (stats_out) {
         *stats_out = st;
     }
diff --git a/lofreq_amd/csrc/lfq_ctx.h b/lofreq_amd/csrc/lfq_ctx.h
--- a/lofreq_amd/csrc/lfq_ctx.h
+++ b/lofreq_amd/csrc/lfq_ctx.h
@@ -376,7 +376,7 @@
     int own_streams;
     int kreg_hint, kreg_hint_indel;
     int cur_indel_mode;
-    int sb_pending;
+    class LfqSbJob *sb_job;
     struct { void *p; size_t cap; int used; } pin_pool[LFQ_PIN_SLOTS];
     struct LfqViterbiState *vit;
     struct LfqBamState *bam;
diff --git a/lofreq_amd/csrc/lfq_host.cpp b/lofreq_amd/csrc/lfq_host.cpp
--- a/lofreq_amd/csrc/lfq_host.cpp
+++ b/lofreq_amd/csrc/lfq_host.cpp
@@ -21,6 +21,7 @@
 
 #include "lofreq_amd.h"
 #include "lfq_internal.h"
+#include "lfq_pool.h"
 
 #ifdef LFQ_TUNE
 #define LFQ_TUNE_I(name, dflt) geti(name, dflt)
@@ -206,45 +207,9 @@
     return budget;
 }
 
-namespace {
-
-class LfqPool {
-public:
-    static LfqPool &instance()
-    {
-        static LfqPool p;
-        return p;
-    }
-    int size() const { return (int)threads_.size(); }
-    void run(const std::function<void()> &f, int helpers)
-    {
-        helpers = std::max(0, std::min(helpers, size()));
-        if (helpers == 0) {
-            f();
-            return;
-        }
-        std::unique_lock<std::mutex> call_lock(call_m_, std::try_to_lock);
-        if (!call_lock.owns_lock()) {
-            f();
-            return;
-        }
-        {
-            std::lock_guard<std::mutex> lk(m_);
-            job_ = &f;
-            want_ = helpers;
-            pending_ = helpers;
-            generation_++;
-        }
-        cv_start_.notify_all();
-        f();
-        std::unique_lock<std::mutex> lk(m_);
-        cv_done_.wait(lk, [&] { return pending_ == 0; });
-        job_ = nullptr;
-    }
-
-private:
-    LfqPool()
-    {
+LfqPool &lfq_host_pool(void)
+{
+    static LfqPool p([] {
         unsigned hw = lfq_cpu_budget();
         const LfqKnobs &kn = lfq_knobs();
         hw = std::max(1u, hw / (unsigned)kn.local_world_size);
@@ -252,147 +217,15 @@
         if (kn.host_threads >= 0) {
             n = std::max(0, std::min(kn.host_threads - 1, 255));
         }
-        for (int i = 0; i < n; i++) {
-            threads_.emplace_back([this, i] { loop(i); });
-        }
-    }
-    ~LfqPool()
-    {
-        {
-            std::lock_guard<std::mutex> lk(m_);
-            stop_ = true;
-            generation_++;
-        }
-        cv_start_.notify_all();
-        for (auto &t : threads_) {
-            t.join();
-        }
-    }
-    void loop(int idx)
-    {
-        int seen = 0;
-        for (;;) {
-            const std::function<void()> *job = nullptr;
-            {
-                std::unique_lock<std::mutex> lk(m_);
-                cv_start_.wait(lk, [&] { return generation_ != seen; });
-                seen = generation_;
-                if (stop_) {
-                    return;
-                }
-                if (idx >= want_) {
-                    continue;
-                }
-                job = job_;
-            }
-            (*job)();
-            {
-                std::lock_guard<std::mutex> lk(m_);
-                pending_--;
-            }
-            cv_done_.notify_one();
-        }
-    }
-    std::vector<std::thread> threads_;
-    std::mutex m_, call_m_;
-    std::condition_variable cv_start_, cv_done_;
-    const std::function<void()> *job_ = nullptr;
-    int generation_ = 0, want_ = 0, pending_ = 0;
-    bool stop_ = false;
-};
-
-}
-
-namespace {
-
-struct SbKey {
-    int32_t a, b, c, d;
-    bool operator==(const SbKey &o) const { return a == o.a && b == o.b && c == o.c && d == o.d; }
-};
-struct SbKeyHash {
-    size_t operator()(const SbKey &k) const
-    {
-        uint64_t h = (uint64_t)(uint32_t)k.a * 0x9E3779B97F4A7C15ull;
-        h ^= ((uint64_t)(uint32_t)k.b + 0x7F4A7C15ull) * 0xC2B2AE3D27D4EB4Full;
-        h ^= ((uint64_t)(uint32_t)k.c + 0x165667B1ull) * 0x9E3779B97F4A7C15ull + (h << 6);
-        h ^= ((uint64_t)(uint32_t)k.d + 0x27D4EB2Full) * 0xC2B2AE3D27D4EB4Full + (h >> 3);
-        return (size_t)h;
-    }
-};
-
-class LfqSbCache {
-public:
-    static LfqSbCache &instance()
-    {
-        static LfqSbCache c;
-        return c;
-    }
-    void publish(std::vector<std::pair<SbKey, int>> &items)
-    {
-        std::lock_guard<std::mutex> lk(m_);
-        if (map_.size() + items.size() > ((size_t)1 << 18)) {
-            map_.clear();
-        }
-        map_.reserve(map_.size() + items.size());
-        for (auto &it : items) {
-            map_.emplace(it.first, it.second);
-        }
-    }
-    bool lookup(const SbKey &k, int *sb)
-    {
-        std::lock_guard<std::mutex> lk(m_);
-        return lookup_locked(k, sb);
-    }
-    template <typename F>
-    void with_lock(F f)
-    {
-        std::lock_guard<std::mutex> lk(m_);
-        f();
-    }
-    bool lookup_locked(const SbKey &k, int *sb)
-    {
-        auto it = map_.find(k);
-        if (it == map_.end()) {
-            return false;
-        }
-        *sb = it->second;
-        return true;
-    }
-
-private:
-    std::mutex m_;
-    std::unordered_map<SbKey, int, SbKeyHash> map_;
-};
-
-}
-
-void lfq_sb_precompute(const int32_t *tuples, int64_t n)
-{
-    std::vector<std::pair<SbKey, int>> items;
-    items.reserve((size_t)std::max<int64_t>(n, 0));
-    for (int64_t i = 0; i < n; i++) {
-        const int32_t *t = tuples + 4 * i;
-        if (t[0] | t[1] | t[2] | t[3]) {
-            items.push_back({SbKey{t[0], t[1], t[2], t[3]}, 0});
-        }
-    }
-    std::sort(items.begin(), items.end(), [](const std::pair<SbKey, int> &x, const std::pair<SbKey, int> &y) {
-        return (int64_t)x.first.c + x.first.d > (int64_t)y.first.c + y.first.d;
-    });
-    std::atomic<int64_t> next(0);
-    const int64_t m = (int64_t)items.size();
-    auto work = [&]() {
-        for (;;) {
-            const int64_t i = next.fetch_add(1);
-            if (i >= m) {
-                break;
-            }
-            const SbKey &k = items[(size_t)i].first;
-            items[(size_t)i].second = lfq_sb_phred(k.a, k.b, k.c, k.d);
-        }
-    };
-    LfqPool::instance().run(work, (int)std::min<int64_t>(LfqPool::instance().size(), m / 2));
-    LfqSbCache::instance().publish(items);
+        return n;
+    }());
+    return p;
+}
+
+LfqSbCache &lfq_sb_cache(void)
+{
+    static LfqSbCache c;
+    return c;
 }
 
 extern "C" {
@@ -567,7 +400,7 @@
                 }
             }
         };
-        LfqPool::instance().run(workp, n_pvals >= 256 ? std::min(LfqPool::instance().size(), 8) : 0);
+        lfq_host_pool().run(workp, n_pvals >= 256 ? std::min(lfq_host_pool().size(), 8) : 0);
     }
 
     tf[1] = now();
@@ -637,13 +470,13 @@
         const int64_t n = n_out;
         std::atomic<int64_t> next(0);
         tf[2] = now();
-        LfqSbCache &cache = LfqSbCache::instance();
+        LfqSbCache &cache = lfq_sb_cache();
         tf[3] = now();
         std::vector<int64_t> miss;
         cache.with_lock([&] {
             for (int64_t i = 0; i < n; i++) {
                 lfq_snv_record &o = records[i];
-                if (!cache.lookup_locked(SbKey{o.ref_fw, o.ref_rv, o.alt_fw, o.alt_rv}, &o.sb)) {
+                if (!cache.lookup_locked(LfqSbKey{o.ref_fw, o.ref_rv, o.alt_fw, o.alt_rv}, &o.sb)) {
                     miss.push_back(i);
                 }
             }
@@ -663,8 +496,8 @@
         for (int64_t j = 0; j < nm; j++) {
             cost += records[miss[(size_t)j]].alt_fw + records[miss[(size_t)j]].alt_rv;
         }
-        const int helpers = cost < 4000 ? 0 : (int)std::min<int64_t>(LfqPool::instance().size(), nm / 4);
-        LfqPool::instance().run(work, helpers);
+        const int helpers = cost < 4000 ? 0 : (int)std::min<int64_t>(lfq_host_pool().size(), nm / 4);
+        lfq_host_pool().run(work, helpers);
         tf[4] = now();
         if (timing) {
             fprintf(stderr, "[lfq timing] finalize: p-values+QUAL %.3f  records %.3f  wait for SB precompute %.3f  SB lookups %.3f ms (%ld misses of %ld)\n",
@@ -908,7 +741,7 @@
                 }
             }
         };
-        LfqPool::instance().run(work, std::min(LfqPool::instance().size(), 8));
+        lfq_host_pool().run(work, std::min(lfq_host_pool().size(), 8));
         if (!bad.load()) {
             int64_t used = 0;
             for (int64_t i = 0; i < n; i++) {
diff --git a/lofreq_amd/csrc/lfq_internal.h b/lofreq_amd/csrc/lfq_internal.h
--- a/lofreq_amd/csrc/lfq_internal.h
+++ b/lofreq_amd/csrc/lfq_internal.h
@@ -250,7 +250,10 @@
 const LfqKnobs &lfq_knobs(void);
 unsigned lfq_cpu_budget(void);
 
-void lfq_sb_precompute(const int32_t *tuples, int64_t n);
+class LfqPool;
+class LfqSbCache;
+LfqPool &lfq_host_pool(void);
+LfqSbCache &lfq_sb_cache(void);
 
 static inline int64_t lfq_al(int64_t b)
 {
diff --git a/lofreq_amd/csrc/lfq_pool.h b/lofreq_amd/csrc/lfq_pool.h
--- /dev/null
+++ b/lofreq_amd/csrc/lfq_pool.h
@@ -0,0 +1,297 @@
+#ifndef LFQ_POOL_H
+#define LFQ_POOL_H
+
+#include <stdint.h>
+
+#include <algorithm>
+#include <atomic>
+#include <condition_variable>
+#include <functional>
+#include <memory>
+#include <mutex>
+#include <thread>
+#include <unordered_map>
+#include <utility>
+#include <vector>
+
+#include "lofreq_amd.h"
+
+class LfqPool {
+public:
+    explicit LfqPool(int n_threads)
+    {
+        for (int i = 0; i < n_threads; i++) {
+            threads_.emplace_back([this] { loop(); });
+        }
+    }
+    ~LfqPool()
+    {
+        {
+            std::lock_guard<std::mutex> lk(m_);
+            stop_ = true;
+        }
+        cv_start_.notify_all();
+        for (auto &t : threads_) {
+            t.join();
+        }
+    }
+    LfqPool(const LfqPool &) = delete;
+    LfqPool &operator=(const LfqPool &) = delete;
+
+    int size() const { return (int)threads_.size(); }
+
+    void run(const std::function<void()> &f, int helpers)
+    {
+        helpers = std::max(0, std::min(helpers, size()));
+        if (helpers == 0) {
+            f();
+            return;
+        }
+        Job j;
+        j.f = &f;
+        j.want = helpers;
+        {
+            std::lock_guard<std::mutex> lk(m_);
+            *tail_ = &j;
+            tail_ = &j.next;
+        }
+        cv_start_.notify_all();
+        f();
+        std::unique_lock<std::mutex> lk(m_);
+        if (j.want > 0) {
+            unlink(&j);
+        }
+        cv_done_.wait(lk, [&] { return j.inside == 0; });
+    }
+
+private:
+    struct Job {
+        const std::function<void()> *f = nullptr;
+        int want = 0;
+        int inside = 0;
+        Job *next = nullptr;
+    };
+    void unlink(Job *j)
+    {
+        Job **pp = &head_;
+        while (*pp != j) {
+            pp = &(*pp)->next;
+        }
+        *pp = j->next;
+        if (tail_ == &j->next) {
+            tail_ = pp;
+        }
+        j->next = nullptr;
+        j->want = 0;
+    }
+    void loop()
+    {
+        std::unique_lock<std::mutex> lk(m_);
+        for (;;) {
+            cv_start_.wait(lk, [&] { return stop_ || head_ != nullptr; });
+            if (stop_) {
+                return;
+            }
+            Job *j = head_;
+            j->inside++;
+            if (--j->want == 0) {
+                unlink(j);
+            }
+            lk.unlock();
+            (*j->f)();
+            lk.lock();
+            if (--j->inside == 0) {
+                cv_done_.notify_all();
+            }
+        }
+    }
+    std::vector<std::thread> threads_;
+    std::mutex m_;
+    std::condition_variable cv_start_, cv_done_;
+    Job *head_ = nullptr, **tail_ = &head_;
+    bool stop_ = false;
+};
+
+struct LfqSbKey {
+    int32_t a, b, c, d;
+    bool operator==(const LfqSbKey &o) const { return a == o.a && b == o.b && c == o.c && d == o.d; }
+};
+struct LfqSbKeyHash {
+    size_t operator()(const LfqSbKey &k) const
+    {
+        uint64_t h = (uint64_t)(uint32_t)k.a * 0x9E3779B97F4A7C15ull;
+        h ^= ((uint64_t)(uint32_t)k.b + 0x7F4A7C15ull) * 0xC2B2AE3D27D4EB4Full;
+        h ^= ((uint64_t)(uint32_t)k.c + 0x165667B1ull) * 0x9E3779B97F4A7C15ull + (h << 6);
+        h ^= ((uint64_t)(uint32_t)k.d + 0x27D4EB2Full) * 0xC2B2AE3D27D4EB4Full + (h >> 3);
+        return (size_t)h;
+    }
+};
+
+class LfqSbCache {
+public:
+    void publish(const std::vector<std::pair<LfqSbKey, int>> &items)
+    {
+        std::lock_guard<std::mutex> lk(m_);
+        if (map_.size() + items.size() > ((size_t)1 << 18)) {
+            map_.clear();
+        }
+        map_.reserve(map_.size() + items.size());
+        for (auto &it : items) {
+            map_.emplace(it.first, it.second);
+        }
+    }
+    bool lookup(const LfqSbKey &k, int *sb)
+    {
+        std::lock_guard<std::mutex> lk(m_);
+        return lookup_locked(k, sb);
+    }
+    template <typename F>
+    void with_lock(F f)
+    {
+        std::lock_guard<std::mutex> lk(m_);
+        f();
+    }
+    bool lookup_locked(const LfqSbKey &k, int *sb)
+    {
+        auto it = map_.find(k);
+        if (it == map_.end()) {
+            return false;
+        }
+        *sb = it->second;
+        return true;
+    }
+
+private:
+    std::mutex m_;
+    std::unordered_map<LfqSbKey, int, LfqSbKeyHash> map_;
+};
+
+class LfqSbJob {
+public:
+    typedef int (*SbFn)(int, int, int, int);
+    LfqSbJob(std::mutex *lm, std::condition_variable *lcv, LfqPool *pool, LfqSbCache *cache, SbFn fn = lfq_sb_phred)
+        : lm_(lm), lcv_(lcv), pool_(pool), cache_(cache), fn_(fn)
+    {
+    }
+    uint64_t arm_locked()
+    {
+        state_ = ARMED;
+        return ++seq_;
+    }
+    uint64_t seq_locked() const { return seq_; }
+
+    bool lead(uint64_t seq, const int32_t *tuples, int64_t n)
+    {
+        {
+            std::lock_guard<std::mutex> lk(*lm_);
+            if (state_ != ARMED || seq_ != seq) {
+                return false;
+            }
+            state_ = BUILDING;
+        }
+        start(tuples, n);
+        return true;
+    }
+    int collect(const int32_t *tuples, int64_t n)
+    {
+        int how;
+        std::shared_ptr<Run> r;
+        {
+            std::unique_lock<std::mutex> lk(*lm_);
+            if (state_ == IDLE || state_ == DONE) {
+                return 0;
+            }
+            how = state_ == ARMED ? 2 : 1;
+            if (state_ == ARMED) {
+                state_ = BUILDING;
+            } else {
+                lcv_->wait(lk, [&] { return state_ != BUILDING; });
+                r = run_;
+            }
+        }
+        if (how == 2) {
+            start(tuples, n);
+        } else {
+            drain(*r);
+        }
+        std::unique_lock<std::mutex> lk(*lm_);
+        lcv_->wait(lk, [&] { return state_ == DONE; });
+        return how;
+    }
+    int64_t n_items_locked() const { return run_ ? run_->m : 0; }
+
+private:
+    enum State { IDLE, ARMED, BUILDING, RUNNING, DONE };
+    struct Run {
+        std::vector<std::pair<LfqSbKey, int>> items;
+        int64_t m = 0;
+        std::atomic<int64_t> next{0};
+        int64_t n_done = 0;
+    };
+    void start(const int32_t *tuples, int64_t n)
+    {
+        std::shared_ptr<Run> r = std::make_shared<Run>();
+        r->items.reserve((size_t)std::max<int64_t>(n, 0));
+        for (int64_t i = 0; i < n; i++) {
+            const int32_t *t = tuples + 4 * i;
+            if (t[0] | t[1] | t[2] | t[3]) {
+                r->items.push_back({LfqSbKey{t[0], t[1], t[2], t[3]}, 0});
+            }
+        }
+        std::sort(r->items.begin(), r->items.end(), [](const std::pair<LfqSbKey, int> &x, const std::pair<LfqSbKey, int> &y) {
+            return (int64_t)x.first.c + x.first.d > (int64_t)y.first.c + y.first.d;
+        });
+        r->m = (int64_t)r->items.size();
+        {
+            std::lock_guard<std::mutex> lk(*lm_);
+            run_ = r;
+            state_ = r->m > 0 ? RUNNING : DONE;
+        }
+        lcv_->notify_all();
+        if (r->m > 0) {
+            const std::function<void()> work = [this, r] { drain(*r); };
+            pool_->run(work, (int)std::min<int64_t>(pool_->size(), r->m / 2));
+        }
+    }
+    void drain(Run &r)
+    {
+        int64_t mine = 0;
+        for (;;) {
+            const int64_t i = r.next.fetch_add(1, std::memory_order_relaxed);
+            if (i >= r.m) {
+                break;
+            }
+            const LfqSbKey &k = r.items[(size_t)i].first;
+            r.items[(size_t)i].second = fn_(k.a, k.b, k.c, k.d);
+            mine++;
+        }
+        if (mine == 0) {
+            return;
+        }
+        bool last;
+        {
+            std::lock_guard<std::mutex> lk(*lm_);
+            r.n_done += mine;
+            last = r.n_done == r.m;
+            if (last) {
+                cache_->publish(r.items);
+                if (state_ == RUNNING && run_.get() == &r) {
+                    state_ = DONE;
+                }
+            }
+        }
+        if (last) {
+            lcv_->notify_all();
+        }
+    }
+    std::mutex *lm_;
+    std::condition_variable *lcv_;
+    LfqPool *pool_;
+    LfqSbCache *cache_;
+    SbFn fn_;
+    State state_ = IDLE;
+    uint64_t seq_ = 0;
+    std::shared_ptr<Run> run_;
+};
+
+#endif
diff --git a/lofreq_amd/csrc/lfq_pool_check.cpp b/lofreq_amd/csrc/lfq_pool_check.cpp
--- /dev/null
+++ b/lofreq_amd/csrc/lfq_pool_check.cpp
@@ -0,0 +1,672 @@
+#include <stdio.h>
+#include <stdlib.h>
+#include <string.h>
+
+#include <algorithm>
+#include <atomic>
+#include <chrono>
+#include <condition_variable>
+#include <functional>
+#include <mutex>
+#include <set>
+#include <thread>
+#include <vector>
+
+#include "lofreq_amd.h"
+#include "lfq_pool.h"
+
+namespace {
+
+#define CHECK(cond, ...)                                  \
+    do {                                                  \
+        if (!(cond)) {                                    \
+            fprintf(stderr, "FAILED %s:%d: ", __FILE__, __LINE__); \
+            fprintf(stderr, __VA_ARGS__);                 \
+            fprintf(stderr, "\n");                        \
+            exit(1);                                      \
+        }                                                 \
+    } while (0)
+
+double now_ms()
+{
+    return std::chrono::duration<double, std::milli>(std::chrono::steady_clock::now().time_since_epoch()).count();
+}
+
+void small_tuple(int i, int32_t *t)
+{
+    t[0] = 100 + i % 50;
+    t[1] = 90 + i % 37;
+    t[2] = 1 + i % 23;
+    t[3] = (i * 7) % 19;
+}
+
+struct Latch {
+    std::mutex m;
+    std::condition_variable cv;
+    bool open = false;
+    void wait()
+    {
+        std::unique_lock<std::mutex> lk(m);
+        cv.wait(lk, [&] { return open; });
+    }
+    void release()
+    {
+        {
+            std::lock_guard<std::mutex> lk(m);
+            open = true;
+        }
+        cv.notify_all();
+    }
+};
+
+int mode_callers()
+{
+    const int P = 4;
+    const int sizes[4] = {0, 1, 7, 1000};
+    std::vector<int> serial(1000);
+    for (int i = 0; i < 1000; i++) {
+        int32_t t[4];
+        small_tuple(i, t);
+        serial[(size_t)i] = lfq_sb_phred(t[0], t[1], t[2], t[3]);
+    }
+    LfqPool pool(P);
+    CHECK(pool.size() == P, "pool size %d", pool.size());
+    long jobs = 0;
+    for (int n_callers : {1, 2, 8}) {
+        for (int helpers = 0; helpers <= P; helpers++) {
+            for (int si = 0; si < 4; si++) {
+                const int n = sizes[si];
+                std::vector<std::vector<std::atomic<int>>> runs((size_t)n_callers);
+                std::vector<std::vector<int>> vals((size_t)n_callers);
+                for (int c = 0; c < n_callers; c++) {
+                    runs[(size_t)c] = std::vector<std::atomic<int>>((size_t)n);
+                    vals[(size_t)c].assign((size_t)n, -12345);
+                }
+                std::atomic<int> at_start(0);
+                std::vector<std::thread> th;
+                for (int c = 0; c < n_callers; c++) {
+                    th.emplace_back([&, c] {
+                        std::atomic<int> next(0);
+                        const std::function<void()> work = [&] {
+                            for (;;) {
+                                const int i = next.fetch_add(1);
+                                if (i >= n) {
+                                    break;
+                                }
+                                int32_t t[4];
+                                small_tuple(i, t);
+                                vals[(size_t)c][(size_t)i] = lfq_sb_phred(t[0], t[1], t[2], t[3]);
+                                runs[(size_t)c][(size_t)i].fetch_add(1);
+                            }
+                        };
+                        at_start.fetch_add(1);
+                        while (at_start.load() < n_callers) {
+                            std::this_thread::yield();
+                        }
+                        pool.run(work, helpers);
+                    });
+                }
+                for (auto &t : th) {
+                    t.join();
+                }
+                for (int c = 0; c < n_callers; c++) {
+                    for (int i = 0; i < n; i++) {
+                        CHECK(runs[(size_t)c][(size_t)i].load() == 1, "callers %d helpers %d items %d: item %d of caller %d ran %d times",
+                              n_callers, helpers, n, i, c, runs[(size_t)c][(size_t)i].load());
+                        CHECK(vals[(size_t)c][(size_t)i] == serial[(size_t)i], "callers %d helpers %d items %d: item %d is %d, serial %d",
+                              n_callers, helpers, n, i, vals[(size_t)c][(size_t)i], serial[(size_t)i]);
+                    }
+                }
+                jobs += n_callers;
+            }
+        }
+    }
+    printf("ok callers: %ld jobs\n", jobs);
+    return 0;
+}
+
+int mode_noalone()
+{
+    LfqPool pool(4);
+    std::mutex m;
+    std::condition_variable cv;
+    std::set<std::thread::id> in_a, in_b;
+    Latch latch;
+    bool a_returned = false;
+
+    const std::function<void()> fa = [&] {
+        {
+            std::lock_guard<std::mutex> lk(m);
+            in_a.insert(std::this_thread::get_id());
+        }
+        cv.notify_all();
+        latch.wait();
+    };
+    std::thread::id id_a, id_b;
+    std::thread ta([&] {
+        id_a = std::this_thread::get_id();
+        pool.run(fa, 1);
+        std::lock_guard<std::mutex> lk(m);
+        a_returned = true;
+    });
+    {
+        std::unique_lock<std::mutex> lk(m);
+        cv.wait(lk, [&] { return in_a.size() == 2; });
+    }
+    const std::function<void()> fb = [&] {
+        std::unique_lock<std::mutex> lk(m);
+        in_b.insert(std::this_thread::get_id());
+        cv.notify_all();
+        cv.wait_until(lk, std::chrono::system_clock::now() + std::chrono::seconds(20), [&] { return in_b.size() >= 2; });
+    };
+    std::thread tb([&] {
+        id_b = std::this_thread::get_id();
+        pool.run(fb, 2);
+    });
+    tb.join();
+    {
+        std::lock_guard<std::mutex> lk(m);
+        CHECK(!a_returned, "A ended before its latch opened");
+        CHECK(in_b.count(id_b) == 1, "B's caller did not work in its own job");
+        size_t pool_threads = 0;
+        for (const auto &id : in_b) {
+            CHECK(id != id_a && in_a.count(id) == 0, "a thread that sits in A entered B");
+            pool_threads += id != id_b;
+        }
+        CHECK(pool_threads >= 1, "B ran alone: no pool thread entered it while A was active");
+        CHECK(pool_threads <= 2, "B wanted 2 helpers and got %zu", pool_threads);
+        CHECK(in_a.size() == 2 && in_a.count(id_a) == 1, "A: %zu threads", in_a.size());
+    }
+    latch.release();
+    ta.join();
+    CHECK(a_returned, "A did not end");
+    printf("ok noalone: %zu pool thread(s) entered B beside A\n", in_b.size() - 1);
+    return 0;
+}
+
+constexpr int SB_N = 96;
+constexpr int SB_BASE = 1000;
+std::atomic<int> g_calls[SB_N];
+Latch *g_hold = nullptr;
+std::atomic<int> g_holding(0);
+
+int counted_sb(int a, int b, int c, int d)
+{
+    const int i = a - SB_BASE;
+    if (i >= 0 && i < SB_N) {
+        g_calls[i].fetch_add(1);
+        if (i == 0 && g_hold) {
+            g_holding.store(1);
+            g_hold->wait();
+        }
+    }
+    return lfq_sb_phred(a, b, c, d);
+}
+
+void sb_tuples(std::vector<int32_t> &t, int round)
+{
+    t.assign(4 * (size_t)(SB_N + 8), 0);
+    for (int i = 0; i < SB_N; i++) {
+        t[4 * (size_t)i + 0] = SB_BASE + i;
+        t[4 * (size_t)i + 1] = 900 + round % 97;
+        t[4 * (size_t)i + 2] = 20 + (i * 5) % 61;
+        t[4 * (size_t)i + 3] = 10 + (i * 3 + round) % 43;
+    }
+}
+
+void sb_expect_all_once(const std::vector<int32_t> &t, LfqSbCache &cache, const char *what, int round)
+{
+    for (int i = 0; i < SB_N; i++) {
+        CHECK(g_calls[i].load() == 1, "%s, round %d: item %d computed %d times", what, round, i, g_calls[i].load());
+        const int32_t *q = &t[4 * (size_t)i];
+        int sb = -1;
+        CHECK(cache.lookup(LfqSbKey{q[0], q[1], q[2], q[3]}, &sb), "%s, round %d: key %d is not in the cache", what, round, i);
+        CHECK(sb == lfq_sb_phred(q[0], q[1], q[2], q[3]), "%s, round %d: key %d holds %d", what, round, i, sb);
+    }
+    for (int i = 0; i < SB_N; i++) {
+        g_calls[i].store(0);
+    }
+}
+
+struct MiniCtx {
+    std::mutex lm;
+    std::condition_variable lcv;
+    int leader_go = 0, leader_stop = 0;
+    LfqSbJob *job = nullptr;
+    const std::vector<int32_t> *tuples = nullptr;
+    std::atomic<int> led{0}, passed{0};
+};
+
+void mini_leader(MiniCtx *c)
+{
+    for (;;) {
+        uint64_t seq;
+        {
+            std::unique_lock<std::mutex> lk(c->lm);
+            c->lcv.wait(lk, [&] { return c->leader_go > 0 || c->leader_stop; });
+            if (c->leader_stop) {
+                return;
+            }
+            c->leader_go--;
+            seq = c->job->seq_locked();
+        }
+        if (c->job->lead(seq, c->tuples->data(), (int64_t)c->tuples->size() / 4)) {
+            c->led.fetch_add(1);
+        } else {
+            c->passed.fetch_add(1);
+        }
+    }
+}
+
+int mode_sbjob()
+{
+    LfqPool pool(4);
+    LfqSbCache cache;
+    std::vector<int32_t> t;
+    const int64_t n = SB_N + 8;
+
+    {
+        std::mutex lm;
+        std::condition_variable lcv;
+        LfqSbJob job(&lm, &lcv, &pool, &cache, counted_sb);
+        sb_tuples(t, 0);
+        CHECK(job.collect(t.data(), n) == 0, "a job that was never armed had something to collect");
+        uint64_t seq;
+        {
+            std::lock_guard<std::mutex> lk(lm);
+            seq = job.arm_locked();
+        }
+        CHECK(job.collect(t.data(), n) == 2, "the collector did not start the armed job");
+        sb_expect_all_once(t, cache, "collector alone", 0);
+        CHECK(!job.lead(seq, t.data(), n), "a leader started a finished job");
+        CHECK(job.collect(t.data(), n) == 0, "a finished job was collected twice");
+        for (int i = 0; i < SB_N; i++) {
+            CHECK(g_calls[i].load() == 0, "late leader: item %d computed again", i);
+        }
+        {
+            std::lock_guard<std::mutex> lk(lm);
+            seq = job.arm_locked();
+        }
+        CHECK(!job.lead(seq - 1, t.data(), n), "a wake-up of the batch before started this batch's job");
+        CHECK(job.lead(seq, t.data(), n), "the leader did not start the armed job");
+        CHECK(job.collect(t.data(), n) == 0, "collect after the leader's whole run");
+        sb_expect_all_once(t, cache, "leader alone", 0);
+        {
+            std::lock_guard<std::mutex> lk(lm);
+            seq = job.arm_locked();
+        }
+        CHECK(job.collect(t.data(), 0) == 2 && job.collect(t.data(), 0) == 0, "an empty job");
+    }
+
+    int led = 0, passed = 0;
+    {
+        MiniCtx c;
+        LfqSbJob job(&c.lm, &c.lcv, &pool, &cache, counted_sb);
+        c.job = &job;
+        c.tuples = &t;
+        std::thread leader(mini_leader, &c);
+        const int rounds = 300;
+        for (int r = 0; r < rounds; r++) {
+            sb_tuples(t, r + 1);
+            {
+                std::lock_guard<std::mutex> lk(c.lm);
+                c.leader_go++;
+                job.arm_locked();
+            }
+            c.lcv.notify_all();
+            for (int spin = 0; spin < (r % 7) * 300; spin++) {
+                std::this_thread::yield();
+            }
+            job.collect(t.data(), n);
+            sb_expect_all_once(t, cache, "race", r);
+        }
+        {
+            std::lock_guard<std::mutex> lk(c.lm);
+            c.leader_stop = 1;
+        }
+        c.lcv.notify_all();
+        leader.join();
+        led = c.led.load();
+        passed = c.passed.load();
+        CHECK(led + passed <= rounds, "the leader ran %d + %d times in %d rounds", led, passed, rounds);
+        for (int i = 0; i < SB_N; i++) {
+            CHECK(g_calls[i].load() == 0, "after the race: item %d computed again", i);
+        }
+    }
+
+    {
+        MiniCtx c;
+        LfqSbJob job(&c.lm, &c.lcv, &pool, &cache, counted_sb);
+        c.job = &job;
+        c.tuples = &t;
+        Latch hold;
+        g_hold = &hold;
+        g_holding.store(0);
+        sb_tuples(t, 1000);
+        std::thread leader(mini_leader, &c);
+        {
+            std::lock_guard<std::mutex> lk(c.lm);
+            c.leader_go++;
+            job.arm_locked();
+        }
+        c.lcv.notify_all();
+        while (!g_holding.load()) {
+            std::this_thread::yield();
+        }
+        {
+            std::lock_guard<std::mutex> lk(c.lm);
+            c.leader_stop = 1;
+        }
+        c.lcv.notify_all();
+        std::atomic<int> collected(-1), collecting(0);
+        std::thread collector([&] {
+            collecting.store(1);
+            collected.store(job.collect(t.data(), n));
+        });
+        while (!collecting.load()) {
+            std::this_thread::yield();
+        }
+        for (;;) {
+            int done = 0;
+            for (int i = 1; i < SB_N; i++) {
+                done += g_calls[i].load();
+            }
+            if (done == SB_N - 1) {
+                break;
+            }
+            std::this_thread::yield();
+        }
+        hold.release();
+        collector.join();
+        leader.join();
+        g_hold = nullptr;
+        CHECK(collected.load() == 1 || collected.load() == 0, "the collector started a job that was running: %d", collected.load());
+        CHECK(c.led.load() == 1, "the leader started the job %d times", c.led.load());
+        sb_expect_all_once(t, cache, "stop in mid-job", 0);
+    }
+    {
+        MiniCtx c;
+        LfqSbJob job(&c.lm, &c.lcv, &pool, &cache, counted_sb);
+        c.job = &job;
+        c.tuples = &t;
+        std::thread leader(mini_leader, &c);
+        {
+            std::lock_guard<std::mutex> lk(c.lm);
+            c.leader_go++;
+            job.arm_locked();
+            c.leader_stop = 1;
+        }
+        c.lcv.notify_all();
+        leader.join();
+        for (int i = 0; i < SB_N; i++) {
+            g_calls[i].store(0);
+        }
+    }
+    {
+        std::mutex lm;
+        std::condition_variable lcv;
+        LfqSbJob job(&lm, &lcv, &pool, &cache, counted_sb);
+        Latch hold;
+        g_hold = &hold;
+        g_holding.store(0);
+        sb_tuples(t, 2000);
+        uint64_t seq;
+        {
+            std::lock_guard<std::mutex> lk(lm);
+            seq = job.arm_locked();
+        }
+        std::thread leader([&] { CHECK(job.lead(seq, t.data(), n), "the leader did not start the armed job"); });
+        while (!g_holding.load()) {
+            std::this_thread::yield();
+        }
+        {
+            std::lock_guard<std::mutex> lk(lm);
+            job.arm_locked();
+        }
+        hold.release();
+        leader.join();
+        g_hold = nullptr;
+        for (int i = 0; i < SB_N; i++) {
+            CHECK(g_calls[i].load() == 1, "armed over a running job: item %d computed %d times", i, g_calls[i].load());
+            g_calls[i].store(0);
+        }
+        CHECK(job.collect(t.data(), n) == 2, "the job armed over a running one was lost");
+        sb_expect_all_once(t, cache, "armed over a running job", 0);
+    }
+    printf("ok sbjob: in the race the leader started %d jobs and found %d taken\n", led, passed);
+    return 0;
+}
+
+
+class OnePool {
+public:
+    explicit OnePool(int n)
+    {
+        for (int i = 0; i < n; i++) {
+            threads_.emplace_back([this, i] { loop(i); });
+        }
+    }
+    ~OnePool()
+    {
+        {
+            std::lock_guard<std::mutex> lk(m_);
+            stop_ = true;
+            generation_++;
+        }
+        cv_start_.notify_all();
+        for (auto &t : threads_) {
+            t.join();
+        }
+    }
+    int size() const { return (int)threads_.size(); }
+    bool run(const std::function<void()> &f, int helpers)
+    {
+        helpers = std::max(0, std::min(helpers, size()));
+        if (helpers == 0) {
+            f();
+            return true;
+        }
+        std::unique_lock<std::mutex> call_lock(call_m_, std::try_to_lock);
+        if (!call_lock.owns_lock()) {
+            f();
+            return false;
+        }
+        {
+            std::lock_guard<std::mutex> lk(m_);
+            job_ = &f;
+            want_ = helpers;
+            pending_ = helpers;
+            generation_++;
+        }
+        cv_start_.notify_all();
+        f();
+        std::unique_lock<std::mutex> lk(m_);
+        cv_done_.wait(lk, [&] { return pending_ == 0; });
+        job_ = nullptr;
+        return true;
+    }
+
+private:
+    void loop(int idx)
+    {
+        int seen = 0;
+        for (;;) {
+            const std::function<void()> *job = nullptr;
+            {
+                std::unique_lock<std::mutex> lk(m_);
+                cv_start_.wait(lk, [&] { return generation_ != seen; });
+                seen = generation_;
+                if (stop_) {
+                    return;
+                }
+                if (idx >= want_) {
+                    continue;
+                }
+                job = job_;
+            }
+            (*job)();
+            {
+                std::lock_guard<std::mutex> lk(m_);
+                pending_--;
+            }
+            cv_done_.notify_one();
+        }
+    }
+    std::vector<std::thread> threads_;
+    std::mutex m_, call_m_;
+    std::condition_variable cv_start_, cv_done_;
+    const std::function<void()> *job_ = nullptr;
+    int generation_ = 0, want_ = 0, pending_ = 0;
+    bool stop_ = false;
+};
+
+void c3_tuples(std::vector<int32_t> &t)
+{
+    t.clear();
+    for (int i = 0; i < 250; i++) {
+        const int32_t row[4] = {5000 + (i * 13) % 90 - 45, 5000 - (i * 7) % 80 + 40, 2500 + (i * 11) % 70 - 35, 2500 - (i * 5) % 60 + 30};
+        t.insert(t.end(), row, row + 4);
+    }
+    for (int i = 0; i < 754; i++) {
+        const int alt = 16 + (i * 37) % 500;
+        const int32_t row[4] = {4900 + (i * 3) % 150, 4950 - (i * 5) % 140, alt / 2 + i % 3, alt - alt / 2};
+        t.insert(t.end(), row, row + 4);
+    }
+}
+
+template <typename Pool>
+void finishing_thread(Pool &pool, std::atomic<bool> &stop)
+{
+    std::vector<double> sink(768);
+    while (!stop.load()) {
+        std::atomic<int> next(0);
+        const std::function<void()> work = [&] {
+            for (;;) {
+                const int i0 = next.fetch_add(64);
+                if (i0 >= 768) {
+                    break;
+                }
+                for (int i = i0; i < i0 + 64; i++) {
+                    long double x = 1.0L + i;
+                    for (int k = 0; k < 6; k++) {
+                        x = 1.0L + 1e-3L * (long double)lfq_sb_phred(30 + i % 7, 28, 3 + k, 2);
+                    }
+                    sink[(size_t)i] = (double)x;
+                }
+            }
+        };
+        pool.run(work, std::min(pool.size(), 8));
+        std::this_thread::sleep_for(std::chrono::microseconds(200));
+    }
+}
+
+int mode_timing(int P)
+{
+    std::vector<int32_t> t;
+    c3_tuples(t);
+    const int64_t n = (int64_t)t.size() / 4;
+    const int reps = 40;
+    std::vector<double> one_ms, one_alone_ms, new_ms;
+    int alone = 0;
+    {
+        const double t0 = now_ms();
+        long s = 0;
+        for (int64_t i = 0; i < n; i++) {
+            s += lfq_sb_phred(t[4 * (size_t)i], t[4 * (size_t)i + 1], t[4 * (size_t)i + 2], t[4 * (size_t)i + 3]);
+        }
+        printf("timing: %ld tuples, one thread %.3f ms (sum %ld), pool of %d\n", (long)n, now_ms() - t0, s, P);
+    }
+    {
+        OnePool pool(P);
+        std::atomic<bool> stop(false);
+        std::thread fin([&] { finishing_thread(pool, stop); });
+        for (int r = 0; r < reps; r++) {
+            std::vector<std::pair<LfqSbKey, int>> items;
+            for (int64_t i = 0; i < n; i++) {
+                const int32_t *q = &t[4 * (size_t)i];
+                items.push_back({LfqSbKey{q[0], q[1], q[2], q[3]}, 0});
+            }
+            const double t0 = now_ms();
+            std::sort(items.begin(), items.end(), [](const std::pair<LfqSbKey, int> &x, const std::pair<LfqSbKey, int> &y) {
+                return (int64_t)x.first.c + x.first.d > (int64_t)y.first.c + y.first.d;
+            });
+            std::atomic<int64_t> next(0);
+            const int64_t m = (int64_t)items.size();
+            const std::function<void()> work = [&] {
+                for (;;) {
+                    const int64_t i = next.fetch_add(1);
+                    if (i >= m) {
+                        break;
+                    }
+                    const LfqSbKey &k = items[(size_t)i].first;
+                    items[(size_t)i].second = lfq_sb_phred(k.a, k.b, k.c, k.d);
+                }
+            };
+            const bool shared = pool.run(work, (int)std::min<int64_t>(pool.size(), m / 2));
+            const double dt = now_ms() - t0;
+            (shared ? one_ms : one_alone_ms).push_back(dt);
+            alone += !shared;
+            std::this_thread::sleep_for(std::chrono::microseconds(700 + 130 * (r % 11)));
+        }
+        stop.store(true);
+        fin.join();
+    }
+    {
+        LfqPool pool(P);
+        LfqSbCache cache;
+        std::mutex lm;
+        std::condition_variable lcv;
+        LfqSbJob job(&lm, &lcv, &pool, &cache);
+        std::atomic<bool> stop(false);
+        std::thread fin([&] { finishing_thread(pool, stop); });
+        for (int r = 0; r < reps; r++) {
+            uint64_t seq;
+            {
+                std::lock_guard<std::mutex> lk(lm);
+                seq = job.arm_locked();
+            }
+            const double t0 = now_ms();
+            CHECK(job.lead(seq, t.data(), n), "the job did not start");
+            CHECK(job.collect(t.data(), n) == 0, "the job was not finished");
+            new_ms.push_back(now_ms() - t0);
+            std::this_thread::sleep_for(std::chrono::microseconds(700 + 130 * (r % 11)));
+        }
+        stop.store(true);
+        fin.join();
+    }
+    auto stats = [](std::vector<double> v, const char *name) {
+        if (v.empty()) {
+            printf("timing: %-44s none\n", name);
+            return;
+        }
+        std::sort(v.begin(), v.end());
+        printf("timing: %-44s %2zu runs  min %.3f  median %.3f  max %.3f ms\n", name, v.size(), v.front(), v[v.size() / 2], v.back());
+    };
+    stats(one_ms, "one job at a time, got the pool");
+    stats(one_alone_ms, "one job at a time, found it taken (alone)");
+    stats(new_ms, "shared pool");
+    printf("ok timing: %d of %d precomputes ran alone on the pool that takes one job at a time\n", alone, reps);
+    return 0;
+}
+
+}
+
+int main(int argc, char **argv)
+{
+    const char *mode = argc > 1 ? argv[1] : "";
+    if (!strcmp(mode, "callers")) {
+        return mode_callers();
+    }
+    if (!strcmp(mode, "noalone")) {
+        return mode_noalone();
+    }
+    if (!strcmp(mode, "sbjob")) {
+        return mode_sbjob();
+    }
+    if (!strcmp(mode, "timing")) {
+        const int hw = (int)std::thread::hardware_concurrency();
+        return mode_timing(argc > 2 ? atoi(argv[2]) : std::max(1, std::min(hw - 1, 15)));
+    }
+    fprintf(stderr, "usage: lfq_pool_check callers | noalone | sbjob | timing [pool threads]\n");
+    return 2;
+}
```

After: 389.0 million, median of 4. About the same (+0.1%).
